# pierotofy/OpenSplat

Hardware: NVIDIA H100
Metric: fwd_bwd_mpixel_per_s (higher is better)
Workload: dtype f32

## Files before the change

include/gsplat_b200.h:

```cpp
#ifndef GSPLAT_B200_H
#define GSPLAT_B200_H

#include <stddef.h>
#include <stdint.h>

#ifdef __cplusplus
extern "C" {
#endif

#define GSB_TILE 16
#define GSB_ERR_INVALID_ARG (-1)
#define GSB_ERR_WORKSPACE (-2)
#define GSB_ERR_UNSUPPORTED (-3)
#define GSB_RASTER_CLAMP_MAX_ONE 1u
#define GSB_BIN_COUNT_VISIBLE 2

typedef void *gsb_stream_t;

int gsb_version(void);
const char *gsb_last_error(void);

int gsb_sh_forward(int n, int degree, int degrees_to_use, const float *viewdirs, const float *coeffs,
                   float *colors, gsb_stream_t stream);
int gsb_sh_backward(int n, int degree, int degrees_to_use, const float *viewdirs, const float *v_colors,
                    float *v_coeffs, gsb_stream_t stream);

int gsb_sh_forward_rgb(int n, int degree, int degrees_to_use, const float *viewdirs, const float *coeffs,
                       float bias, float *rgbs, gsb_stream_t stream);
int gsb_sh_backward_rgb(int n, int degree, int degrees_to_use, const float *viewdirs, const float *rgbs,
                        const float *v_rgbs, float *v_coeffs, gsb_stream_t stream);

int gsb_sh_forward_split(int n, int degree, int degrees_to_use, const float *means, const float *cam_pos,
                         const float *features_dc, const float *features_rest, float bias, float *rgbs,
                         gsb_stream_t stream);
int gsb_sh_backward_split(int n, int degree, int degrees_to_use, const float *means, const float *cam_pos,
                          const float *rgbs, const float *v_rgbs, float *v_features_dc, float *v_features_rest,
                          gsb_stream_t stream);
int gsb_sh_forward_rgb_cam(int n, int degree, int degrees_to_use, const float *means, const float *cam_pos,
                           const float *coeffs, float bias, float *rgbs, gsb_stream_t stream);
int gsb_sh_backward_rgb_cam(int n, int degree, int degrees_to_use, const float *means, const float *cam_pos,
                            const float *rgbs, const float *v_rgbs, float *v_coeffs, gsb_stream_t stream);
int gsb_sh_forward_rgb_cam_multiview(int n, int degree, int degrees_to_use, const float *means, int num_views,
                                     const float *cam_positions, const float *coeffs, float bias, float *rgbs,
                                     gsb_stream_t stream);

int gsb_mask_rgb_grad(int n, const float *rgbs, float *v_rgbs, gsb_stream_t stream);
int gsb_sh_backward_multiview(int n, int degree, int degrees_to_use, const float *means, int num_views,
                              const float *cam_positions, const float *const *v_rgbs_per_view, float scale,
                              float *v_coeffs, gsb_stream_t stream);
int gsb_exchange_gradients(int n, int degree, int degrees_to_use, const float *means, int num_views,
                           const float *cam_positions, const float *const *v_rgbs_per_view, float scale,
                           float *v_coeffs, int rank, int world, long long geom_floats,
                           float *const *geom_per_rank, float *geom_multicast, gsb_stream_t stream);
int gsb_sh_backward_multiview_cams(int n, int degree, int degrees_to_use, const float *means, int num_views,
                                   const float *const *cam_pos_per_view, const float *const *v_rgbs_per_view,
                                   float scale, float *v_coeffs, gsb_stream_t stream);
int gsb_exchange_gradients_cams(int n, int degree, int degrees_to_use, const float *means, int num_views,
                                const float *const *cam_pos_per_view, const float *const *v_rgbs_per_view,
                                float scale, float *v_coeffs, int rank, int world, long long geom_floats,
                                float *const *geom_per_rank, float *geom_multicast, gsb_stream_t stream);

int gsb_project_forward(int n, const float *means3d, const float *scales, float glob_scale,
                        const float *quats, const float *viewmat, const float *projmat, float fx, float fy,
                        float cx, float cy, int img_h, int img_w, int tiles_x, int tiles_y,
                        float clip_thresh, float *cov3d, float *xys, float *depths, int32_t *radii,
                        float *conics, int32_t *num_tiles_hit, gsb_stream_t stream);
int gsb_project_backward(int n, const float *means3d, const float *scales, float glob_scale,
                         const float *quats, const float *viewmat, const float *projmat, float fx, float fy,
                         float cx, float cy, int img_h, int img_w, const float *cov3d,
                         const int32_t *radii, const float *conics, const float *v_xy,
                         const float *v_depth, const float *v_conic, float *v_mean3d, float *v_scale,
                         float *v_quat, gsb_stream_t stream);
int gsb_project_forward_activated(int n, const float *means3d, const float *log_scales, float glob_scale,
                                  const float *raw_quats, const float *opacity_logits, const float *viewmat,
                                  const float *projmat, float fx, float fy, float cx, float cy, int img_h,
                                  int img_w, int tiles_x, int tiles_y, float clip_thresh, float *cov3d, float *xys,
                                  float *depths, int32_t *radii, float *conics, int32_t *num_tiles_hit,
                                  float *opacities, gsb_stream_t stream);
int gsb_project_backward_activated(int n, const float *means3d, const float *log_scales, float glob_scale,
                                   const float *raw_quats, const float *opacities, const float *viewmat,
                                   const float *projmat, float fx, float fy, int img_h, int img_w,
                                   const int32_t *radii, const float *conics, const float *v_xy,
                                   const float *v_depth, const float *v_conic, const float *v_opacity,
                                   float *v_mean3d, float *v_log_scales, float *v_raw_quats,
                                   float *v_opacity_logits, gsb_stream_t stream);
int gsb_project_backward_activated_acc(int n, const float *means3d, const float *log_scales, float glob_scale,
                                       const float *raw_quats, const float *opacities, const float *viewmat,
                                       const float *projmat, float fx, float fy, int img_h, int img_w,
                                       const int32_t *radii, const float *conics, const float *v_xy,
                                       const float *v_depth, const float *v_conic, const float *v_opacity,
                                       float *v_mean3d, float *v_log_scales, float *v_raw_quats,
                                       float *v_opacity_logits, gsb_stream_t stream);
int gsb_project_forward_activated_aa(int n, const float *means3d, const float *log_scales, float glob_scale,
                                     const float *raw_quats, const float *opacity_logits, const float *viewmat,
                                     const float *projmat, float fx, float fy, float cx, float cy, int img_h,
                                     int img_w, int tiles_x, int tiles_y, float clip_thresh, float *cov3d, float *xys,
                                     float *depths, int32_t *radii, float *conics, int32_t *num_tiles_hit,
                                     float *opacities, gsb_stream_t stream);
int gsb_project_backward_activated_aa(int n, const float *means3d, const float *log_scales, float glob_scale,
                                      const float *raw_quats, const float *opacity_logits, const float *viewmat,
                                      const float *projmat, float fx, float fy, int img_h, int img_w,
                                      const int32_t *radii, const float *conics, const float *v_xy,
                                      const float *v_depth, const float *v_conic, const float *v_opacity,
                                      float *v_mean3d, float *v_log_scales, float *v_raw_quats,
                                      float *v_opacity_logits, gsb_stream_t stream);
int gsb_project_backward_activated_aa_acc(int n, const float *means3d, const float *log_scales, float glob_scale,
                                          const float *raw_quats, const float *opacity_logits, const float *viewmat,
                                          const float *projmat, float fx, float fy, int img_h, int img_w,
                                          const int32_t *radii, const float *conics, const float *v_xy,
                                          const float *v_depth, const float *v_conic, const float *v_opacity,
                                          float *v_mean3d, float *v_log_scales, float *v_raw_quats,
                                          float *v_opacity_logits, gsb_stream_t stream);

size_t gsb_cumsum_workspace_bytes(int n);
int gsb_cumsum_tiles_hit(int n, const int32_t *num_tiles_hit, int32_t *cum_tiles_hit, void *workspace,
                         size_t workspace_bytes, gsb_stream_t stream);
int gsb_map_gaussian_to_intersects(int n, int m, const float *xys, const float *depths,
                                   const int32_t *radii, const int32_t *cum_tiles_hit, int tiles_x,
                                   int tiles_y, int64_t *isect_ids, int32_t *gaussian_ids,
                                   gsb_stream_t stream);
size_t gsb_sort_workspace_bytes(int m);
int gsb_sort_intersects(int m, int num_tiles, const int64_t *isect_ids, int64_t *isect_ids_sorted,
                        int32_t *sorted_index, void *workspace, size_t workspace_bytes,
                        gsb_stream_t stream);
int gsb_gather_bin_edges(int m, int num_tiles, const int64_t *isect_ids_sorted,
                         const int32_t *sorted_index, const int32_t *gaussian_ids,
                         int32_t *gaussian_ids_sorted, int32_t *tile_bins, gsb_stream_t stream);

int gsb_bucket_max_tile_len(void);
size_t gsb_bucket_workspace_bytes(int n, int m_capacity, int num_tiles);
int gsb_bucket_tile_ranges(int n, const float *xys, const int32_t *radii, const float *conics, const float *colors,
                           const float *opacities, int cull, int tiles_x, int tiles_y, int m_capacity,
                           int len_capacity, void *workspace, size_t workspace_bytes, int32_t *cum_tiles_hit,
                           int32_t *tile_bins, int32_t *tile_order, int32_t *stats, gsb_stream_t stream);
int gsb_bucket_sort_pack(int n, int m_capacity, int len_capacity, const float *depths, const int32_t *radii,
                         const int32_t *cum_tiles_hit, int cull, int tiles_x, int tiles_y, const int32_t *tile_bins,
                         const int32_t *stats, void *workspace, size_t workspace_bytes, void *records,
                         int32_t *sorted_index, int32_t *gaussian_ids_sorted, gsb_stream_t stream);

size_t gsb_raster_records_bytes(int m);
size_t gsb_raster_grad_rows_bytes(int m);
int gsb_pack_records(int m, const int32_t *gaussian_ids_sorted, const int32_t *sorted_index, const float *xys,
                     const float *conics, const float *colors, const float *opacities, void *records,
                     gsb_stream_t stream);
int gsb_rasterize_forward_packed(int img_h, int img_w, int tiles_x, int tiles_y, int m, const int32_t *tile_bins,
                                 const int32_t *tile_order, const int32_t *bin_stats, const float *background,
                                 void *records, float *out_img, float *final_Ts, int32_t *final_idx,
                                 unsigned flags, gsb_stream_t stream);
int gsb_rasterize_forward_count(int img_h, int img_w, int tiles_x, int tiles_y, int m, const int32_t *tile_bins,
                                const float *background, void *records, float *out_img, float *final_Ts,
                                int32_t *final_idx, unsigned long long *pair_counts, gsb_stream_t stream);
int gsb_rasterize_backward(int img_h, int img_w, int tiles_x, int tiles_y, int n, int m, const int32_t *tile_bins,
                           const int32_t *tile_order, const float *conics, const float *opacities, void *records,
                           const int32_t *cum_tiles_hit, const float *background, const float *final_Ts,
                           const int32_t *final_idx, const float *v_output, const float *v_output_alpha,
                           void *grad_rows, float *v_xy, float *v_conic, float *v_colors, float *v_opacity,
                           unsigned flags, gsb_stream_t stream);
int gsb_gather_record_depths(int m, const int32_t *gaussian_ids_sorted, const float *depths, const int32_t *bin_stats,
                             float *record_depths, gsb_stream_t stream);
int gsb_rasterize_forward_packed_depth(int img_h, int img_w, int tiles_x, int tiles_y, int m, const int32_t *tile_bins,
                                       const int32_t *tile_order, const int32_t *bin_stats, const float *background,
                                       void *records, float *out_img, float *final_Ts, int32_t *final_idx,
                                       unsigned flags, const float *record_depths, float *out_depth, float *out_alpha,
                                       gsb_stream_t stream);
int gsb_rasterize_backward_depth(int img_h, int img_w, int tiles_x, int tiles_y, int n, int m,
                                 const int32_t *tile_bins, const int32_t *tile_order, const float *conics,
                                 const float *opacities, void *records, const int32_t *cum_tiles_hit,
                                 const float *background, const float *final_Ts, const int32_t *final_idx,
                                 const float *v_output, const float *v_output_alpha, void *grad_rows, float *v_xy,
                                 float *v_conic, float *v_colors, float *v_opacity, unsigned flags,
                                 const float *record_depths, const float *v_output_depth, float *v_depths,
                                 gsb_stream_t stream);
int gsb_rasterize_backward_absgrad(int img_h, int img_w, int tiles_x, int tiles_y, int n, int m,
                                   const int32_t *tile_bins, const int32_t *tile_order, const float *conics,
                                   const float *opacities, void *records, const int32_t *cum_tiles_hit,
                                   const float *background, const float *final_Ts, const int32_t *final_idx,
                                   const float *v_output, const float *v_output_alpha, void *grad_rows, float *v_xy,
                                   float *v_conic, float *v_colors, float *v_opacity, unsigned flags,
                                   const float *record_depths, const float *v_output_depth, float *v_depths,
                                   float *v_xy_abs, gsb_stream_t stream);

int gsb_mse_loss_grad(long long n, const float *img, const float *target, float *v_img, float *loss_out,
                      float inv_count, gsb_stream_t stream);
int gsb_adam_step(long long n, float *param, const float *grad, float *exp_avg, float *exp_avg_sq, float lr,
                  float beta1, float beta2, float eps, float bias_correction1, float bias_correction2,
                  gsb_stream_t stream);
#define GSB_ADAM_MAX_SEGMENTS 8
typedef struct gsb_adam_segment {
    long long offset, count;
    int row_floats, head_floats;
    float lr_head, lr_rest;
} gsb_adam_segment;
int gsb_adam_step_segments(int num_segments, const gsb_adam_segment *segments, float *param, const float *grad,
                           float *exp_avg, float *exp_avg_sq, float beta1, float beta2, float eps,
                           float bias_correction1, float bias_correction2, gsb_stream_t stream);

int gsb_activate_forward(int n, const float *means, const float *log_scales, const float *raw_quats,
                         const float *opacity_logits, const float *cam_pos, float *scales, float *quats,
                         float *opacities, float *viewdirs, gsb_stream_t stream);
int gsb_activate_backward(int n, const float *scales, const float *raw_quats, const float *opacities,
                          const float *v_scales, const float *v_quats, const float *v_opacities,
                          float *v_log_scales, float *v_raw_quats, float *v_opacity_logits, gsb_stream_t stream);

int gsb_densify_stats_update(int n, const float *v_xy, const int32_t *radii, int img_h, int img_w,
                             float *xys_grad_norm, float *vis_counts, float *max_2d_size, gsb_stream_t stream);
int gsb_densify_stats_init(int n, const float *v_xy, const int32_t *radii, int img_h, int img_w,
                           float *xys_grad_norm, float *vis_counts, float *max_2d_size, gsb_stream_t stream);

size_t gsb_densify_workspace_bytes(int n);
int gsb_densify_classify(int n, const float *scales, const float *opacities, const float *xys_grad_norm,
                         const float *vis_counts, const float *max_2d_size, float max_dim,
                         float densify_grad_thresh, float densify_size_thresh, int check_split_screen,
                         float split_screen_size, float cull_alpha_thresh, int check_huge, float cull_scale_thresh,
                         int check_cull_screen, float cull_screen_size, float size_fac, void *workspace,
                         size_t workspace_bytes, int32_t *src_map, int32_t *split_rank, int32_t *counts,
                         gsb_stream_t stream);
int gsb_densify_means_scales(int new_n, int n_splits, const int32_t *src_map, const int32_t *split_rank,
                             const float *samples, const float *means, const float *scales, const float *quats,
                             float size_fac, float *new_means, float *new_scales, gsb_stream_t stream);
int gsb_densify_gather_rows(int new_n, int row_floats, const int32_t *src_map, const float *src, float *dst,
                            int zero_children, gsb_stream_t stream);
int gsb_reset_opacity(int n, float max_logit, float *opacities, float *exp_avg, float *exp_avg_sq,
                      gsb_stream_t stream);

#define GSB_MCMC_MAX_SEGMENTS 8
typedef struct gsb_row_segment {
    long long offset;
    int row_floats, reserved;
} gsb_row_segment;
size_t gsb_mcmc_workspace_bytes(int n);
int gsb_mcmc_plan(int n, const float *logits, float min_opacity, int mask_dead, void *workspace,
                  size_t workspace_bytes, double *cdf, int32_t *dead, int32_t *result, gsb_stream_t stream);
int gsb_mcmc_sample(int num_samples, int n, const double *cdf, unsigned key0, unsigned key1, int step, int tag,
                    int32_t *samples, int32_t *counts, gsb_stream_t stream);
int gsb_mcmc_relocate(int n, const int32_t *counts, float min_opacity, float *logits, float *log_scales,
                      int zero_moments, int num_segments, const gsb_row_segment *segments, float *exp_avg,
                      float *exp_avg_sq, gsb_stream_t stream);
int gsb_mcmc_copy_rows(int num_rows, const int32_t *dst_rows, const int32_t *src_rows, int num_segments,
                       const gsb_row_segment *segments, float *param, gsb_stream_t stream);
int gsb_mcmc_regularize(int n, const float *logits, const float *log_scales, float opacity_coef, float scale_coef,
                        float *grad_logits, float *grad_log_scales, gsb_stream_t stream);
int gsb_mcmc_add_noise(int n, const float *logits, const float *log_scales, const float *raw_quats, unsigned key0,
                       unsigned key1, int step, float noise_scale, float *means, gsb_stream_t stream);
int gsb_mcmc_draws(int count, unsigned key0, unsigned key1, int step, int tag, int32_t *words, float *normals,
                   gsb_stream_t stream);

#define GSB_BILAGRID_X 16
#define GSB_BILAGRID_Y 16
#define GSB_BILAGRID_L 8
#define GSB_BILAGRID_COEFFS 12
#define GSB_BILAGRID_FLOATS (GSB_BILAGRID_L * GSB_BILAGRID_Y * GSB_BILAGRID_X * GSB_BILAGRID_COEFFS)
int gsb_bilagrid_slice_forward(int H, int W, const float *grid, const float *rgb, float *out, gsb_stream_t stream);
size_t gsb_bilagrid_workspace_bytes(int H, int W);
int gsb_bilagrid_slice_backward(int H, int W, const float *grid, const float *rgb, const float *v_out, float scale,
                                float *v_rgb, float *v_grid, void *workspace, size_t workspace_bytes,
                                gsb_stream_t stream);
int gsb_bilagrid_tv(int num_grids, const float *grids, float weight, float *v_grids, float *tv_out,
                    gsb_stream_t stream);

#define GSB_POSE_FLOATS 9
size_t gsb_project_camera_partials_floats(int n);
int gsb_project_backward_activated_camgrad(int n, const float *means3d, const float *log_scales, float glob_scale,
                                           const float *raw_quats, const float *opacities, const float *viewmat,
                                           const float *projmat, float fx, float fy, int img_h, int img_w,
                                           const int32_t *radii, const float *conics, const float *v_xy,
                                           const float *v_depth, const float *v_conic, const float *v_opacity,
                                           float *v_mean3d, float *v_log_scales, float *v_raw_quats,
                                           float *v_opacity_logits, int accumulate, int antialiased,
                                           float *cam_partials, gsb_stream_t stream);
int gsb_project_camera_grad_reduce(int nblocks, const float *partials, float *v_viewmat, float *v_projmat,
                                   gsb_stream_t stream);
int gsb_pose_apply(const float *pose, const float *view, const float *centre, float *view_out, float *centre_out,
                   gsb_stream_t stream);
int gsb_pose_backward(const float *pose, const float *view, const float *proj, const float *v_viewmat,
                      const float *v_projmat, float scale, float *grad, gsb_stream_t stream);

int gsb_inverse_depths(int n, const float *depths, const int32_t *radii, float *inv, gsb_stream_t stream);
int gsb_inverse_depths_backward(int n, const float *depths, const int32_t *radii, const float *v_inv, float *v_z,
                                gsb_stream_t stream);
size_t gsb_inverse_depth_l1_workspace_bytes(int img_h, int img_w);
int gsb_inverse_depth_l1(int img_h, int img_w, const float *rendered, const float *prior, float scale_g,
                         float *v_rendered, float *loss_out, void *workspace, size_t workspace_bytes,
                         gsb_stream_t stream);
int gsb_depth_downscale_mean(int h, int w, int factor, const float *src, float *dst, gsb_stream_t stream);

int gsb_ply_row_floats(int sh_bases);
int gsb_pack_ply_rows(int n, int sh_bases, const float *means, const float *features_dc, int dc_stride,
                      const float *features_rest, int rest_stride, const float *opacities, const float *scales,
                      const float *quats, int keep_crs, float crs_scale, const float *crs_translation,
                      float *out_rows, gsb_stream_t stream);
int gsb_unpack_ply_rows(int n, int sh_bases, const float *rows, int keep_crs, float crs_scale,
                        const float *crs_translation, float *means, float *features_dc, int dc_stride,
                        float *features_rest, int rest_stride, float *opacities, float *scales, float *quats,
                        gsb_stream_t stream);
int gsb_splat_order_keys(int n, const float *scales, const float *opacities, int keep_crs, float crs_scale,
                         int64_t *keys, gsb_stream_t stream);
int gsb_pack_splat_rows(int n, const int32_t *order, const float *means, const float *scales,
                        const float *features_dc, int dc_stride, const float *opacities, const float *quats,
                        int keep_crs, float crs_scale, const float *crs_translation, void *out_rows,
                        gsb_stream_t stream);

size_t gsb_ssim_workspace_bytes(int img_h, int img_w);
int gsb_ssim_l1_loss(int img_h, int img_w, const float *rendered, const float *gt, float ssim_weight,
                     float *v_rendered, float *loss_out, void *workspace, size_t workspace_bytes,
                     gsb_stream_t stream);

size_t gsb_knn_workspace_bytes(int n);
int gsb_knn_mean_dist(int n, const float *xyz, float *mean_dist, void *workspace, size_t workspace_bytes,
                      gsb_stream_t stream);

#define GSB_FILTER3D_CAM_FLOATS 18
int gsb_project_forward_activated_filter3d(int n, const float *means3d, const float *log_scales, float glob_scale,
                                           const float *raw_quats, const float *opacity_logits, const float *filter3d,
                                           const float *viewmat, const float *projmat, float fx, float fy, float cx,
                                           float cy, int img_h, int img_w, int tiles_x, int tiles_y,
                                           float clip_thresh, float *cov3d, float *xys, float *depths, int32_t *radii,
                                           float *conics, int32_t *num_tiles_hit, float *opacities, int antialiased,
                                           gsb_stream_t stream);
int gsb_project_backward_activated_filter3d(int n, const float *means3d, const float *log_scales, float glob_scale,
                                            const float *raw_quats, const float *opacity_logits,
                                            const float *filter3d, const float *viewmat, const float *projmat,
                                            float fx, float fy, int img_h, int img_w, const int32_t *radii,
                                            const float *conics, const float *v_xy, const float *v_depth,
                                            const float *v_conic, const float *v_opacity, float *v_mean3d,
                                            float *v_log_scales, float *v_raw_quats, float *v_opacity_logits,
                                            int accumulate, int antialiased, int camgrad, float *cam_partials,
                                            gsb_stream_t stream);
size_t gsb_filter3d_workspace_bytes(void);
int gsb_filter3d_compute(int n, const float *means, int num_cameras, const float *cameras, float near, float margin,
                         float variance, void *workspace, size_t workspace_bytes, float *filter3d,
                         gsb_stream_t stream);
int gsb_filter3d_bake(int n, const float *log_scales, const float *opacity_logits, const float *filter3d,
                      float *out_log_scales, float *out_opacity_logits, gsb_stream_t stream);
int gsb_reset_opacity_filter3d(int n, float max_logit, float reset_value, const float *log_scales,
                               const float *filter3d, float *opacities, float *exp_avg, float *exp_avg_sq,
                               gsb_stream_t stream);

int gsb_resize_area_u8(int src_h, int src_w, const uint8_t *src, int dst_h, int dst_w, uint8_t *dst, float inv_scale,
                       gsb_stream_t stream);
int gsb_undistort_u8(int h, int w, const uint8_t *src, float fx, float fy, float cx, float cy, float k1, float k2,
                     float p1, float p2, float k3, float new_fx, float new_fy, float new_cx, float new_cy, int roi_x,
                     int roi_y, int roi_w, int roi_h, uint8_t *dst, gsb_stream_t stream);
int gsb_u8_to_f32_views(int num_views, const int64_t *views, int h, int w, float *out, gsb_stream_t stream);

#ifdef __cplusplus
}
#endif
#endif
```

opensplat_b200/capi.py:

```python
import ctypes as C
import os

import torch

_HERE = os.path.dirname(os.path.abspath(__file__))
LIB_PATH = os.environ.get("GSB_LIB") or os.path.join(_HERE, "lib", "libgsplat_b200.so")
_lib = None

_vp, _i, _f, _sz = C.c_void_p, C.c_int, C.c_float, C.c_size_t

_SIGS = {
    "gsb_version": (C.c_int, []),
    "gsb_last_error": (C.c_char_p, []),
    "gsb_sh_forward": (_i, [_i, _i, _i, _vp, _vp, _vp, _vp]),
    "gsb_sh_backward": (_i, [_i, _i, _i, _vp, _vp, _vp, _vp]),
    "gsb_sh_forward_rgb": (_i, [_i, _i, _i, _vp, _vp, _f, _vp, _vp]),
    "gsb_sh_backward_rgb": (_i, [_i, _i, _i, _vp, _vp, _vp, _vp, _vp]),
    "gsb_sh_forward_split": (_i, [_i, _i, _i, _vp, _vp, _vp, _vp, _f, _vp, _vp]),
    "gsb_sh_backward_split": (_i, [_i, _i, _i, _vp, _vp, _vp, _vp, _vp, _vp, _vp]),
    "gsb_sh_forward_rgb_cam": (_i, [_i, _i, _i, _vp, _vp, _vp, _f, _vp, _vp]),
    "gsb_sh_backward_rgb_cam": (_i, [_i, _i, _i, _vp, _vp, _vp, _vp, _vp, _vp]),
    "gsb_sh_forward_rgb_cam_multiview": (_i, [_i, _i, _i, _vp, _i, _vp, _vp, _f, _vp, _vp]),
    "gsb_mask_rgb_grad": (_i, [_i, _vp, _vp, _vp]),
    "gsb_sh_backward_multiview": (_i, [_i, _i, _i, _vp, _i, _vp, _vp, _f, _vp, _vp]),
    "gsb_exchange_gradients": (_i, [_i, _i, _i, _vp, _i, _vp, _vp, _f, _vp, _i, _i, C.c_longlong, _vp, _vp, _vp]),
    "gsb_sh_backward_multiview_cams": (_i, [_i, _i, _i, _vp, _i, _vp, _vp, _f, _vp, _vp]),
    "gsb_exchange_gradients_cams": (_i, [_i, _i, _i, _vp, _i, _vp, _vp, _f, _vp, _i, _i, C.c_longlong, _vp, _vp,
                                         _vp]),
    "gsb_project_forward": (_i, [_i, _vp, _vp, _f, _vp, _vp, _vp, _f, _f, _f, _f, _i, _i, _i, _i, _f,
                                 _vp, _vp, _vp, _vp, _vp, _vp, _vp]),
    "gsb_project_backward": (_i, [_i, _vp, _vp, _f, _vp, _vp, _vp, _f, _f, _f, _f, _i, _i,
                                  _vp, _vp, _vp, _vp, _vp, _vp, _vp, _vp, _vp, _vp]),
    "gsb_project_forward_activated": (_i, [_i, _vp, _vp, _f, _vp, _vp, _vp, _vp, _f, _f, _f, _f, _i, _i, _i, _i, _f,
                                           _vp, _vp, _vp, _vp, _vp, _vp, _vp, _vp]),
    "gsb_project_backward_activated": (_i, [_i, _vp, _vp, _f, _vp, _vp, _vp, _vp, _f, _f, _i, _i,
                                            _vp, _vp, _vp, _vp, _vp, _vp, _vp, _vp, _vp, _vp, _vp]),
    "gsb_project_backward_activated_acc": (_i, [_i, _vp, _vp, _f, _vp, _vp, _vp, _vp, _f, _f, _i, _i,
                                                _vp, _vp, _vp, _vp, _vp, _vp, _vp, _vp, _vp, _vp, _vp]),
    "gsb_project_forward_activated_aa": (_i, [_i, _vp, _vp, _f, _vp, _vp, _vp, _vp, _f, _f, _f, _f, _i, _i, _i, _i,
                                              _f, _vp, _vp, _vp, _vp, _vp, _vp, _vp, _vp]),
    "gsb_project_backward_activated_aa": (_i, [_i, _vp, _vp, _f, _vp, _vp, _vp, _vp, _f, _f, _i, _i,
                                               _vp, _vp, _vp, _vp, _vp, _vp, _vp, _vp, _vp, _vp, _vp]),
    "gsb_project_backward_activated_aa_acc": (_i, [_i, _vp, _vp, _f, _vp, _vp, _vp, _vp, _f, _f, _i, _i,
                                                   _vp, _vp, _vp, _vp, _vp, _vp, _vp, _vp, _vp, _vp, _vp]),
    "gsb_cumsum_workspace_bytes": (_sz, [_i]),
    "gsb_cumsum_tiles_hit": (_i, [_i, _vp, _vp, _vp, _sz, _vp]),
    "gsb_map_gaussian_to_intersects": (_i, [_i, _i, _vp, _vp, _vp, _vp, _i, _i, _vp, _vp, _vp]),
    "gsb_sort_workspace_bytes": (_sz, [_i]),
    "gsb_sort_intersects": (_i, [_i, _i, _vp, _vp, _vp, _vp, _sz, _vp]),
    "gsb_gather_bin_edges": (_i, [_i, _i, _vp, _vp, _vp, _vp, _vp, _vp]),
    "gsb_raster_records_bytes": (_sz, [_i]),
    "gsb_raster_grad_rows_bytes": (_sz, [_i]),
    "gsb_pack_records": (_i, [_i, _vp, _vp, _vp, _vp, _vp, _vp, _vp, _vp]),
    "gsb_rasterize_forward_packed": (_i, [_i, _i, _i, _i, _i, _vp, _vp, _vp, _vp, _vp, _vp, _vp, _vp, C.c_uint, _vp]),
    "gsb_rasterize_forward_count": (_i, [_i, _i, _i, _i, _i, _vp, _vp, _vp, _vp, _vp, _vp, _vp, _vp]),
    "gsb_rasterize_backward": (_i, [_i, _i, _i, _i, _i, _i, _vp, _vp, _vp, _vp, _vp, _vp, _vp, _vp, _vp, _vp,
                                    _vp, _vp, _vp, _vp, _vp, _vp, C.c_uint, _vp]),
    "gsb_gather_record_depths": (_i, [_i, _vp, _vp, _vp, _vp, _vp]),
    "gsb_rasterize_forward_packed_depth": (_i, [_i, _i, _i, _i, _i, _vp, _vp, _vp, _vp, _vp, _vp, _vp, _vp, C.c_uint,
                                                _vp, _vp, _vp, _vp]),
    "gsb_rasterize_backward_depth": (_i, [_i, _i, _i, _i, _i, _i, _vp, _vp, _vp, _vp, _vp, _vp, _vp, _vp, _vp, _vp,
                                          _vp, _vp, _vp, _vp, _vp, _vp, C.c_uint, _vp, _vp, _vp, _vp]),
    "gsb_rasterize_backward_absgrad": (_i, [_i, _i, _i, _i, _i, _i, _vp, _vp, _vp, _vp, _vp, _vp, _vp, _vp, _vp, _vp,
                                            _vp, _vp, _vp, _vp, _vp, _vp, C.c_uint, _vp, _vp, _vp, _vp, _vp]),
    "gsb_bucket_max_tile_len": (_i, []),
    "gsb_bucket_workspace_bytes": (_sz, [_i, _i, _i]),
    "gsb_bucket_tile_ranges": (_i, [_i, _vp, _vp, _vp, _vp, _vp, _i, _i, _i, _i, _i, _vp, _sz, _vp, _vp, _vp, _vp, _vp]),
    "gsb_bucket_sort_pack": (_i, [_i, _i, _i, _vp, _vp, _vp, _i, _i, _i, _vp, _vp, _vp, _sz, _vp, _vp, _vp, _vp]),
    "gsb_activate_forward": (_i, [_i, _vp, _vp, _vp, _vp, _vp, _vp, _vp, _vp, _vp, _vp]),
    "gsb_activate_backward": (_i, [_i, _vp, _vp, _vp, _vp, _vp, _vp, _vp, _vp, _vp, _vp]),
    "gsb_densify_stats_update": (_i, [_i, _vp, _vp, _i, _i, _vp, _vp, _vp, _vp]),
    "gsb_densify_stats_init": (_i, [_i, _vp, _vp, _i, _i, _vp, _vp, _vp, _vp]),
    "gsb_densify_workspace_bytes": (_sz, [_i]),
    "gsb_densify_classify": (_i, [_i, _vp, _vp, _vp, _vp, _vp, _f, _f, _f, _i, _f, _f, _i, _f, _i, _f, _f, _vp, _sz,
                                  _vp, _vp, _vp, _vp]),
    "gsb_densify_means_scales": (_i, [_i, _i, _vp, _vp, _vp, _vp, _vp, _vp, _f, _vp, _vp, _vp]),
    "gsb_densify_gather_rows": (_i, [_i, _i, _vp, _vp, _vp, _i, _vp]),
    "gsb_reset_opacity": (_i, [_i, _f, _vp, _vp, _vp, _vp]),
    "gsb_mcmc_workspace_bytes": (_sz, [_i]),
    "gsb_mcmc_plan": (_i, [_i, _vp, _f, _i, _vp, _sz, _vp, _vp, _vp, _vp]),
    "gsb_mcmc_sample": (_i, [_i, _i, _vp, C.c_uint, C.c_uint, _i, _i, _vp, _vp, _vp]),
    "gsb_mcmc_relocate": (_i, [_i, _vp, _f, _vp, _vp, _i, _i, _vp, _vp, _vp, _vp]),
    "gsb_mcmc_copy_rows": (_i, [_i, _vp, _vp, _i, _vp, _vp, _vp]),
    "gsb_mcmc_regularize": (_i, [_i, _vp, _vp, _f, _f, _vp, _vp, _vp]),
    "gsb_mcmc_add_noise": (_i, [_i, _vp, _vp, _vp, C.c_uint, C.c_uint, _i, _f, _vp, _vp]),
    "gsb_mcmc_draws": (_i, [_i, C.c_uint, C.c_uint, _i, _i, _vp, _vp, _vp]),
    "gsb_bilagrid_slice_forward": (_i, [_i, _i, _vp, _vp, _vp, _vp]),
    "gsb_bilagrid_workspace_bytes": (_sz, [_i, _i]),
    "gsb_bilagrid_slice_backward": (_i, [_i, _i, _vp, _vp, _vp, _f, _vp, _vp, _vp, _sz, _vp]),
    "gsb_bilagrid_tv": (_i, [_i, _vp, _f, _vp, _vp, _vp]),
    "gsb_project_camera_partials_floats": (_sz, [_i]),
    "gsb_project_backward_activated_camgrad": (_i, [_i, _vp, _vp, _f, _vp, _vp, _vp, _vp, _f, _f, _i, _i,
                                                    _vp, _vp, _vp, _vp, _vp, _vp, _vp, _vp, _vp, _vp, _i, _i, _vp,
                                                    _vp]),
    "gsb_project_camera_grad_reduce": (_i, [_i, _vp, _vp, _vp, _vp]),
    "gsb_pose_apply": (_i, [_vp, _vp, _vp, _vp, _vp, _vp]),
    "gsb_pose_backward": (_i, [_vp, _vp, _vp, _vp, _vp, _f, _vp, _vp]),
    "gsb_inverse_depths": (_i, [_i, _vp, _vp, _vp, _vp]),
    "gsb_inverse_depths_backward": (_i, [_i, _vp, _vp, _vp, _vp, _vp]),
    "gsb_inverse_depth_l1_workspace_bytes": (_sz, [_i, _i]),
    "gsb_inverse_depth_l1": (_i, [_i, _i, _vp, _vp, _f, _vp, _vp, _vp, _sz, _vp]),
    "gsb_depth_downscale_mean": (_i, [_i, _i, _i, _vp, _vp, _vp]),
    "gsb_project_forward_activated_filter3d": (_i, [_i, _vp, _vp, _f, _vp, _vp, _vp, _vp, _vp, _f, _f, _f, _f, _i, _i,
                                                    _i, _i, _f, _vp, _vp, _vp, _vp, _vp, _vp, _vp, _i, _vp]),
    "gsb_project_backward_activated_filter3d": (_i, [_i, _vp, _vp, _f, _vp, _vp, _vp, _vp, _vp, _f, _f, _i, _i,
                                                     _vp, _vp, _vp, _vp, _vp, _vp, _vp, _vp, _vp, _vp, _i, _i, _i,
                                                     _vp, _vp]),
    "gsb_filter3d_workspace_bytes": (_sz, []),
    "gsb_filter3d_compute": (_i, [_i, _vp, _i, _vp, _f, _f, _f, _vp, _sz, _vp, _vp]),
    "gsb_filter3d_bake": (_i, [_i, _vp, _vp, _vp, _vp, _vp, _vp]),
    "gsb_reset_opacity_filter3d": (_i, [_i, _f, _f, _vp, _vp, _vp, _vp, _vp, _vp]),
    "gsb_ply_row_floats": (_i, [_i]),
    "gsb_pack_ply_rows": (_i, [_i, _i, _vp, _vp, _i, _vp, _i, _vp, _vp, _vp, _i, _f, C.POINTER(C.c_float), _vp, _vp]),
    "gsb_unpack_ply_rows": (_i, [_i, _i, _vp, _i, _f, C.POINTER(C.c_float), _vp, _vp, _i, _vp, _i, _vp, _vp, _vp, _vp]),
    "gsb_splat_order_keys": (_i, [_i, _vp, _vp, _i, _f, _vp, _vp]),
    "gsb_pack_splat_rows": (_i, [_i, _vp, _vp, _vp, _vp, _i, _vp, _vp, _i, _f, C.POINTER(C.c_float), _vp, _vp]),
    "gsb_ssim_workspace_bytes": (_sz, [_i, _i]),
    "gsb_ssim_l1_loss": (_i, [_i, _i, _vp, _vp, _f, _vp, _vp, _vp, _sz, _vp]),
    "gsb_adam_step": (_i, [C.c_longlong, _vp, _vp, _vp, _vp, _f, _f, _f, _f, _f, _f, _vp]),
    "gsb_adam_step_segments": (_i, [_i, _vp, _vp, _vp, _vp, _vp, _f, _f, _f, _f, _f, _vp]),
    "gsb_mse_loss_grad": (_i, [C.c_longlong, _vp, _vp, _vp, _vp, _f, _vp]),
    "gsb_knn_workspace_bytes": (_sz, [_i]),
    "gsb_knn_mean_dist": (_i, [_i, _vp, _vp, _vp, _sz, _vp]),
    "gsb_resize_area_u8": (_i, [_i, _i, _vp, _i, _i, _vp, _f, _vp]),
    "gsb_undistort_u8": (_i, [_i, _i, _vp, _f, _f, _f, _f, _f, _f, _f, _f, _f, _f, _f, _f, _f, _i, _i, _i, _i, _vp,
                              _vp]),
    "gsb_u8_to_f32_views": (_i, [_i, _vp, _i, _i, _vp, _vp]),
}

ADAM_MAX_SEGMENTS = 8


class AdamSegment(C.Structure):
    _fields_ = [("offset", C.c_longlong), ("count", C.c_longlong), ("row_floats", C.c_int),
                ("head_floats", C.c_int), ("lr_head", C.c_float), ("lr_rest", C.c_float)]


MCMC_MAX_SEGMENTS = 8


class RowSegment(C.Structure):
    _fields_ = [("offset", C.c_longlong), ("row_floats", C.c_int), ("reserved", C.c_int)]


BILAGRID_X, BILAGRID_Y, BILAGRID_L, BILAGRID_COEFFS = 16, 16, 8, 12
BILAGRID_FLOATS = BILAGRID_L * BILAGRID_Y * BILAGRID_X * BILAGRID_COEFFS
POSE_FLOATS = 9
CAMGRAD_TERMS = 24
FILTER3D_CAM_FLOATS = 18


_OPT_SIGS = {}


class GsbError(RuntimeError):
    pass


def lib():
    global _lib
    if _lib is None:
        if not os.path.exists(LIB_PATH):
            raise GsbError(f"{LIB_PATH} not built -- run `python -m opensplat_b200.build` "
                           "(there is no CPU fallback)")
        L = C.CDLL(LIB_PATH)
        for name, (res, args) in _SIGS.items():
            fn = getattr(L, name)
            fn.restype, fn.argtypes = res, args
        for name, (res, args) in _OPT_SIGS.items():
            if hasattr(L, name):
                fn = getattr(L, name)
                fn.restype, fn.argtypes = res, args
        _lib = L
    return _lib


def exported_symbols():
    return list(_SIGS.keys())


def check(code):
    if code != 0:
        raise GsbError(lib().gsb_last_error().decode() or f"gsplat_b200 error {code}")


def ptr(t):
    if t is None:
        return None
    if not t.is_cuda:
        raise GsbError("gsplat_b200 kernels need CUDA tensors (no CPU fallback)")
    if not t.is_contiguous():
        raise GsbError("tensor must be contiguous")
    return t.data_ptr()


def stream():
    return torch.cuda.current_stream().cuda_stream


def f32(t):
    return t.contiguous() if t.dtype == torch.float32 else t.float().contiguous()
```

opensplat_b200/csrc/project.cu:

```cuda
#include "gsb_common.cuh"

namespace {

constexpr int PJ_THREADS = 256;
constexpr int CG_TERMS = 24;

__device__ __forceinline__ void camgrad_block_sum(const float (&cg)[CG_TERMS], float *__restrict__ out) {
    __shared__ float red[PJ_THREADS / 32][CG_TERMS];
    const int lane = threadIdx.x & 31, warp = threadIdx.x >> 5;
#pragma unroll
    for (int k = 0; k < CG_TERMS; ++k) {
        float v = cg[k];
#pragma unroll
        for (int o = 16; o > 0; o >>= 1) v = v + __shfl_down_sync(0xffffffffu, v, o);
        if (lane == 0) red[warp][k] = v;
    }
    __syncthreads();
    if (threadIdx.x < CG_TERMS) {
        float v = red[0][threadIdx.x];
#pragma unroll
        for (int w = 1; w < PJ_THREADS / 32; ++w) v = v + red[w][threadIdx.x];
        out[threadIdx.x] = v;
    }
}

struct Cam {
    float V[12];
    float P[16];
};

__device__ __forceinline__ void quat_to_rotmat(float qw, float qx, float qy, float qz, float R[3][3]) {
    float s = 1.0f / sqrtf(qw * qw + qx * qx + qy * qy + qz * qz);
    float w = qw * s, x = qx * s, y = qy * s, z = qz * s;
    R[0][0] = 1.f - 2.f * (y * y + z * z);
    R[0][1] = 2.f * (x * y - w * z);
    R[0][2] = 2.f * (x * z + w * y);
    R[1][0] = 2.f * (x * y + w * z);
    R[1][1] = 1.f - 2.f * (x * x + z * z);
    R[1][2] = 2.f * (y * z - w * x);
    R[2][0] = 2.f * (x * z - w * y);
    R[2][1] = 2.f * (y * z + w * x);
    R[2][2] = 1.f - 2.f * (x * x + y * y);
}

__device__ __forceinline__ void load_cam(const float *__restrict__ viewmat,
                                         const float *__restrict__ projmat, Cam &c) {
#pragma unroll
    for (int i = 0; i < 12; ++i) c.V[i] = __ldg(viewmat + i);
#pragma unroll
    for (int i = 0; i < 16; ++i) c.P[i] = __ldg(projmat + i);
}

__device__ __forceinline__ void filter3d_scales(float glob_scale, const float (&e)[3], float f, float (&sig)[3],
                                                float (&r)[3], float &c3) {
    const float ff = f * f;
#pragma unroll
    for (int k = 0; k < 3; ++k) {
        const float s = glob_scale * e[k];
        sig[k] = sqrtf(s * s + ff);
        r[k] = s / sig[k];
    }
    c3 = r[0] * r[1] * r[2];
}

template <bool ACT, bool AA = false, bool F3D = false>
__global__ void __launch_bounds__(PJ_THREADS)
project_forward_kernel(int n, const float *__restrict__ means3d, const float *__restrict__ scales,
                       float glob_scale, const float *__restrict__ quats,
                       const float *__restrict__ viewmat, const float *__restrict__ projmat, float fx,
                       float fy, float cx, float cy, float tan_fovx, float tan_fovy, int img_h, int img_w,
                       int tiles_x, int tiles_y, float clip_thresh, float *__restrict__ cov3d,
                       float2 *__restrict__ xys, float *__restrict__ depths, int *__restrict__ radii,
                       float *__restrict__ conics, int *__restrict__ num_tiles_hit,
                       const float *__restrict__ opacity_logits, float *__restrict__ opacities,
                       const float *__restrict__ filter3d = nullptr) {
    static_assert(ACT || !AA, "the anti-aliased opacity needs the activated projection");
    static_assert(ACT || !F3D, "the 3-D filter needs the activated projection");
    const int i = blockIdx.x * PJ_THREADS + threadIdx.x;
    if (i >= n) return;
    if (ACT && !AA && !F3D) opacities[i] = 1.f / (1.f + expf(-opacity_logits[i]));
    float fsig[3] = {0.f, 0.f, 0.f}, fc3 = 1.f;
    if constexpr (F3D) {
        const float e[3] = {expf(scales[3 * i]), expf(scales[3 * i + 1]), expf(scales[3 * i + 2])};
        float r[3];
        filter3d_scales(glob_scale, e, filter3d[i], fsig, r, fc3);
        if (!AA) opacities[i] = 1.f / (1.f + expf(-opacity_logits[i])) * fc3;
    }
    float comp = 0.f;
    Cam cam;
    load_cam(viewmat, projmat, cam);
    const float *V = cam.V, *P = cam.P;

    float c3[6] = {0.f, 0.f, 0.f, 0.f, 0.f, 0.f};
    float conic0 = 0.f, conic1 = 0.f, conic2 = 0.f;
    float ux = 0.f, uy = 0.f, depth = 0.f;
    int radius_i = 0, area = 0;

    const float px = means3d[3 * i], py = means3d[3 * i + 1], pz = means3d[3 * i + 2];
    const float tx = V[0] * px + V[1] * py + V[2] * pz + V[3];
    const float ty = V[4] * px + V[5] * py + V[6] * pz + V[7];
    const float tz = V[8] * px + V[9] * py + V[10] * pz + V[11];
    if (tz > clip_thresh) {
        const float4 q = reinterpret_cast<const float4 *>(quats)[i];
        float R[3][3], M[3][3];
        quat_to_rotmat(q.x, q.y, q.z, q.w, R);
        const float a0 = scales[3 * i], a1 = scales[3 * i + 1], a2 = scales[3 * i + 2];
        const float s0 = F3D ? fsig[0] : glob_scale * (ACT ? expf(a0) : a0),
                    s1 = F3D ? fsig[1] : glob_scale * (ACT ? expf(a1) : a1),
                    s2 = F3D ? fsig[2] : glob_scale * (ACT ? expf(a2) : a2);
#pragma unroll
        for (int r = 0; r < 3; ++r) {
            M[r][0] = R[r][0] * s0;
            M[r][1] = R[r][1] * s1;
            M[r][2] = R[r][2] * s2;
        }
        float C[3][3];
#pragma unroll
        for (int r = 0; r < 3; ++r)
#pragma unroll
            for (int c = 0; c < 3; ++c)
                C[r][c] = M[r][0] * M[c][0] + M[r][1] * M[c][1] + M[r][2] * M[c][2];
        c3[0] = C[0][0]; c3[1] = C[0][1]; c3[2] = C[0][2];
        c3[3] = C[1][1]; c3[4] = C[1][2]; c3[5] = C[2][2];

        const float lim_x = 1.3f * tan_fovx, lim_y = 1.3f * tan_fovy;
        const float ttx = tz * fminf(lim_x, fmaxf(-lim_x, tx / tz));
        const float tty = tz * fminf(lim_y, fmaxf(-lim_y, ty / tz));
        const float rz = 1.f / tz, rz2 = rz * rz;
        const float J00 = fx * rz, J02 = -fx * ttx * rz2, J11 = fy * rz, J12 = -fy * tty * rz2;
        float T[2][3];
#pragma unroll
        for (int c = 0; c < 3; ++c) {
            T[0][c] = J00 * V[c] + J02 * V[8 + c];
            T[1][c] = J11 * V[4 + c] + J12 * V[8 + c];
        }
        const float Cs[3][3] = {{c3[0], c3[1], c3[2]}, {c3[1], c3[3], c3[4]}, {c3[2], c3[4], c3[5]}};
        float TV[2][3];
#pragma unroll
        for (int r = 0; r < 2; ++r)
#pragma unroll
            for (int c = 0; c < 3; ++c)
                TV[r][c] = T[r][0] * Cs[0][c] + T[r][1] * Cs[1][c] + T[r][2] * Cs[2][c];
        const float cxx0 = TV[0][0] * T[0][0] + TV[0][1] * T[0][1] + TV[0][2] * T[0][2];
        const float cxy = TV[0][0] * T[1][0] + TV[0][1] * T[1][1] + TV[0][2] * T[1][2];
        const float cyy0 = TV[1][0] * T[1][0] + TV[1][1] * T[1][1] + TV[1][2] * T[1][2];
        const float cxx = cxx0 + 0.3f, cyy = cyy0 + 0.3f;

        const float det = cxx * cyy - cxy * cxy;
        if (det != 0.f) {
            const float inv_det = 1.f / det;
            conic0 = cyy * inv_det;
            conic1 = -cxy * inv_det;
            conic2 = cxx * inv_det;
            const float b = 0.5f * (cxx + cyy);
            const float sq = sqrtf(fmaxf(0.1f, b * b - det));
            const float v1 = b + sq, v2 = b - sq;
            const float radius = ceilf(3.f * sqrtf(fmaxf(v1, v2)));

            const float hx = P[0] * px + P[1] * py + P[2] * pz + P[3];
            const float hy = P[4] * px + P[5] * py + P[6] * pz + P[7];
            const float hw = P[12] * px + P[13] * py + P[14] * pz + P[15];
            const float rw = 1.f / (hw + 1e-6f);
            const float ndcx = hx * rw, ndcy = hy * rw;
            const float pxc = 0.5f * (float)img_w * ndcx + cx - 0.5f;
            const float pyc = 0.5f * (float)img_h * ndcy + cy - 0.5f;

            int x0, x1, y0, y1;
            gsb_tile_bbox(pxc, pyc, radius, tiles_x, tiles_y, x0, x1, y0, y1);
            const int a = (x1 - x0) * (y1 - y0);
            if (a > 0) {
                area = a;
                depth = tz;
                radius_i = (int)radius;
                ux = pxc;
                uy = pyc;
                if (AA && radius_i > 0) comp = sqrtf(fmaxf(0.f, (cxx0 * cyy0 - cxy * cxy) / det));
            }
        }
    }
    if constexpr (AA && F3D) opacities[i] = 1.f / (1.f + expf(-opacity_logits[i])) * fc3 * comp;
    else if (AA) opacities[i] = 1.f / (1.f + expf(-opacity_logits[i])) * comp;
    float *c3o = cov3d + 6 * (size_t)i;
#pragma unroll
    for (int k = 0; k < 6; ++k) c3o[k] = c3[k];
    xys[i] = make_float2(ux, uy);
    depths[i] = depth;
    radii[i] = radius_i;
    conics[3 * i] = conic0;
    conics[3 * i + 1] = conic1;
    conics[3 * i + 2] = conic2;
    num_tiles_hit[i] = area;
}

template <bool ACT, bool ACC, bool AA = false, bool CAMGRAD = false, bool F3D = false>
__global__ void __launch_bounds__(PJ_THREADS)
project_backward_kernel(int n, const float *__restrict__ means3d, const float *__restrict__ scales,
                        float glob_scale, const float *__restrict__ quats,
                        const float *__restrict__ viewmat, const float *__restrict__ projmat, float fx,
                        float fy, float tan_fovx, float tan_fovy, int img_h, int img_w,
                        const int *__restrict__ radii, const float *__restrict__ conics,
                        const float2 *__restrict__ v_xy, const float *__restrict__ v_depth,
                        const float *__restrict__ v_conic, float *__restrict__ v_mean3d,
                        float *__restrict__ v_scale, float4 *__restrict__ v_quat,
                        const float *__restrict__ opacities, const float *__restrict__ v_opacity,
                        float *__restrict__ v_opacity_logits, float *__restrict__ cam_partials = nullptr,
                        const float *__restrict__ filter3d = nullptr) {
    static_assert(ACT || !AA, "the anti-aliased opacity needs the activated projection");
    static_assert(ACT || !F3D, "the 3-D filter needs the activated projection");
    static_assert(ACT || !CAMGRAD, "the camera gradient is taken with the activated projection");
    const int i = blockIdx.x * PJ_THREADS + threadIdx.x;
    if (!CAMGRAD && i >= n) return;
    float cg[CG_TERMS];
#pragma unroll
    for (int k = 0; k < CG_TERMS; ++k) cg[k] = 0.f;
    if (!CAMGRAD || i < n) {
        float comp = 0.f;
        float f3 = 0.f, fr[3] = {1.f, 1.f, 1.f}, fc3 = 1.f, fsh[3] = {0.f, 0.f, 0.f};
        if constexpr (F3D) f3 = filter3d[i];
        if (ACT && !AA && !F3D) {
            const float o = opacities[i];
            if constexpr (ACC)
                v_opacity_logits[i] = v_opacity_logits[i] + (v_opacity ? v_opacity[i] * o * (1.f - o) : 0.f);
            else
                v_opacity_logits[i] = v_opacity ? v_opacity[i] * o * (1.f - o) : 0.f;
        }
        float vm[3] = {0.f, 0.f, 0.f}, vs[3] = {0.f, 0.f, 0.f};
        float4 vq = make_float4(0.f, 0.f, 0.f, 0.f);
        if (radii[i] > 0) {
            Cam cam;
            load_cam(viewmat, projmat, cam);
            const float *V = cam.V, *P = cam.P;
            const float px = means3d[3 * i], py = means3d[3 * i + 1], pz = means3d[3 * i + 2];

            const float hx = P[0] * px + P[1] * py + P[2] * pz + P[3];
            const float hy = P[4] * px + P[5] * py + P[6] * pz + P[7];
            const float hw = P[12] * px + P[13] * py + P[14] * pz + P[15];
            const float rw = 1.f / (hw + 1e-6f);
            const float2 vxy = v_xy[i];
            const float vndcx = 0.5f * (float)img_w * vxy.x, vndcy = 0.5f * (float)img_h * vxy.y;
            const float vhx = vndcx * rw, vhy = vndcy * rw;
            const float vhw = -(vndcx * hx + vndcy * hy) * rw * rw;
            vm[0] = P[0] * vhx + P[4] * vhy + P[12] * vhw;
            vm[1] = P[1] * vhx + P[5] * vhy + P[13] * vhw;
            vm[2] = P[2] * vhx + P[6] * vhy + P[14] * vhw;

            const float tx = V[0] * px + V[1] * py + V[2] * pz + V[3];
            const float ty = V[4] * px + V[5] * py + V[6] * pz + V[7];
            const float tz = V[8] * px + V[9] * py + V[10] * pz + V[11];
            float vtx = 0.f, vty = 0.f, vtz = v_depth ? v_depth[i] : 0.f;

            const float A = conics[3 * i], B = conics[3 * i + 1], Cc = conics[3 * i + 2];
            const float gA = v_conic[3 * i], gB = 0.5f * v_conic[3 * i + 1], gC = v_conic[3 * i + 2];
            const float xg00 = A * gA + B * gB, xg01 = A * gB + B * gC;
            const float xg10 = B * gA + Cc * gB, xg11 = B * gB + Cc * gC;
            float vS00 = -(xg00 * A + xg01 * B);
            float vS01 = -(xg00 * B + xg01 * Cc);
            float vS11 = -(xg10 * B + xg11 * Cc);

            const float4 q = reinterpret_cast<const float4 *>(quats)[i];
            float R[3][3], M[3][3];
            quat_to_rotmat(q.x, q.y, q.z, q.w, R);
            const float a[3] = {scales[3 * i], scales[3 * i + 1], scales[3 * i + 2]};
            const float e[3] = {ACT ? expf(a[0]) : a[0], ACT ? expf(a[1]) : a[1], ACT ? expf(a[2]) : a[2]};
            float s[3] = {glob_scale * e[0], glob_scale * e[1], glob_scale * e[2]};
            if constexpr (F3D) filter3d_scales(glob_scale, e, f3, s, fr, fc3);
#pragma unroll
            for (int r = 0; r < 3; ++r)
#pragma unroll
                for (int c = 0; c < 3; ++c) M[r][c] = R[r][c] * s[c];
            float Cs[3][3];
#pragma unroll
            for (int r = 0; r < 3; ++r)
#pragma unroll
                for (int c = 0; c < 3; ++c)
                    Cs[r][c] = M[r][0] * M[c][0] + M[r][1] * M[c][1] + M[r][2] * M[c][2];
            const float lim_x = 1.3f * tan_fovx, lim_y = 1.3f * tan_fovy;
            const float qx = tx / tz, qy = ty / tz;
            const bool clamp_x = !(qx > -lim_x && qx < lim_x), clamp_y = !(qy > -lim_y && qy < lim_y);
            const float cqx = fminf(lim_x, fmaxf(-lim_x, qx)), cqy = fminf(lim_y, fmaxf(-lim_y, qy));
            const float ttx = tz * cqx, tty = tz * cqy;
            const float rz = 1.f / tz, rz2 = rz * rz, rz3 = rz2 * rz;
            const float J00 = fx * rz, J02 = -fx * ttx * rz2, J11 = fy * rz, J12 = -fy * tty * rz2;
            float T[2][3];
#pragma unroll
            for (int c = 0; c < 3; ++c) {
                T[0][c] = J00 * V[c] + J02 * V[8 + c];
                T[1][c] = J11 * V[4 + c] + J12 * V[8 + c];
            }
            if constexpr (AA) {
                float TV[2][3];
#pragma unroll
                for (int r = 0; r < 2; ++r)
#pragma unroll
                    for (int c = 0; c < 3; ++c)
                        TV[r][c] = T[r][0] * Cs[0][c] + T[r][1] * Cs[1][c] + T[r][2] * Cs[2][c];
                const float cxx0 = TV[0][0] * T[0][0] + TV[0][1] * T[0][1] + TV[0][2] * T[0][2];
                const float cxy = TV[0][0] * T[1][0] + TV[0][1] * T[1][1] + TV[0][2] * T[1][2];
                const float cyy0 = TV[1][0] * T[1][0] + TV[1][1] * T[1][1] + TV[1][2] * T[1][2];
                const float det = (cxx0 + 0.3f) * (cyy0 + 0.3f) - cxy * cxy;
                comp = sqrtf(fmaxf(0.f, (cxx0 * cyy0 - cxy * cxy) / det));
                if (v_opacity && comp > 0.f) {
                    const float o = 1.f / (1.f + expf(-opacities[i]));
                    const float k = 0.5f * (v_opacity[i] * (F3D ? o * fc3 : o)) / comp;
                    const float id = 1.f / det;
                    const float a = cyy0 * id, b = cxy * id, c = cxx0 * id, e = 0.3f * id;
                    vS00 = vS00 + k * (0.3f * (a * a + b * b + e * a));
                    vS01 = vS01 - k * (0.3f * (b * (a + c + e)));
                    vS11 = vS11 + k * (0.3f * (c * c + b * b + e * c));
                }
            }
            float vST[2][3];
#pragma unroll
            for (int c = 0; c < 3; ++c) {
                vST[0][c] = vS00 * T[0][c] + vS01 * T[1][c];
                vST[1][c] = vS01 * T[0][c] + vS11 * T[1][c];
            }
            float vV[3][3];
#pragma unroll
            for (int r = 0; r < 3; ++r)
#pragma unroll
                for (int c = 0; c < 3; ++c) vV[r][c] = T[0][r] * vST[0][c] + T[1][r] * vST[1][c];
            float vT[2][3];
#pragma unroll
            for (int r = 0; r < 2; ++r)
#pragma unroll
                for (int c = 0; c < 3; ++c)
                    vT[r][c] = 2.f * (vST[r][0] * Cs[0][c] + vST[r][1] * Cs[1][c] + vST[r][2] * Cs[2][c]);
            const float vJ00 = vT[0][0] * V[0] + vT[0][1] * V[1] + vT[0][2] * V[2];
            const float vJ02 = vT[0][0] * V[8] + vT[0][1] * V[9] + vT[0][2] * V[10];
            const float vJ11 = vT[1][0] * V[4] + vT[1][1] * V[5] + vT[1][2] * V[6];
            const float vJ12 = vT[1][0] * V[8] + vT[1][1] * V[9] + vT[1][2] * V[10];
            const float vttx = -fx * rz2 * vJ02, vtty = -fy * rz2 * vJ12;
            vtz += -fx * rz2 * vJ00 + 2.f * fx * ttx * rz3 * vJ02 - fy * rz2 * vJ11 +
                   2.f * fy * tty * rz3 * vJ12;
            if (qx == lim_x || qx == -lim_x) { const float h = 0.5f * vttx; vtx += h; vtz += cqx * h; }
            else if (clamp_x) vtz += cqx * vttx; else vtx += vttx;
            if (qy == lim_y || qy == -lim_y) { const float h = 0.5f * vtty; vty += h; vtz += cqy * h; }
            else if (clamp_y) vtz += cqy * vtty; else vty += vtty;
            vm[0] += V[0] * vtx + V[4] * vty + V[8] * vtz;
            vm[1] += V[1] * vtx + V[5] * vty + V[9] * vtz;
            vm[2] += V[2] * vtx + V[6] * vty + V[10] * vtz;
            if constexpr (CAMGRAD) {
                const float pc[3] = {px, py, pz}, vt[3] = {vtx, vty, vtz}, vh[3] = {vhx, vhy, vhw};
#pragma unroll
                for (int r = 0; r < 3; ++r) {
#pragma unroll
                    for (int c = 0; c < 3; ++c) {
                        cg[4 * r + c] = vt[r] * pc[c];
                        cg[12 + 4 * r + c] = vh[r] * pc[c];
                    }
                    cg[4 * r + 3] = vt[r];
                    cg[12 + 4 * r + 3] = vh[r];
                }
#pragma unroll
                for (int c = 0; c < 3; ++c) {
                    cg[c] = cg[c] + J00 * vT[0][c];
                    cg[4 + c] = cg[4 + c] + J11 * vT[1][c];
                    cg[8 + c] = cg[8 + c] + (J02 * vT[0][c] + J12 * vT[1][c]);
                }
            }

            float vM[3][3];
#pragma unroll
            for (int r = 0; r < 3; ++r)
#pragma unroll
                for (int c = 0; c < 3; ++c)
                    vM[r][c] = 2.f * (vV[r][0] * M[0][c] + vV[r][1] * M[1][c] + vV[r][2] * M[2][c]);
#pragma unroll
            for (int c = 0; c < 3; ++c) {
                vs[c] = glob_scale * (R[0][c] * vM[0][c] + R[1][c] * vM[1][c] + R[2][c] * vM[2][c]);
                if (ACT) vs[c] = vs[c] * e[c];
                if (F3D) vs[c] = vs[c] * fr[c];
            }
            float vR[3][3];
#pragma unroll
            for (int r = 0; r < 3; ++r)
#pragma unroll
                for (int c = 0; c < 3; ++c) vR[r][c] = vM[r][c] * s[c];
            const float nq = sqrtf(q.x * q.x + q.y * q.y + q.z * q.z + q.w * q.w);
            const float inv = 1.0f / nq;
            const float w = q.x * inv, x = q.y * inv, y = q.z * inv, z = q.w * inv;
            const float gw = 2.f * (x * (vR[2][1] - vR[1][2]) + y * (vR[0][2] - vR[2][0]) + z * (vR[1][0] - vR[0][1]));
            const float gx = 2.f * (-2.f * x * (vR[1][1] + vR[2][2]) + y * (vR[1][0] + vR[0][1]) +
                                    z * (vR[2][0] + vR[0][2]) + w * (vR[2][1] - vR[1][2]));
            const float gy = 2.f * (x * (vR[1][0] + vR[0][1]) - 2.f * y * (vR[0][0] + vR[2][2]) +
                                    z * (vR[2][1] + vR[1][2]) + w * (vR[0][2] - vR[2][0]));
            const float gz = 2.f * (x * (vR[2][0] + vR[0][2]) + y * (vR[2][1] + vR[1][2]) -
                                    2.f * z * (vR[0][0] + vR[1][1]) + w * (vR[1][0] - vR[0][1]));
            const float dot = w * gw + x * gx + y * gy + z * gz;
            vq = make_float4((gw - w * dot) * inv, (gx - x * dot) * inv, (gy - y * dot) * inv,
                             (gz - z * dot) * inv);
            if constexpr (F3D) {
#pragma unroll
                for (int k = 0; k < 3; ++k) { const float t = f3 / s[k]; fsh[k] = t * t; }
            }
        } else if constexpr (F3D) {
            const float e[3] = {expf(scales[3 * i]), expf(scales[3 * i + 1]), expf(scales[3 * i + 2])};
            float sg[3];
            filter3d_scales(glob_scale, e, f3, sg, fr, fc3);
#pragma unroll
            for (int k = 0; k < 3; ++k) { const float t = f3 / sg[k]; fsh[k] = t * t; }
        }
        if constexpr (AA && !F3D) {
            float vol = 0.f;
            if (v_opacity) {
                const float o = 1.f / (1.f + expf(-opacities[i]));
                vol = v_opacity[i] * comp * o * (1.f - o);
            }
            v_opacity_logits[i] = ACC ? v_opacity_logits[i] + vol : vol;
        }
        if constexpr (F3D) {
            float vol = 0.f;
            if (v_opacity) {
                const float o = 1.f / (1.f + expf(-opacities[i]));
                vol = AA ? v_opacity[i] * fc3 * comp * o * (1.f - o) : v_opacity[i] * fc3 * o * (1.f - o);
                if (f3 > 0.f) {
                    const float vo = v_opacity[i] * (AA ? o * fc3 * comp : o * fc3);
#pragma unroll
                    for (int k = 0; k < 3; ++k) vs[k] = vs[k] + vo * fsh[k];
                }
            }
            v_opacity_logits[i] = ACC ? v_opacity_logits[i] + vol : vol;
        }
        if constexpr (ACC) {
            const float4 pq = v_quat[i];
            v_mean3d[3 * i] += vm[0]; v_mean3d[3 * i + 1] += vm[1]; v_mean3d[3 * i + 2] += vm[2];
            v_scale[3 * i] += vs[0]; v_scale[3 * i + 1] += vs[1]; v_scale[3 * i + 2] += vs[2];
            v_quat[i] = make_float4(pq.x + vq.x, pq.y + vq.y, pq.z + vq.z, pq.w + vq.w);
        } else {
            v_mean3d[3 * i] = vm[0]; v_mean3d[3 * i + 1] = vm[1]; v_mean3d[3 * i + 2] = vm[2];
            v_scale[3 * i] = vs[0]; v_scale[3 * i + 1] = vs[1]; v_scale[3 * i + 2] = vs[2];
            v_quat[i] = vq;
        }
    }
    if constexpr (CAMGRAD) camgrad_block_sum(cg, cam_partials + CG_TERMS * (size_t)blockIdx.x);
}

__global__ void __launch_bounds__(CG_TERMS * 32)
camgrad_reduce_kernel(int nblocks, const float *__restrict__ partials, float *__restrict__ v_viewmat,
                      float *__restrict__ v_projmat) {
    const int k = threadIdx.x >> 5, lane = threadIdx.x & 31;
    double s = 0.0;
    for (int b = lane; b < nblocks; b += 32) s += (double)partials[CG_TERMS * (size_t)b + k];
#pragma unroll
    for (int o = 16; o > 0; o >>= 1) s += __shfl_down_sync(0xffffffffu, s, o);
    if (lane == 0) {
        const float r = (float)s;
        if (k < 12) v_viewmat[k] = r;
        else v_projmat[k < 20 ? k - 12 : k - 8] = r;
    }
    if (threadIdx.x < 4) {
        v_viewmat[12 + threadIdx.x] = 0.f;
        v_projmat[8 + threadIdx.x] = 0.f;
    }
}

}

static int project_forward_impl(bool act, bool aa, int n, const float *means3d, const float *scales, float glob_scale,
                                const float *quats, const float *opacity_logits, const float *filter3d,
                                const float *viewmat,
                                const float *projmat, float fx, float fy, float cx, float cy, int img_h, int img_w,
                                int tiles_x, int tiles_y, float clip_thresh, float *cov3d, float *xys, float *depths,
                                int32_t *radii, float *conics, int32_t *num_tiles_hit, float *opacities,
                                gsb_stream_t stream) {
    GSB_CHECK_ARG(n >= 0 && img_h > 0 && img_w > 0 && tiles_x > 0 && tiles_y > 0);
    if (n == 0) return 0;
    GSB_CHECK_ARG(means3d && scales && quats && viewmat && projmat && cov3d && xys && depths && radii &&
                  conics && num_tiles_hit);
    GSB_CHECK_ARG(!act || (opacity_logits && opacities));
    GSB_CHECK_ARG(((uintptr_t)quats % 16) == 0 && ((uintptr_t)xys % 8) == 0);
    const float tan_fovx = (float)(0.5 * (double)img_w / (double)fx);
    const float tan_fovy = (float)(0.5 * (double)img_h / (double)fy);
#define GSB_PJ_F(A, AA, F3D) project_forward_kernel<A, AA, F3D><<<gsb_div_up(n, PJ_THREADS), PJ_THREADS, 0, (cudaStream_t)stream>>>( \
        n, means3d, scales, glob_scale, quats, viewmat, projmat, fx, fy, cx, cy, tan_fovx, tan_fovy, img_h, img_w,   \
        tiles_x, tiles_y, clip_thresh, cov3d, reinterpret_cast<float2 *>(xys), depths, radii, conics, num_tiles_hit, \
        opacity_logits, opacities, filter3d)
    if (filter3d) { if (aa) GSB_PJ_F(true, true, true); else GSB_PJ_F(true, false, true); }
    else if (aa) GSB_PJ_F(true, true, false); else if (act) GSB_PJ_F(true, false, false);
    else GSB_PJ_F(false, false, false);
#undef GSB_PJ_F
    GSB_LAUNCH_CHECK();
    return 0;
}

extern "C" int gsb_project_forward(int n, const float *means3d, const float *scales, float glob_scale,
                                   const float *quats, const float *viewmat, const float *projmat,
                                   float fx, float fy, float cx, float cy, int img_h, int img_w,
                                   int tiles_x, int tiles_y, float clip_thresh, float *cov3d, float *xys,
                                   float *depths, int32_t *radii, float *conics, int32_t *num_tiles_hit,
                                   gsb_stream_t stream) {
    return project_forward_impl(false, false, n, means3d, scales, glob_scale, quats, nullptr, nullptr, viewmat, projmat, fx, fy, cx,
                                cy, img_h, img_w, tiles_x, tiles_y, clip_thresh, cov3d, xys, depths, radii, conics,
                                num_tiles_hit, nullptr, stream);
}

extern "C" int gsb_project_forward_activated(int n, const float *means3d, const float *log_scales, float glob_scale,
                                             const float *raw_quats, const float *opacity_logits,
                                             const float *viewmat, const float *projmat, float fx, float fy,
                                             float cx, float cy, int img_h, int img_w, int tiles_x, int tiles_y,
                                             float clip_thresh, float *cov3d, float *xys, float *depths,
                                             int32_t *radii, float *conics, int32_t *num_tiles_hit,
                                             float *opacities, gsb_stream_t stream) {
    return project_forward_impl(true, false, n, means3d, log_scales, glob_scale, raw_quats, opacity_logits, nullptr, viewmat, projmat,
                                fx, fy, cx, cy, img_h, img_w, tiles_x, tiles_y, clip_thresh, cov3d, xys, depths, radii,
                                conics, num_tiles_hit, opacities, stream);
}

static int project_backward_impl(bool act, bool acc, bool aa, int n, const float *means3d, const float *scales, float glob_scale,
                                 const float *quats, const float *opacities, const float *viewmat,
                                 const float *projmat, float fx, float fy, int img_h, int img_w,
                                 const int32_t *radii, const float *conics, const float *v_xy, const float *v_depth,
                                 const float *v_conic, const float *v_opacity, float *v_mean3d, float *v_scale,
                                 float *v_quat, float *v_opacity_logits, float *cam_partials, gsb_stream_t stream,
                                 const float *filter3d = nullptr) {
    GSB_CHECK_ARG(n >= 0 && img_h > 0 && img_w > 0);
    if (n == 0) return 0;
    GSB_CHECK_ARG(means3d && scales && quats && viewmat && projmat && radii && conics && v_xy && v_conic &&
                  v_mean3d && v_scale && v_quat);
    GSB_CHECK_ARG(!act || (opacities && v_opacity_logits));
    GSB_CHECK_ARG(((uintptr_t)quats % 16) == 0 && ((uintptr_t)v_quat % 16) == 0 && ((uintptr_t)v_xy % 8) == 0);
    const float tan_fovx = (float)(0.5 * (double)img_w / (double)fx);
    const float tan_fovy = (float)(0.5 * (double)img_h / (double)fy);
#define GSB_PJ_B5(A, ACC, AA, CG, F3D) project_backward_kernel<A, ACC, AA, CG, F3D><<<gsb_div_up(n, PJ_THREADS), PJ_THREADS, 0, (cudaStream_t)stream>>>( \
        n, means3d, scales, glob_scale, quats, viewmat, projmat, fx, fy, tan_fovx, tan_fovy, img_h, img_w, radii,     \
        conics, reinterpret_cast<const float2 *>(v_xy), v_depth, v_conic, v_mean3d, v_scale,                          \
        reinterpret_cast<float4 *>(v_quat), opacities, v_opacity, v_opacity_logits, cam_partials, filter3d)
#define GSB_PJ_B(A, ACC, AA, CG) GSB_PJ_B5(A, ACC, AA, CG, false)
#define GSB_PJ_BF(ACC, AA, CG) GSB_PJ_B5(true, ACC, AA, CG, true)
    if (filter3d) {
        if (cam_partials) {
            if (aa) { if (acc) GSB_PJ_BF(true, true, true); else GSB_PJ_BF(false, true, true); }
            else if (acc) GSB_PJ_BF(true, false, true); else GSB_PJ_BF(false, false, true);
        } else if (aa) { if (acc) GSB_PJ_BF(true, true, false); else GSB_PJ_BF(false, true, false); }
        else if (acc) GSB_PJ_BF(true, false, false); else GSB_PJ_BF(false, false, false);
    } else if (cam_partials) {
        if (aa) { if (acc) GSB_PJ_B(true, true, true, true); else GSB_PJ_B(true, false, true, true); }
        else if (acc) GSB_PJ_B(true, true, false, true); else GSB_PJ_B(true, false, false, true);
    } else if (aa) { if (acc) GSB_PJ_B(true, true, true, false); else GSB_PJ_B(true, false, true, false); }
    else if (acc) GSB_PJ_B(true, true, false, false); else if (act) GSB_PJ_B(true, false, false, false);
    else GSB_PJ_B(false, false, false, false);
#undef GSB_PJ_BF
#undef GSB_PJ_B
#undef GSB_PJ_B5
    GSB_LAUNCH_CHECK();
    return 0;
}

extern "C" int gsb_project_backward(int n, const float *means3d, const float *scales, float glob_scale,
                                    const float *quats, const float *viewmat, const float *projmat,
                                    float fx, float fy, float cx, float cy, int img_h, int img_w,
                                    const float *cov3d, const int32_t *radii, const float *conics,
                                    const float *v_xy, const float *v_depth, const float *v_conic,
                                    float *v_mean3d, float *v_scale, float *v_quat, gsb_stream_t stream) {
    (void)cov3d; (void)cx; (void)cy;
    return project_backward_impl(false, false, false, n, means3d, scales, glob_scale, quats, nullptr, viewmat, projmat, fx,
                                 fy, img_h, img_w, radii, conics, v_xy, v_depth, v_conic, nullptr, v_mean3d, v_scale,
                                 v_quat, nullptr, nullptr, stream);
}

extern "C" int gsb_project_backward_activated(int n, const float *means3d, const float *log_scales, float glob_scale,
                                              const float *raw_quats, const float *opacities, const float *viewmat,
                                              const float *projmat, float fx, float fy, int img_h, int img_w,
                                              const int32_t *radii, const float *conics, const float *v_xy,
                                              const float *v_depth, const float *v_conic, const float *v_opacity,
                                              float *v_mean3d, float *v_log_scales, float *v_raw_quats,
                                              float *v_opacity_logits, gsb_stream_t stream) {
    return project_backward_impl(true, false, false, n, means3d, log_scales, glob_scale, raw_quats, opacities, viewmat,
                                 projmat, fx, fy, img_h, img_w, radii, conics, v_xy, v_depth, v_conic, v_opacity,
                                 v_mean3d, v_log_scales, v_raw_quats, v_opacity_logits, nullptr, stream);
}

extern "C" int gsb_project_backward_activated_acc(int n, const float *means3d, const float *log_scales,
                                                  float glob_scale, const float *raw_quats, const float *opacities,
                                                  const float *viewmat, const float *projmat, float fx, float fy,
                                                  int img_h, int img_w, const int32_t *radii, const float *conics,
                                                  const float *v_xy, const float *v_depth, const float *v_conic,
                                                  const float *v_opacity, float *v_mean3d, float *v_log_scales,
                                                  float *v_raw_quats, float *v_opacity_logits, gsb_stream_t stream) {
    return project_backward_impl(true, true, false, n, means3d, log_scales, glob_scale, raw_quats, opacities, viewmat,
                                 projmat, fx, fy, img_h, img_w, radii, conics, v_xy, v_depth, v_conic, v_opacity,
                                 v_mean3d, v_log_scales, v_raw_quats, v_opacity_logits, nullptr, stream);
}

extern "C" int gsb_project_forward_activated_aa(int n, const float *means3d, const float *log_scales,
                                                float glob_scale, const float *raw_quats, const float *opacity_logits,
                                                const float *viewmat, const float *projmat, float fx, float fy,
                                                float cx, float cy, int img_h, int img_w, int tiles_x, int tiles_y,
                                                float clip_thresh, float *cov3d, float *xys, float *depths,
                                                int32_t *radii, float *conics, int32_t *num_tiles_hit,
                                                float *opacities, gsb_stream_t stream) {
    return project_forward_impl(true, true, n, means3d, log_scales, glob_scale, raw_quats, opacity_logits, nullptr, viewmat,
                                projmat, fx, fy, cx, cy, img_h, img_w, tiles_x, tiles_y, clip_thresh, cov3d, xys,
                                depths, radii, conics, num_tiles_hit, opacities, stream);
}

extern "C" int gsb_project_backward_activated_aa(int n, const float *means3d, const float *log_scales,
                                                 float glob_scale, const float *raw_quats,
                                                 const float *opacity_logits, const float *viewmat,
                                                 const float *projmat, float fx, float fy, int img_h, int img_w,
                                                 const int32_t *radii, const float *conics, const float *v_xy,
                                                 const float *v_depth, const float *v_conic, const float *v_opacity,
                                                 float *v_mean3d, float *v_log_scales, float *v_raw_quats,
                                                 float *v_opacity_logits, gsb_stream_t stream) {
    return project_backward_impl(true, false, true, n, means3d, log_scales, glob_scale, raw_quats, opacity_logits,
                                 viewmat, projmat, fx, fy, img_h, img_w, radii, conics, v_xy, v_depth, v_conic,
                                 v_opacity, v_mean3d, v_log_scales, v_raw_quats, v_opacity_logits, nullptr, stream);
}

extern "C" int gsb_project_backward_activated_aa_acc(int n, const float *means3d, const float *log_scales,
                                                     float glob_scale, const float *raw_quats,
                                                     const float *opacity_logits, const float *viewmat,
                                                     const float *projmat, float fx, float fy, int img_h, int img_w,
                                                     const int32_t *radii, const float *conics, const float *v_xy,
                                                     const float *v_depth, const float *v_conic,
                                                     const float *v_opacity, float *v_mean3d, float *v_log_scales,
                                                     float *v_raw_quats, float *v_opacity_logits,
                                                     gsb_stream_t stream) {
    return project_backward_impl(true, true, true, n, means3d, log_scales, glob_scale, raw_quats, opacity_logits,
                                 viewmat, projmat, fx, fy, img_h, img_w, radii, conics, v_xy, v_depth, v_conic,
                                 v_opacity, v_mean3d, v_log_scales, v_raw_quats, v_opacity_logits, nullptr, stream);
}

extern "C" size_t gsb_project_camera_partials_floats(int n) {
    return n > 0 ? (size_t)CG_TERMS * gsb_div_up(n, PJ_THREADS) : 0;
}

extern "C" int gsb_project_backward_activated_camgrad(int n, const float *means3d, const float *log_scales,
                                                      float glob_scale, const float *raw_quats,
                                                      const float *opacities, const float *viewmat,
                                                      const float *projmat, float fx, float fy, int img_h, int img_w,
                                                      const int32_t *radii, const float *conics, const float *v_xy,
                                                      const float *v_depth, const float *v_conic,
                                                      const float *v_opacity, float *v_mean3d, float *v_log_scales,
                                                      float *v_raw_quats, float *v_opacity_logits, int accumulate,
                                                      int antialiased, float *cam_partials, gsb_stream_t stream) {
    GSB_CHECK_ARG((accumulate == 0 || accumulate == 1) && (antialiased == 0 || antialiased == 1));
    GSB_CHECK_ARG(n >= 0 && (n == 0 || cam_partials));
    return project_backward_impl(true, accumulate != 0, antialiased != 0, n, means3d, log_scales, glob_scale,
                                 raw_quats, opacities, viewmat, projmat, fx, fy, img_h, img_w, radii, conics, v_xy,
                                 v_depth, v_conic, v_opacity, v_mean3d, v_log_scales, v_raw_quats, v_opacity_logits,
                                 cam_partials, stream);
}

extern "C" int gsb_project_camera_grad_reduce(int nblocks, const float *partials, float *v_viewmat, float *v_projmat,
                                              gsb_stream_t stream) {
    GSB_CHECK_ARG(nblocks >= 0 && (nblocks == 0 || partials) && v_viewmat && v_projmat);
    camgrad_reduce_kernel<<<1, CG_TERMS * 32, 0, (cudaStream_t)stream>>>(nblocks, partials, v_viewmat, v_projmat);
    GSB_LAUNCH_CHECK();
    return 0;
}

extern "C" int gsb_project_forward_activated_filter3d(int n, const float *means3d, const float *log_scales,
                                                      float glob_scale, const float *raw_quats,
                                                      const float *opacity_logits, const float *filter3d,
                                                      const float *viewmat, const float *projmat, float fx, float fy,
                                                      float cx, float cy, int img_h, int img_w, int tiles_x,
                                                      int tiles_y, float clip_thresh, float *cov3d, float *xys,
                                                      float *depths, int32_t *radii, float *conics,
                                                      int32_t *num_tiles_hit, float *opacities, int antialiased,
                                                      gsb_stream_t stream) {
    GSB_CHECK_ARG(antialiased == 0 || antialiased == 1);
    GSB_CHECK_ARG(n >= 0 && (n == 0 || filter3d));
    return project_forward_impl(true, antialiased != 0, n, means3d, log_scales, glob_scale, raw_quats, opacity_logits,
                                filter3d, viewmat, projmat, fx, fy, cx, cy, img_h, img_w, tiles_x, tiles_y,
                                clip_thresh, cov3d, xys, depths, radii, conics, num_tiles_hit, opacities, stream);
}

extern "C" int gsb_project_backward_activated_filter3d(int n, const float *means3d, const float *log_scales,
                                                       float glob_scale, const float *raw_quats,
                                                       const float *opacity_logits, const float *filter3d,
                                                       const float *viewmat, const float *projmat, float fx, float fy,
                                                       int img_h, int img_w, const int32_t *radii,
                                                       const float *conics, const float *v_xy, const float *v_depth,
                                                       const float *v_conic, const float *v_opacity, float *v_mean3d,
                                                       float *v_log_scales, float *v_raw_quats,
                                                       float *v_opacity_logits, int accumulate, int antialiased,
                                                       int camgrad, float *cam_partials, gsb_stream_t stream) {
    GSB_CHECK_ARG((accumulate == 0 || accumulate == 1) && (antialiased == 0 || antialiased == 1) &&
                  (camgrad == 0 || camgrad == 1));
    GSB_CHECK_ARG(n >= 0 && (n == 0 || (filter3d && (!camgrad || cam_partials))));
    return project_backward_impl(true, accumulate != 0, antialiased != 0, n, means3d, log_scales, glob_scale,
                                 raw_quats, opacity_logits, viewmat, projmat, fx, fy, img_h, img_w, radii, conics,
                                 v_xy, v_depth, v_conic, v_opacity, v_mean3d, v_log_scales, v_raw_quats,
                                 v_opacity_logits, camgrad ? cam_partials : nullptr, stream, filter3d);
}
```

opensplat_b200/csrc/raster_bwd.cu:

```cuda
#include "raster_common.cuh"

int gsb_blend_grid(const void *kernel, int num_tiles);

namespace {

__device__ __forceinline__ float rcp_approx(float x) {
    float y;
    asm("rcp.approx.ftz.f32 %0, %1;" : "=f"(y) : "f"(x));
    return y;
}

__device__ __forceinline__ void zero_row(float *grad_rows, int k) {
    float4 *row = reinterpret_cast<float4 *>(grad_rows + (size_t)k * GSB_GRAD_ROW_FLOATS);
    const float4 z = make_float4(0.f, 0.f, 0.f, 0.f);
    row[0] = z; row[1] = z; row[2] = z;
}

constexpr int BWD_MIN_BLOCKS = 6;
constexpr int BWD_DEPTH_MIN_BLOCKS = 5;
constexpr int BWD_ABS_MIN_BLOCKS = 5;
constexpr int BWD_DEPTH_ABS_MIN_BLOCKS = 4;
template <bool SAT, bool DEPTH, bool ABS>
__global__ void __launch_bounds__(RK_THREADS, ABS ? (DEPTH ? BWD_DEPTH_ABS_MIN_BLOCKS : BWD_ABS_MIN_BLOCKS)
                                                  : (DEPTH ? BWD_DEPTH_MIN_BLOCKS : BWD_MIN_BLOCKS))
rasterize_backward_kernel(int img_h, int img_w, int tiles_x, int num_tiles,
                          const int2 *__restrict__ tile_bins, const GsbRecord *__restrict__ records,
                          const float *__restrict__ background, const float *__restrict__ final_Ts,
                          const int *__restrict__ final_idx, const float *__restrict__ v_output,
                          const float *__restrict__ v_output_alpha, float *__restrict__ grad_rows,
                          unsigned *__restrict__ tile_counter, const int *__restrict__ tile_order,
                          const float *__restrict__ record_depths, const float *__restrict__ v_output_depth) {
    __shared__ WarpRing rings[RK_WARPS];
    const int warp = threadIdx.x >> 5, lane = threadIdx.x & 31;
    WarpRing &ring = rings[warp];
    if (lane == 0) {
#pragma unroll
        for (int s = 0; s < RK_STAGES; ++s) mbar_init(&ring.full[s], 1);
        mbar_fence_init();
    }
    __syncwarp();
    const float bg0 = __ldg(background), bg1 = __ldg(background + 1), bg2 = __ldg(background + 2);
    unsigned gchunk = 0;

    while (true) {
        int tile = 0;
        if (lane == 0) tile = (int)atomicAdd(tile_counter, 1u);
        tile = __shfl_sync(0xffffffffu, tile, 0);
        if (tile >= num_tiles) break;
        if (tile_order) tile = __ldg(tile_order + tile);
        const int2 range = tile_bins[tile];
        if (range.y <= range.x) continue;

        const int tx = tile % tiles_x, ty = tile / tiles_x;
        const int X = tx * GSB_TILE + (lane & 15);
        const int Y0 = ty * GSB_TILE + (lane >> 4);
        const float px = (float)X;
        const float tile_x0 = (float)(tx * GSB_TILE), tile_y0 = (float)(ty * GSB_TILE);

        float T[RK_PIX], Bq[RK_PIX];
        const float py0 = (float)Y0;
        float vor[RK_PIX], vog[RK_PIX], vob[RK_PIX];
        float vD[RK_PIX];
        int binf[RK_PIX];
        int my_max = -1;
#pragma unroll
        for (int j = 0; j < RK_PIX; ++j) {
            const int Y = Y0 + 2 * j;
            if (X < img_w && Y < img_h) {
                const size_t p = (size_t)Y * img_w + X;
                const float Tf = final_Ts[p];
                T[j] = Tf;
                vor[j] = v_output[3 * p]; vog[j] = v_output[3 * p + 1]; vob[j] = v_output[3 * p + 2];
                binf[j] = final_idx[p];
                if (SAT) {
                    const int f = binf[j];
                    if (f & GSB_SAT_BIT0) vor[j] = 0.f;
                    if (f & (GSB_SAT_BIT0 << 1)) vog[j] = 0.f;
                    if (f & (GSB_SAT_BIT0 << 2)) vob[j] = 0.f;
                    binf[j] = f & ~GSB_SAT_MASK;
                }
                if (DEPTH) vD[j] = v_output_depth ? v_output_depth[p] : 0.f;
                const float voa = v_output_alpha ? v_output_alpha[p] : 0.f;
                Bq[j] = -(Tf * (voa - (bg0 * vor[j] + bg1 * vog[j] + bg2 * vob[j])));
            } else {
                T[j] = 1.f; vor[j] = vog[j] = vob[j] = 0.f; Bq[j] = 0.f;
                if (DEPTH) vD[j] = 0.f;
                binf[j] = -1;
            }
            my_max = max(my_max, binf[j]);
        }
        const int warp_max = __reduce_max_sync(0xffffffffu, my_max);
        const int hi = min(range.y - 1, max(warp_max, range.x - 1));

        for (int idx = hi + 1 + lane; idx < range.y; idx += 32)
            zero_row(grad_rows, __float_as_int(__ldg(&records[idx].q0.w)));
        const int L = hi - range.x + 1;
        if (L <= 0) continue;
        const int nchunks = (L + RK_CHUNK - 1) / RK_CHUNK;

        const unsigned g0 = gchunk;
        auto stage_of = [&](int c) { return (g0 + (unsigned)c) % RK_STAGES; };
        auto parity_of = [&](int c) { return ((g0 + (unsigned)c) / RK_STAGES) & 1u; };
        auto chunk_lo = [&](int c) { return max(range.x, hi + 1 - (c + 1) * RK_CHUNK); };
        auto chunk_cnt = [&](int c) { return (hi + 1 - c * RK_CHUNK) - chunk_lo(c); };
        auto issue = [&](int c) {
            if (lane == 0) {
                const unsigned s = stage_of(c);
                const uint32_t bytes = (uint32_t)chunk_cnt(c) * (uint32_t)sizeof(GsbRecord);
                mbar_arrive_expect_tx(&ring.full[s], bytes);
                tma_load_1d(&ring.rec[s][0], records + chunk_lo(c), bytes, &ring.full[s]);
            }
        };
        const int pro = min(RK_STAGES, nchunks);
        for (int c = 0; c < pro; ++c) issue(c);
        int issued = pro;

        for (int c = 0; c < nchunks; ++c) {
            const unsigned s = stage_of(c);
            float zl = 0.f;
            if (DEPTH && lane < chunk_cnt(c)) zl = __ldg(record_depths + chunk_lo(c) + lane);
            mbar_wait(&ring.full[s], parity_of(c));
            const int lo = chunk_lo(c), cnt = chunk_cnt(c);
            unsigned my_mask = 0;
            if (lane < cnt) {
                my_mask = record_slot_mask(ring.rec[s][lane], tile_x0, tile_y0);
                if (my_mask == 0u) zero_row(grad_rows, __float_as_int(ring.rec[s][lane].q0.w));
            }
            unsigned live = __ballot_sync(0xffffffffu, my_mask != 0u);
            while (live) {
                const int t = 31 - __clz(live);
                live &= ~(1u << t);
                const unsigned rm = __shfl_sync(0xffffffffu, my_mask, t);
                float z = 0.f;
                if (DEPTH) z = __shfl_sync(0xffffffffu, zl, t);
                const int idx = lo + t;
                const float4 q0 = ring.rec[s][t].q0;
                const float4 q1 = ring.rec[s][t].q1;
                const float4 q2 = ring.rec[s][t].q2;
                const float smax = fmaxf(0.f, fmaf(q0.z, GSB_LN2, GSB_SMAX_BIAS));
                const float dx = q0.x - px;
                const float adx2 = q1.x * dx * dx;
                const float bdx = q1.y * dx;
                const float dy0 = q0.y - py0;
                float s0 = 0.f, s1 = 0.f, s2 = 0.f;
                float a_r = 0.f, a_g = 0.f, a_b = 0.f;
                float a_z = 0.f;
                float g_x = 0.f, g_y = 0.f;
                float adx = 0.f, c2 = 0.f;
                if (ABS) { adx = (2.f * q1.x) * dx; c2 = 2.f * q1.z; }
                bool any = false;
                const int jlo = __ffs(rm) - 1, jhi = 31 - __clz(rm);
#define GSB_BWD_SLOT(j)                                                                                   \
    {                                                                                                     \
        const float dy = dy0 - (float)(2 * j);                                                                      \
        const float sigma = fmaf(dy, fmaf(q1.z, dy, bdx), adx2);                                          \
        if (__float_as_uint(sigma) <= __float_as_uint(smax)) {                    \
            const float au = ex2_approx(fmaf(sigma, -GSB_LOG2E, q0.z));           \
            const float alpha = fminf(0.99f, au);                                                         \
            if (idx <= binf[j] && alpha >= (1.f / 255.f)) {                                               \
                any = true;                                                                               \
                const float ra = rcp_approx(1.f - alpha);                                                 \
                T[j] *= ra;                                                                               \
                const float fac = alpha * T[j];                                                           \
                a_r = fmaf(fac, vor[j], a_r);                                                             \
                a_g = fmaf(fac, vog[j], a_g);                                                             \
                a_b = fmaf(fac, vob[j], a_b);                                                             \
                if (DEPTH) a_z = fmaf(fac, vD[j], a_z);                                                   \
                float d = fmaf(q2.z, vob[j], fmaf(q2.y, vog[j], q2.x * vor[j]));         \
                if (DEPTH) d = fmaf(z, vD[j], d);                                        \
                const float v_alpha = fmaf(d, T[j], -(ra * Bq[j]));                                       \
                Bq[j] = fmaf(d, fac, Bq[j]);                                                              \
                 \
                const float w = au * v_alpha;                                                             \
                const float wdy = w * dy;                                                                 \
                s0 += w;                                                                                  \
                s1 += wdy;                                                                                \
                s2 = fmaf(wdy, dy, s2);                                                                   \
                if (ABS) {                                                                                \
                    g_x = fmaf(fabsf(w), fabsf(fmaf(q1.y, dy, adx)), g_x);                                \
                    g_y = fmaf(fabsf(w), fabsf(fmaf(c2, dy, bdx)), g_y);                                  \
                }                                                                                         \
            }                                                                                             \
        }                                                                                                 \
        if (jhi == j) break;                                                                              \
    }
                switch (jlo) {
                    case 0: GSB_BWD_SLOT(0)
                    case 1: GSB_BWD_SLOT(1)
                    case 2: GSB_BWD_SLOT(2)
                    case 3: GSB_BWD_SLOT(3)
                    case 4: GSB_BWD_SLOT(4)
                    case 5: GSB_BWD_SLOT(5)
                    case 6: GSB_BWD_SLOT(6)
                    default: GSB_BWD_SLOT(7)
                }
#undef GSB_BWD_SLOT
                const int k = __float_as_int(q0.w);
                float *row = grad_rows + (size_t)k * GSB_GRAD_ROW_FLOATS;
                if (!__any_sync(0xffffffffu, any)) {
                    if (lane < (ABS ? 12 : DEPTH ? 10 : 9)) row[lane] = 0.f;
                    continue;
                }
                const float sx = dx * s0;
                float v0 = s0, v1 = sx, v2 = s1, v3 = dx * sx, v4 = dx * s1, v5 = s2, v6 = a_r, v7 = a_g;
                float v8 = a_b;
                {
                    const bool up = lane & 16;
                    const float t0 = up ? v0 : v4, t1 = up ? v1 : v5, t2 = up ? v2 : v6, t3 = up ? v3 : v7;
                    const float k0 = up ? v4 : v0, k1 = up ? v5 : v1, k2 = up ? v6 : v2, k3 = up ? v7 : v3;
                    v0 = k0 + __shfl_xor_sync(0xffffffffu, t0, 16);
                    v1 = k1 + __shfl_xor_sync(0xffffffffu, t1, 16);
                    v2 = k2 + __shfl_xor_sync(0xffffffffu, t2, 16);
                    v3 = k3 + __shfl_xor_sync(0xffffffffu, t3, 16);
                }
                {
                    const bool up = lane & 8;
                    const float t0 = up ? v0 : v2, t1 = up ? v1 : v3;
                    const float k0 = up ? v2 : v0, k1 = up ? v3 : v1;
                    v0 = k0 + __shfl_xor_sync(0xffffffffu, t0, 8);
                    v1 = k1 + __shfl_xor_sync(0xffffffffu, t1, 8);
                }
                {
                    const bool up = lane & 4;
                    const float t0 = up ? v0 : v1;
                    const float k0 = up ? v1 : v0;
                    v0 = k0 + __shfl_xor_sync(0xffffffffu, t0, 4);
                }
                v0 += __shfl_xor_sync(0xffffffffu, v0, 2);
                v0 += __shfl_xor_sync(0xffffffffu, v0, 1);
                if (ABS) {
                    const bool up = lane & 16;
                    const float t8 = up ? v8 : a_z, k8 = up ? a_z : v8;
                    const float tg = up ? g_x : g_y, kg = up ? g_y : g_x;
                    v8 = k8 + __shfl_xor_sync(0xffffffffu, t8, 16);
                    const float e = kg + __shfl_xor_sync(0xffffffffu, tg, 16);
                    const bool up8 = lane & 8;
                    const float t = up8 ? v8 : e, kk = up8 ? e : v8;
                    v8 = kk + __shfl_xor_sync(0xffffffffu, t, 8);
#pragma unroll
                    for (int o = 4; o > 0; o >>= 1) v8 += __shfl_xor_sync(0xffffffffu, v8, o);
                    const bool wx = (lane & 7) == 1 && (DEPTH || lane != 17);
                    if (((lane & 3) == 0) || wx) row[wx ? 8 + ((lane >> 3) & 1) * 2 + (lane >> 4) : (lane >> 2)] =
                        wx ? v8 : v0;
                } else if (DEPTH) {
                    const bool up = lane & 16;
                    const float t8 = up ? v8 : a_z, k8 = up ? a_z : v8;
                    v8 = k8 + __shfl_xor_sync(0xffffffffu, t8, 16);
#pragma unroll
                    for (int o = 8; o > 0; o >>= 1) v8 += __shfl_xor_sync(0xffffffffu, v8, o);
                    const bool w8 = (lane == 1), w9 = (lane == 17);
                    if (((lane & 3) == 0) || w8 || w9) row[w8 ? 8 : w9 ? 9 : (lane >> 2)] = (w8 || w9) ? v8 : v0;
                } else {
#pragma unroll
                    for (int o = 16; o > 0; o >>= 1) v8 += __shfl_xor_sync(0xffffffffu, v8, o);
                    const bool w8 = (lane == 1);
                    if (((lane & 3) == 0) || w8) row[w8 ? 8 : (lane >> 2)] = w8 ? v8 : v0;
                }
            }
            __syncwarp();
            if (issued < nchunks) { issue(issued); ++issued; }
        }
        gchunk = g0 + (unsigned)issued;
        __syncwarp();
    }
}

template <bool DEPTH, bool ABS>
__global__ void __launch_bounds__(256)
reduce_grad_rows_kernel(int n, const int *__restrict__ cum_tiles_hit, const float *__restrict__ grad_rows,
                        const float *__restrict__ conics, const float *__restrict__ opacities,
                        float2 *__restrict__ v_xy, float *__restrict__ v_conic,
                        float *__restrict__ v_colors, float *__restrict__ v_opacity, float *__restrict__ v_depths,
                        float2 *__restrict__ v_xy_abs) {
    const int g = blockIdx.x * blockDim.x + threadIdx.x;
    if (g >= n) return;
    const int k0 = g ? cum_tiles_hit[g - 1] : 0, k1 = cum_tiles_hit[g];
    float a[9] = {0.f, 0.f, 0.f, 0.f, 0.f, 0.f, 0.f, 0.f, 0.f};
    float az = 0.f;
    float ax = 0.f, ay = 0.f;
    for (int k = k0; k < k1; ++k) {
        const float4 *row = reinterpret_cast<const float4 *>(grad_rows + (size_t)k * GSB_GRAD_ROW_FLOATS);
        const float4 r0 = row[0], r1 = row[1];
        a[0] += r0.x; a[1] += r0.y; a[2] += r0.z; a[3] += r0.w;
        a[4] += r1.x; a[5] += r1.y; a[6] += r1.z; a[7] += r1.w;
        if (ABS) {
            const float4 r2 = row[2];
            a[8] += r2.x;
            if (DEPTH) az += r2.y;
            ax += r2.z; ay += r2.w;
        } else {
            a[8] += reinterpret_cast<const float *>(row)[8];
            if (DEPTH) az += reinterpret_cast<const float *>(row)[9];
        }
    }
    const float S0 = a[0], Sx = a[1], Sy = a[2], Sxx = a[3], Sxy = a[4], Syy = a[5];
    const float ca = conics[3 * g], cb = conics[3 * g + 1], cc = conics[3 * g + 2];
    const float op = opacities[g];
    v_xy[g] = make_float2(-(ca * Sx + cb * Sy), -(cb * Sx + cc * Sy));
    v_conic[3 * g] = -0.5f * Sxx; v_conic[3 * g + 1] = -0.5f * Sxy; v_conic[3 * g + 2] = -0.5f * Syy;
    v_colors[3 * g] = a[6]; v_colors[3 * g + 1] = a[7]; v_colors[3 * g + 2] = a[8];
    v_opacity[g] = (op > 0.f) ? S0 / op : 0.f;
    if (DEPTH) v_depths[g] = az;
    if (ABS) v_xy_abs[g] = make_float2(ax, ay);
}

}

extern "C" size_t gsb_raster_grad_rows_bytes(int m) {
    return gsb_align_up((size_t)(m > 0 ? m : 0) * GSB_GRAD_ROW_FLOATS * 4 + 256, 256);
}

static int backward(int img_h, int img_w, int tiles_x, int tiles_y, int n, int m, const int32_t *tile_bins,
                    const int32_t *tile_order, const float *conics, const float *opacities, void *records,
                    const int32_t *cum_tiles_hit, const float *background, const float *final_Ts,
                    const int32_t *final_idx, const float *v_output, const float *v_output_alpha, void *grad_rows,
                    float *v_xy, float *v_conic, float *v_colors, float *v_opacity, unsigned flags, bool depth,
                    const float *record_depths, const float *v_output_depth, float *v_depths, float *v_xy_abs,
                    gsb_stream_t stream) {
    GSB_CHECK_ARG(img_h > 0 && img_w > 0 && n >= 0 && m >= 0);
    GSB_CHECK_ARG((flags & ~(unsigned)GSB_RASTER_CLAMP_MAX_ONE) == 0);
    const bool sat = (flags & GSB_RASTER_CLAMP_MAX_ONE) != 0;
    GSB_CHECK_ARG(tiles_x == gsb_div_up(img_w, GSB_TILE) && tiles_y == gsb_div_up(img_h, GSB_TILE));
    if (n == 0) return 0;
    GSB_CHECK_ARG(tile_bins && conics && opacities && cum_tiles_hit && background && final_Ts && final_idx &&
                  v_output && v_xy && v_conic && v_colors && v_opacity);
    GSB_CHECK_ARG(!depth || (v_depths && (record_depths || m == 0)));
    GSB_CHECK_ARG(((uintptr_t)v_xy % 8) == 0 && ((uintptr_t)v_xy_abs % 8) == 0);
    const bool abs = v_xy_abs != nullptr;
    cudaStream_t s = (cudaStream_t)stream;
    if (m > 0) {
        GSB_CHECK_ARG(records && grad_rows && ((uintptr_t)records % 16) == 0 && ((uintptr_t)grad_rows % 16) == 0);
        unsigned *counters = reinterpret_cast<unsigned *>(
            reinterpret_cast<char *>(records) + gsb_raster_records_bytes(m) - 256);
        GSB_CUDA(cudaMemsetAsync(counters, 0, 256, s));
        const int num_tiles = tiles_x * tiles_y;
#define GSB_BWD_LAUNCH(S, D, A)                                                                                 \
    rasterize_backward_kernel<S, D, A><<<gsb_blend_grid((const void *)rasterize_backward_kernel<S, D, A>,       \
                                                        num_tiles), RK_THREADS, 0, s>>>(                        \
        img_h, img_w, tiles_x, num_tiles, reinterpret_cast<const int2 *>(tile_bins),                            \
        reinterpret_cast<const GsbRecord *>(records), background, final_Ts, final_idx, v_output, v_output_alpha, \
        reinterpret_cast<float *>(grad_rows), counters, tile_order, record_depths, v_output_depth)
        if (abs) {
            if (depth) {
                if (sat) GSB_BWD_LAUNCH(true, true, true); else GSB_BWD_LAUNCH(false, true, true);
            } else {
                if (sat) GSB_BWD_LAUNCH(true, false, true); else GSB_BWD_LAUNCH(false, false, true);
            }
        } else if (depth) {
            if (sat) GSB_BWD_LAUNCH(true, true, false); else GSB_BWD_LAUNCH(false, true, false);
        } else {
            if (sat) GSB_BWD_LAUNCH(true, false, false); else GSB_BWD_LAUNCH(false, false, false);
        }
#undef GSB_BWD_LAUNCH
    }
#define GSB_REDUCE_LAUNCH(D, A)                                                                                 \
    reduce_grad_rows_kernel<D, A><<<gsb_div_up(n, 256), 256, 0, s>>>(                                           \
        n, cum_tiles_hit, reinterpret_cast<const float *>(grad_rows), conics, opacities,                        \
        reinterpret_cast<float2 *>(v_xy), v_conic, v_colors, v_opacity, v_depths,                               \
        reinterpret_cast<float2 *>(v_xy_abs))
    if (abs) {
        if (depth) GSB_REDUCE_LAUNCH(true, true); else GSB_REDUCE_LAUNCH(false, true);
    } else if (depth) {
        GSB_REDUCE_LAUNCH(true, false);
    } else {
        GSB_REDUCE_LAUNCH(false, false);
    }
#undef GSB_REDUCE_LAUNCH
    GSB_LAUNCH_CHECK();
    return 0;
}

extern "C" int gsb_rasterize_backward(int img_h, int img_w, int tiles_x, int tiles_y, int n, int m,
                                      const int32_t *tile_bins, const int32_t *tile_order, const float *conics,
                                      const float *opacities, void *records, const int32_t *cum_tiles_hit,
                                      const float *background, const float *final_Ts, const int32_t *final_idx,
                                      const float *v_output, const float *v_output_alpha, void *grad_rows,
                                      float *v_xy, float *v_conic, float *v_colors, float *v_opacity, unsigned flags,
                                      gsb_stream_t stream) {
    return backward(img_h, img_w, tiles_x, tiles_y, n, m, tile_bins, tile_order, conics, opacities, records,
                    cum_tiles_hit, background, final_Ts, final_idx, v_output, v_output_alpha, grad_rows, v_xy, v_conic,
                    v_colors, v_opacity, flags, false, nullptr, nullptr, nullptr, nullptr, stream);
}

extern "C" int gsb_rasterize_backward_depth(int img_h, int img_w, int tiles_x, int tiles_y, int n, int m,
                                            const int32_t *tile_bins, const int32_t *tile_order, const float *conics,
                                            const float *opacities, void *records, const int32_t *cum_tiles_hit,
                                            const float *background, const float *final_Ts, const int32_t *final_idx,
                                            const float *v_output, const float *v_output_alpha, void *grad_rows,
                                            float *v_xy, float *v_conic, float *v_colors, float *v_opacity,
                                            unsigned flags, const float *record_depths, const float *v_output_depth,
                                            float *v_depths, gsb_stream_t stream) {
    return backward(img_h, img_w, tiles_x, tiles_y, n, m, tile_bins, tile_order, conics, opacities, records,
                    cum_tiles_hit, background, final_Ts, final_idx, v_output, v_output_alpha, grad_rows, v_xy, v_conic,
                    v_colors, v_opacity, flags, true, record_depths, v_output_depth, v_depths, nullptr, stream);
}

extern "C" int gsb_rasterize_backward_absgrad(int img_h, int img_w, int tiles_x, int tiles_y, int n, int m,
                                              const int32_t *tile_bins, const int32_t *tile_order,
                                              const float *conics, const float *opacities, void *records,
                                              const int32_t *cum_tiles_hit, const float *background,
                                              const float *final_Ts, const int32_t *final_idx, const float *v_output,
                                              const float *v_output_alpha, void *grad_rows, float *v_xy,
                                              float *v_conic, float *v_colors, float *v_opacity, unsigned flags,
                                              const float *record_depths, const float *v_output_depth,
                                              float *v_depths, float *v_xy_abs, gsb_stream_t stream) {
    GSB_CHECK_ARG(v_xy_abs != nullptr);
    GSB_CHECK_ARG(v_depths || (!record_depths && !v_output_depth));
    return backward(img_h, img_w, tiles_x, tiles_y, n, m, tile_bins, tile_order, conics, opacities, records,
                    cum_tiles_hit, background, final_Ts, final_idx, v_output, v_output_alpha, grad_rows, v_xy, v_conic,
                    v_colors, v_opacity, flags, v_depths != nullptr, record_depths, v_output_depth, v_depths, v_xy_abs,
                    stream);
}
```

opensplat_b200/csrc/sh.cu:

```cuda
#include <type_traits>

#include "gsb_common.cuh"

int gsb_sm_count();

namespace {

constexpr int SH_THREADS = 128;

__host__ __device__ constexpr int sh_row_stride(int K) {
    int q = (3 * K + 3) / 4;
    return 4 * ((q & 1) ? q : q + 1);
}

template <bool ROUNDED_PRODUCTS = false>
__device__ __forceinline__ void sh_basis(int nb, float vx, float vy, float vz, float *Y) {
    Y[0] = 0.28209479177387814f;
    if (nb <= 1) return;
    float norm = sqrtf(vx * vx + vy * vy + vz * vz);
    float x = vx / norm, y = vy / norm, z = vz / norm;
    float xx, xy, xz, yy, yz, zz;
    if constexpr (ROUNDED_PRODUCTS) {
        xx = __fmul_rn(x, x); xy = __fmul_rn(x, y); xz = __fmul_rn(x, z);
        yy = __fmul_rn(y, y); yz = __fmul_rn(y, z); zz = __fmul_rn(z, z);
    } else {
        xx = x * x; xy = x * y; xz = x * z; yy = y * y; yz = y * z; zz = z * z;
    }
    Y[1] = -0.4886025119029199f * y;
    Y[2] = 0.4886025119029199f * z;
    Y[3] = -0.4886025119029199f * x;
    if (nb <= 4) return;
    Y[4] = 1.0925484305920792f * xy;
    Y[5] = -1.0925484305920792f * yz;
    Y[6] = 0.31539156525252005f * (2.f * zz - xx - yy);
    Y[7] = -1.0925484305920792f * xz;
    Y[8] = 0.5462742152960396f * (xx - yy);
    if (nb <= 9) return;
    Y[9] = -0.5900435899266435f * y * (3.f * xx - yy);
    Y[10] = 2.890611442640554f * xy * z;
    Y[11] = -0.4570457994644658f * y * (4.f * zz - xx - yy);
    Y[12] = 0.3731763325901154f * z * (2.f * zz - 3.f * xx - 3.f * yy);
    Y[13] = -0.4570457994644658f * x * (4.f * zz - xx - yy);
    Y[14] = 1.445305721320277f * z * (xx - yy);
    Y[15] = -0.5900435899266435f * x * (xx - 3.f * yy);
    if (nb <= 16) return;
    Y[16] = 2.5033429417967046f * xy * (xx - yy);
    Y[17] = -1.7701307697799304f * yz * (3.f * xx - yy);
    Y[18] = 0.9461746957575601f * xy * (7.f * zz - 1.f);
    Y[19] = -0.6690465435572892f * yz * (7.f * zz - 3.f);
    Y[20] = 0.10578554691520431f * (zz * (35.f * zz - 30.f) + 3.f);
    Y[21] = -0.6690465435572892f * xz * (7.f * zz - 3.f);
    Y[22] = 0.47308734787878004f * (xx - yy) * (7.f * zz - 1.f);
    Y[23] = -1.7701307697799304f * xz * (xx - 3.f * yy);
    Y[24] = 0.6258357354491761f * (xx * (xx - 3.f * yy) - yy * (3.f * xx - yy));
}

__device__ __forceinline__ int nb_of(int degrees_to_use) {
    return (degrees_to_use + 1) * (degrees_to_use + 1);
}

__device__ __forceinline__ float clamp_rgb(float s) { return s > 0.f ? s : (s == 0.f ? -0.f : 0.f); }
__device__ __forceinline__ bool rgb_grad_passes(float rgb) { return rgb > 0.f || (rgb == 0.f && signbit(rgb)); }

template <int K>
__global__ void __launch_bounds__(SH_THREADS)
sh_forward_kernel(int n, int degrees_to_use, const float *__restrict__ viewdirs,
                  const float *__restrict__ coeffs, float *__restrict__ colors, int vec_ok, int fuse_rgb,
                  float bias,
                  int split, const float *__restrict__ rest, const float *__restrict__ cam_pos) {
    constexpr int C = 3 * K;
    constexpr int S = sh_row_stride(K);
    __shared__ __align__(16) float tile[SH_THREADS * S];
    const int g0 = blockIdx.x * SH_THREADS;
    const int ng = min(SH_THREADS, n - g0);
    const int nb = min(nb_of(degrees_to_use), K);
    const float *src = coeffs + (size_t)g0 * C;
    const int total = ng * C;
    if (split) {
        const float *dc = coeffs + (size_t)g0 * 3, *rs = rest + (size_t)g0 * (C - 3);
        for (int e = threadIdx.x; e < ng * 3; e += SH_THREADS) tile[(e / 3) * S + (e % 3)] = __ldg(dc + e);
        if (C > 3)
            for (int e = threadIdx.x; e < ng * (C - 3); e += SH_THREADS) {
                const int g = e / (C - 3), j = e - g * (C - 3);
                tile[g * S + 3 + j] = __ldg(rs + e);
            }
    } else if (vec_ok && (C % 4 == 0)) {
        const float4 *src4 = reinterpret_cast<const float4 *>(src);
        for (int f = threadIdx.x; f < total / 4; f += SH_THREADS) {
            float4 v = ldg_stream4(src4 + f);
            int e = 4 * f, g = e / C, j = e - g * C;
            *reinterpret_cast<float4 *>(&tile[g * S + j]) = v;
        }
    } else {
        for (int e = threadIdx.x; e < total; e += SH_THREADS) {
            int g = e / C, j = e - g * C;
            tile[g * S + j] = __ldg(src + e);
        }
    }
    __syncthreads();
    const int t = threadIdx.x;
    if (t >= ng) return;
    const int g = g0 + t;
    float Y[K];
    {
        float vx = viewdirs[3 * g], vy = viewdirs[3 * g + 1], vz = viewdirs[3 * g + 2];
        if (cam_pos) { vx -= __ldg(cam_pos); vy -= __ldg(cam_pos + 1); vz -= __ldg(cam_pos + 2); }
        sh_basis(nb, vx, vy, vz, Y);
    }
    float row[S];
#pragma unroll
    for (int j = 0; j < S; j += 4) {
        float4 v = *reinterpret_cast<const float4 *>(&tile[t * S + j]);
        row[j] = v.x; row[j + 1] = v.y; row[j + 2] = v.z; row[j + 3] = v.w;
    }
    float c0 = 0.f, c1 = 0.f, c2 = 0.f;
#pragma unroll
    for (int b = 0; b < K; ++b) {
        if (b < nb) {
            c0 += Y[b] * row[3 * b];
            c1 += Y[b] * row[3 * b + 1];
            c2 += Y[b] * row[3 * b + 2];
        }
    }
    if (fuse_rgb) {
        c0 = clamp_rgb(c0 + bias);
        c1 = clamp_rgb(c1 + bias);
        c2 = clamp_rgb(c2 + bias);
    }
    colors[3 * g] = c0;
    colors[3 * g + 1] = c1;
    colors[3 * g + 2] = c2;
}

template <int K>
__global__ void __launch_bounds__(SH_THREADS)
sh_forward_multiview_kernel(int n, int degrees_to_use, const float *__restrict__ means, int num_views,
                            const float *__restrict__ cam_pos, const float *__restrict__ coeffs, float bias,
                            float *__restrict__ rgbs, int vec_ok) {
    constexpr int C = 3 * K;
    constexpr int S = sh_row_stride(K);
    __shared__ __align__(16) float tile[SH_THREADS * S];
    const int g0 = blockIdx.x * SH_THREADS;
    const int ng = min(SH_THREADS, n - g0);
    const int nb = min(nb_of(degrees_to_use), K);
    const float *src = coeffs + (size_t)g0 * C;
    const int total = ng * C;
    if (vec_ok && (C % 4 == 0)) {
        const float4 *src4 = reinterpret_cast<const float4 *>(src);
        for (int f = threadIdx.x; f < total / 4; f += SH_THREADS) {
            float4 v = ldg_stream4(src4 + f);
            int e = 4 * f, g = e / C, j = e - g * C;
            *reinterpret_cast<float4 *>(&tile[g * S + j]) = v;
        }
    } else {
        for (int e = threadIdx.x; e < total; e += SH_THREADS) {
            int g = e / C, j = e - g * C;
            tile[g * S + j] = __ldg(src + e);
        }
    }
    __syncthreads();
    const int t = threadIdx.x;
    if (t >= ng) return;
    const int g = g0 + t;
    const float mx = means[3 * g], my = means[3 * g + 1], mz = means[3 * g + 2];
    float row[S];
#pragma unroll
    for (int j = 0; j < S; j += 4) {
        float4 v = *reinterpret_cast<const float4 *>(&tile[t * S + j]);
        row[j] = v.x; row[j + 1] = v.y; row[j + 2] = v.z; row[j + 3] = v.w;
    }
    for (int view = 0; view < num_views; ++view) {
        float Y[K];
        {
            float vx = mx, vy = my, vz = mz;
            vx -= __ldg(cam_pos + 3 * view); vy -= __ldg(cam_pos + 3 * view + 1); vz -= __ldg(cam_pos + 3 * view + 2);
            sh_basis<(K >= 16)>(nb, vx, vy, vz, Y);
        }
        float c0 = 0.f, c1 = 0.f, c2 = 0.f;
#pragma unroll
        for (int b = 0; b < K; ++b) {
            if (b < nb) {
                c0 += Y[b] * row[3 * b];
                c1 += Y[b] * row[3 * b + 1];
                c2 += Y[b] * row[3 * b + 2];
            }
        }
        c0 = clamp_rgb(c0 + bias);
        c1 = clamp_rgb(c1 + bias);
        c2 = clamp_rgb(c2 + bias);
        float *out = rgbs + (size_t)view * 3 * n;
        out[3 * g] = c0;
        out[3 * g + 1] = c1;
        out[3 * g + 2] = c2;
    }
}

template <int K>
__global__ void __launch_bounds__(SH_THREADS)
sh_backward_kernel(int n, int degrees_to_use, const float *__restrict__ viewdirs,
                   const float *__restrict__ v_colors, float *__restrict__ v_coeffs, int vec_ok,
                   const float *__restrict__ rgb_mask,
                   int split, float *__restrict__ v_rest, const float *__restrict__ cam_pos) {
    constexpr int C = 3 * K;
    constexpr int S = sh_row_stride(K);
    __shared__ __align__(16) float tile[SH_THREADS * S];
    const int g0 = blockIdx.x * SH_THREADS;
    const int ng = min(SH_THREADS, n - g0);
    const int nb = min(nb_of(degrees_to_use), K);
    const int t = threadIdx.x;
    if (t < ng) {
        const int g = g0 + t;
        float Y[K];
        {
            float vx = viewdirs[3 * g], vy = viewdirs[3 * g + 1], vz = viewdirs[3 * g + 2];
            if (cam_pos) { vx -= __ldg(cam_pos); vy -= __ldg(cam_pos + 1); vz -= __ldg(cam_pos + 2); }
            sh_basis(nb, vx, vy, vz, Y);
        }
        float v0 = v_colors[3 * g], v1 = v_colors[3 * g + 1], v2 = v_colors[3 * g + 2];
        if (rgb_mask) {
            v0 = rgb_grad_passes(rgb_mask[3 * g]) ? v0 : 0.f;
            v1 = rgb_grad_passes(rgb_mask[3 * g + 1]) ? v1 : 0.f;
            v2 = rgb_grad_passes(rgb_mask[3 * g + 2]) ? v2 : 0.f;
        }
        float row[S];
#pragma unroll
        for (int b = 0; b < K; ++b) {
            float yb = (b < nb) ? Y[b] : 0.f;
            row[3 * b] = yb * v0;
            row[3 * b + 1] = yb * v1;
            row[3 * b + 2] = yb * v2;
        }
#pragma unroll
        for (int j = C; j < S; ++j) row[j] = 0.f;
#pragma unroll
        for (int j = 0; j < S; j += 4)
            *reinterpret_cast<float4 *>(&tile[t * S + j]) = make_float4(row[j], row[j + 1], row[j + 2], row[j + 3]);
    }
    __syncthreads();
    float *dst = v_coeffs + (size_t)g0 * C;
    const int total = ng * C;
    if (split) {
        float *dc = v_coeffs + (size_t)g0 * 3, *rs = v_rest + (size_t)g0 * (C - 3);
        for (int e = threadIdx.x; e < ng * 3; e += SH_THREADS) dc[e] = tile[(e / 3) * S + (e % 3)];
        if (C > 3)
            for (int e = threadIdx.x; e < ng * (C - 3); e += SH_THREADS) {
                const int g = e / (C - 3), j = e - g * (C - 3);
                rs[e] = tile[g * S + 3 + j];
            }
    } else if (vec_ok && (C % 4 == 0)) {
        float4 *dst4 = reinterpret_cast<float4 *>(dst);
        for (int f = threadIdx.x; f < total / 4; f += SH_THREADS) {
            int e = 4 * f, g = e / C, j = e - g * C;
            stg_stream4(dst4 + f, *reinterpret_cast<const float4 *>(&tile[g * S + j]));
        }
    } else {
        for (int e = threadIdx.x; e < total; e += SH_THREADS) {
            int g = e / C, j = e - g * C;
            dst[e] = tile[g * S + j];
        }
    }
}

template <bool PEER_CAMS>
using MvCamPos = typename std::conditional<PEER_CAMS, const float *const *, const float *>::type;

__device__ __forceinline__ float4 multimem_ld_reduce_add(const float *mc_ptr) {
    float4 v;
    asm volatile("multimem.ld_reduce.relaxed.sys.global.add.v4.f32 {%0,%1,%2,%3}, [%4];"
                 : "=f"(v.x), "=f"(v.y), "=f"(v.z), "=f"(v.w) : "l"(mc_ptr) : "memory");
    return v;
}
__device__ __forceinline__ void multimem_st(float *mc_ptr, float4 v) {
    asm volatile("multimem.st.relaxed.sys.global.v4.f32 [%0], {%1,%2,%3,%4};"
                 :: "l"(mc_ptr), "f"(v.x), "f"(v.y), "f"(v.z), "f"(v.w) : "memory");
}

constexpr int MV_MAX_RANKS = 16;

template <int K, bool PEER_CAMS>
__global__ void __launch_bounds__(SH_THREADS)
sh_backward_multiview_kernel(int n, int degrees_to_use, const float *__restrict__ means, int num_views,
                             MvCamPos<PEER_CAMS> __restrict__ cam_pos, const float *const *__restrict__ v_rgb_views,
                             float scale, float *__restrict__ v_coeffs, int vec_ok,
                             int geom_blocks, int rank, int world, long long geom_vec4,
                             float *const *__restrict__ geom_ranks, float *geom_mc) {
    constexpr int C = 3 * K;
    constexpr int S = sh_row_stride(K);
    constexpr int VB = (K > 16) ? 4 : 8;
    if ((int)blockIdx.x < geom_blocks) {
        const long long chunk = (geom_vec4 + world - 1) / world;
        const long long lo = chunk * rank, hi = min(geom_vec4, lo + chunk);
        const long long stride = (long long)geom_blocks * SH_THREADS;
        if (geom_mc != nullptr) {
            constexpr int GU = 4;
            for (long long i0 = lo + (long long)blockIdx.x * SH_THREADS + threadIdx.x; i0 < hi; i0 += GU * stride) {
                float4 v[GU];
#pragma unroll
                for (int u = 0; u < GU; ++u)
                    if (i0 + u * stride < hi) v[u] = multimem_ld_reduce_add(geom_mc + 4 * (i0 + u * stride));
#pragma unroll
                for (int u = 0; u < GU; ++u)
                    if (i0 + u * stride < hi) {
                        v[u].x *= scale; v[u].y *= scale; v[u].z *= scale; v[u].w *= scale;
                        multimem_st(geom_mc + 4 * (i0 + u * stride), v[u]);
                    }
            }
        } else {
            for (long long i = lo + (long long)blockIdx.x * SH_THREADS + threadIdx.x; i < hi; i += stride) {
                float4 acc = make_float4(0.f, 0.f, 0.f, 0.f);
                float4 part[MV_MAX_RANKS];
#pragma unroll
                for (int r = 0; r < MV_MAX_RANKS; ++r)
                    if (r < world) part[r] = *(reinterpret_cast<const float4 *>(geom_ranks[r]) + i);
#pragma unroll
                for (int r = 0; r < MV_MAX_RANKS; ++r)
                    if (r < world) { acc.x += part[r].x; acc.y += part[r].y; acc.z += part[r].z; acc.w += part[r].w; }
                acc.x *= scale; acc.y *= scale; acc.z *= scale; acc.w *= scale;
#pragma unroll
                for (int r = 0; r < MV_MAX_RANKS; ++r)
                    if (r < world) *(reinterpret_cast<float4 *>(geom_ranks[r]) + i) = acc;
            }
        }
        return;
    }
    __shared__ __align__(16) float tile[SH_THREADS * S];
    __shared__ float stage[VB][3 * SH_THREADS];
    __shared__ float cam_stage[3 * VB];
    const int blk = (int)blockIdx.x - geom_blocks;
    const int g0 = blk * SH_THREADS;
    const int ng = min(SH_THREADS, n - g0);
    const int nb = min(nb_of(degrees_to_use), K);
    const int t = threadIdx.x;
    const int g = g0 + t;
    float mx = 0.f, my = 0.f, mz = 0.f;
    if (t < ng) { mx = means[3 * g]; my = means[3 * g + 1]; mz = means[3 * g + 2]; }
    float row[S];
#pragma unroll
    for (int j = 0; j < S; ++j) row[j] = 0.f;
    const int span = 3 * ng;
    for (int r0 = 0; r0 < num_views; r0 += VB) {
        float pull[VB][3];
#pragma unroll
        for (int u = 0; u < VB; ++u) {
            pull[u][0] = pull[u][1] = pull[u][2] = 0.f;
            if (r0 + u < num_views) {
                const float *vr = v_rgb_views[r0 + u] + (size_t)3 * g0;
#pragma unroll
                for (int q = 0; q < 3; ++q)
                    if (t + q * SH_THREADS < span) pull[u][q] = vr[t + q * SH_THREADS];
            }
        }
        float cam_pull = 0.f;
        if constexpr (PEER_CAMS) {
            if (t < 3 * VB && r0 + t / 3 < num_views) cam_pull = cam_pos[r0 + t / 3][t % 3];
        }
        __syncthreads();
#pragma unroll
        for (int u = 0; u < VB; ++u)
#pragma unroll
            for (int q = 0; q < 3; ++q) stage[u][t + q * SH_THREADS] = pull[u][q];
        if constexpr (PEER_CAMS) {
            if (t < 3 * VB) cam_stage[t] = cam_pull;
        }
        __syncthreads();
        float cam_x[VB], cam_y[VB], cam_z[VB];
        if constexpr (PEER_CAMS) {
#pragma unroll
            for (int u = 0; u < VB; ++u) {
                cam_x[u] = cam_stage[3 * u]; cam_y[u] = cam_stage[3 * u + 1]; cam_z[u] = cam_stage[3 * u + 2];
            }
        }
        if (t < ng) {
#pragma unroll
            for (int u = 0; u < VB; ++u) {
                if (r0 + u >= num_views) break;
                const float v0 = stage[u][3 * t], v1 = stage[u][3 * t + 1], v2 = stage[u][3 * t + 2];
                if (v0 == 0.f && v1 == 0.f && v2 == 0.f) continue;
                const int r = r0 + u;
                float Y[K];
                if constexpr (PEER_CAMS)
                    sh_basis(nb, mx - cam_x[u], my - cam_y[u], mz - cam_z[u], Y);
                else
                    sh_basis(nb, mx - __ldg(cam_pos + 3 * r), my - __ldg(cam_pos + 3 * r + 1),
                             mz - __ldg(cam_pos + 3 * r + 2), Y);
#pragma unroll
                for (int b = 0; b < K; ++b) {
                    if (b < nb) {
                        row[3 * b] = fmaf(Y[b], v0, row[3 * b]);
                        row[3 * b + 1] = fmaf(Y[b], v1, row[3 * b + 1]);
                        row[3 * b + 2] = fmaf(Y[b], v2, row[3 * b + 2]);
                    }
                }
            }
        }
    }
    if (t < ng) {
#pragma unroll
        for (int j = 0; j < S; j += 4)
            *reinterpret_cast<float4 *>(&tile[t * S + j]) =
                make_float4(scale * row[j], scale * row[j + 1], scale * row[j + 2], scale * row[j + 3]);
    }
    __syncthreads();
    float *dst = v_coeffs + (size_t)g0 * C;
    const int total = ng * C;
    if (vec_ok && (C % 4 == 0)) {
        float4 *dst4 = reinterpret_cast<float4 *>(dst);
        for (int f = threadIdx.x; f < total / 4; f += SH_THREADS) {
            int e = 4 * f, gg = e / C, j = e - gg * C;
            stg_stream4(dst4 + f, *reinterpret_cast<const float4 *>(&tile[gg * S + j]));
        }
    } else {
        for (int e = threadIdx.x; e < total; e += SH_THREADS) {
            int gg = e / C, j = e - gg * C;
            dst[e] = tile[gg * S + j];
        }
    }
}

__global__ void __launch_bounds__(256)
mask_rgb_grad_kernel(long long n3, const float *__restrict__ rgbs, float *__restrict__ v_rgbs) {
    const long long i = (long long)blockIdx.x * blockDim.x + threadIdx.x;
    if (i < n3 && !rgb_grad_passes(rgbs[i])) v_rgbs[i] = 0.f;
}

int bases_of_degree(int degree) {
    switch (degree) {
        case 0: return 1;
        case 1: return 4;
        case 2: return 9;
        case 3: return 16;
        case 4: return 25;
        default: return -1;
    }
}

}

static int launch_sh_forward(int n, int degree, int degrees_to_use, const float *viewdirs, const float *coeffs,
                             float *colors, int fuse_rgb, float bias, gsb_stream_t stream, int split = 0,
                             const float *rest = nullptr, const float *cam_pos = nullptr) {
    GSB_CHECK_ARG(n >= 0 && bases_of_degree(degree) > 0 && degrees_to_use >= 0 && degrees_to_use <= degree);
    if (n == 0) return 0;
    GSB_CHECK_ARG(viewdirs && coeffs && colors);
    cudaStream_t s = (cudaStream_t)stream;
    int grid = gsb_div_up(n, SH_THREADS);
    int vec_ok = ((uintptr_t)coeffs % 16) == 0;
#define GSB_SH_F(K) sh_forward_kernel<K><<<grid, SH_THREADS, 0, s>>>(n, degrees_to_use, viewdirs, coeffs, colors, vec_ok, fuse_rgb, bias, split, rest, cam_pos)
    switch (degree) {
        case 0: GSB_SH_F(1); break;
        case 1: GSB_SH_F(4); break;
        case 2: GSB_SH_F(9); break;
        case 3: GSB_SH_F(16); break;
        default: GSB_SH_F(25); break;
    }
#undef GSB_SH_F
    GSB_LAUNCH_CHECK();
    return 0;
}

static int launch_sh_backward(int n, int degree, int degrees_to_use, const float *viewdirs, const float *v_colors,
                              float *v_coeffs, const float *rgb_mask, gsb_stream_t stream, int split = 0,
                              float *v_rest = nullptr, const float *cam_pos = nullptr) {
    GSB_CHECK_ARG(n >= 0 && bases_of_degree(degree) > 0 && degrees_to_use >= 0 && degrees_to_use <= degree);
    if (n == 0) return 0;
    GSB_CHECK_ARG(viewdirs && v_colors && v_coeffs);
    cudaStream_t s = (cudaStream_t)stream;
    int grid = gsb_div_up(n, SH_THREADS);
    int vec_ok = ((uintptr_t)v_coeffs % 16) == 0;
#define GSB_SH_B(K) sh_backward_kernel<K><<<grid, SH_THREADS, 0, s>>>(n, degrees_to_use, viewdirs, v_colors, v_coeffs, vec_ok, rgb_mask, split, v_rest, cam_pos)
    switch (degree) {
        case 0: GSB_SH_B(1); break;
        case 1: GSB_SH_B(4); break;
        case 2: GSB_SH_B(9); break;
        case 3: GSB_SH_B(16); break;
        default: GSB_SH_B(25); break;
    }
#undef GSB_SH_B
    GSB_LAUNCH_CHECK();
    return 0;
}

extern "C" int gsb_sh_forward(int n, int degree, int degrees_to_use, const float *viewdirs,
                              const float *coeffs, float *colors, gsb_stream_t stream) {
    return launch_sh_forward(n, degree, degrees_to_use, viewdirs, coeffs, colors, 0, 0.f, stream);
}

extern "C" int gsb_sh_backward(int n, int degree, int degrees_to_use, const float *viewdirs,
                               const float *v_colors, float *v_coeffs, gsb_stream_t stream) {
    return launch_sh_backward(n, degree, degrees_to_use, viewdirs, v_colors, v_coeffs, nullptr, stream);
}

extern "C" int gsb_sh_forward_rgb(int n, int degree, int degrees_to_use, const float *viewdirs,
                                  const float *coeffs, float bias, float *rgbs, gsb_stream_t stream) {
    return launch_sh_forward(n, degree, degrees_to_use, viewdirs, coeffs, rgbs, 1, bias, stream);
}

extern "C" int gsb_sh_backward_rgb(int n, int degree, int degrees_to_use, const float *viewdirs,
                                   const float *rgbs, const float *v_rgbs, float *v_coeffs,
                                   gsb_stream_t stream) {
    GSB_CHECK_ARG(n == 0 || rgbs);
    return launch_sh_backward(n, degree, degrees_to_use, viewdirs, v_rgbs, v_coeffs, rgbs, stream);
}

extern "C" int gsb_sh_forward_split(int n, int degree, int degrees_to_use, const float *means, const float *cam_pos,
                                    const float *features_dc, const float *features_rest, float bias, float *rgbs,
                                    gsb_stream_t stream) {
    GSB_CHECK_ARG(n == 0 || (cam_pos && features_dc && (degree == 0 || features_rest)));
    return launch_sh_forward(n, degree, degrees_to_use, means, features_dc, rgbs, 1, bias, stream, 1, features_rest,
                             cam_pos);
}

extern "C" int gsb_sh_backward_split(int n, int degree, int degrees_to_use, const float *means, const float *cam_pos,
                                     const float *rgbs, const float *v_rgbs, float *v_features_dc,
                                     float *v_features_rest, gsb_stream_t stream) {
    GSB_CHECK_ARG(n == 0 || (cam_pos && rgbs && v_features_dc && (degree == 0 || v_features_rest)));
    return launch_sh_backward(n, degree, degrees_to_use, means, v_rgbs, v_features_dc, rgbs, stream, 1,
                              v_features_rest, cam_pos);
}

extern "C" int gsb_sh_forward_rgb_cam(int n, int degree, int degrees_to_use, const float *means, const float *cam_pos,
                                      const float *coeffs, float bias, float *rgbs, gsb_stream_t stream) {
    GSB_CHECK_ARG(n == 0 || cam_pos);
    return launch_sh_forward(n, degree, degrees_to_use, means, coeffs, rgbs, 1, bias, stream, 0, nullptr, cam_pos);
}

extern "C" int gsb_sh_backward_rgb_cam(int n, int degree, int degrees_to_use, const float *means,
                                       const float *cam_pos, const float *rgbs, const float *v_rgbs, float *v_coeffs,
                                       gsb_stream_t stream) {
    GSB_CHECK_ARG(n == 0 || (cam_pos && rgbs));
    return launch_sh_backward(n, degree, degrees_to_use, means, v_rgbs, v_coeffs, rgbs, stream, 0, nullptr, cam_pos);
}

extern "C" int gsb_sh_forward_rgb_cam_multiview(int n, int degree, int degrees_to_use, const float *means,
                                                int num_views, const float *cam_positions, const float *coeffs,
                                                float bias, float *rgbs, gsb_stream_t stream) {
    GSB_CHECK_ARG(n >= 0 && num_views >= 1 && bases_of_degree(degree) > 0 && degrees_to_use >= 0 &&
                  degrees_to_use <= degree);
    if (n == 0) return 0;
    GSB_CHECK_ARG(means && cam_positions && coeffs && rgbs);
    cudaStream_t s = (cudaStream_t)stream;
    int grid = gsb_div_up(n, SH_THREADS);
    int vec_ok = ((uintptr_t)coeffs % 16) == 0;
#define GSB_SH_FM(K) sh_forward_multiview_kernel<K><<<grid, SH_THREADS, 0, s>>>(n, degrees_to_use, means, num_views, cam_positions, coeffs, bias, rgbs, vec_ok)
    switch (degree) {
        case 0: GSB_SH_FM(1); break;
        case 1: GSB_SH_FM(4); break;
        case 2: GSB_SH_FM(9); break;
        case 3: GSB_SH_FM(16); break;
        default: GSB_SH_FM(25); break;
    }
#undef GSB_SH_FM
    GSB_LAUNCH_CHECK();
    return 0;
}

extern "C" int gsb_mask_rgb_grad(int n, const float *rgbs, float *v_rgbs, gsb_stream_t stream) {
    GSB_CHECK_ARG(n >= 0);
    if (n == 0) return 0;
    GSB_CHECK_ARG(rgbs && v_rgbs);
    const long long n3 = 3ll * n;
    mask_rgb_grad_kernel<<<(unsigned)((n3 + 255) / 256), 256, 0, (cudaStream_t)stream>>>(n3, rgbs, v_rgbs);
    GSB_LAUNCH_CHECK();
    return 0;
}

template <bool PEER_CAMS>
static int launch_multiview(int n, int degree, int degrees_to_use, const float *means, int num_views,
                            MvCamPos<PEER_CAMS> cam_positions, const float *const *v_rgbs_per_view, float scale,
                            float *v_coeffs, int rank, int world, long long geom_floats, float *const *geom_per_rank,
                            float *geom_multicast, gsb_stream_t stream) {
    GSB_CHECK_ARG(n >= 0 && bases_of_degree(degree) > 0 && degrees_to_use >= 0 && degrees_to_use <= degree);
    GSB_CHECK_ARG(num_views >= 1 && geom_floats >= 0);
    int geom_blocks = 0;
    if (geom_floats > 0) {
        GSB_CHECK_ARG(world >= 1 && rank >= 0 && rank < world && (geom_floats % 4) == 0);
        GSB_CHECK_ARG(geom_multicast || (geom_per_rank && world <= MV_MAX_RANKS));
        GSB_CHECK_ARG(((uintptr_t)geom_multicast % 16) == 0);
        const int sms = gsb_sm_count();
        const long long slice = (geom_floats / 4 + world - 1) / world;
        const long long want = (slice + 2 * 4 * SH_THREADS - 1) / (2 * 4 * SH_THREADS);
        geom_blocks = (int)(want < sms ? sms : (want > 8LL * sms ? 8LL * sms : want));
    }
    if (n == 0 && geom_blocks == 0) return 0;
    GSB_CHECK_ARG(n == 0 || (means && cam_positions && v_rgbs_per_view && v_coeffs));
    cudaStream_t s = (cudaStream_t)stream;
    int grid = geom_blocks + gsb_div_up(n, SH_THREADS);
    int vec_ok = ((uintptr_t)v_coeffs % 16) == 0;
#define GSB_SH_M(K) sh_backward_multiview_kernel<K, PEER_CAMS><<<grid, SH_THREADS, 0, s>>>(n, degrees_to_use, means, num_views, cam_positions, v_rgbs_per_view, scale, v_coeffs, vec_ok, geom_blocks, rank, world, geom_floats / 4, geom_per_rank, geom_multicast)
    switch (degree) {
        case 0: GSB_SH_M(1); break;
        case 1: GSB_SH_M(4); break;
        case 2: GSB_SH_M(9); break;
        case 3: GSB_SH_M(16); break;
        default: GSB_SH_M(25); break;
    }
#undef GSB_SH_M
    GSB_LAUNCH_CHECK();
    return 0;
}

extern "C" int gsb_sh_backward_multiview(int n, int degree, int degrees_to_use, const float *means,
                                         int num_views, const float *cam_positions,
                                         const float *const *v_rgbs_per_view, float scale, float *v_coeffs,
                                         gsb_stream_t stream) {
    return launch_multiview<false>(n, degree, degrees_to_use, means, num_views, cam_positions, v_rgbs_per_view,
                                   scale, v_coeffs, 0, 1, 0, nullptr, nullptr, stream);
}

extern "C" int gsb_exchange_gradients(int n, int degree, int degrees_to_use, const float *means, int num_views,
                                      const float *cam_positions, const float *const *v_rgbs_per_view, float scale,
                                      float *v_coeffs, int rank, int world, long long geom_floats,
                                      float *const *geom_per_rank, float *geom_multicast, gsb_stream_t stream) {
    return launch_multiview<false>(n, degree, degrees_to_use, means, num_views, cam_positions, v_rgbs_per_view,
                                   scale, v_coeffs, rank, world, geom_floats, geom_per_rank, geom_multicast, stream);
}

extern "C" int gsb_sh_backward_multiview_cams(int n, int degree, int degrees_to_use, const float *means,
                                              int num_views, const float *const *cam_pos_per_view,
                                              const float *const *v_rgbs_per_view, float scale, float *v_coeffs,
                                              gsb_stream_t stream) {
    return launch_multiview<true>(n, degree, degrees_to_use, means, num_views, cam_pos_per_view, v_rgbs_per_view,
                                  scale, v_coeffs, 0, 1, 0, nullptr, nullptr, stream);
}

extern "C" int gsb_exchange_gradients_cams(int n, int degree, int degrees_to_use, const float *means, int num_views,
                                           const float *const *cam_pos_per_view,
                                           const float *const *v_rgbs_per_view, float scale, float *v_coeffs,
                                           int rank, int world, long long geom_floats, float *const *geom_per_rank,
                                           float *geom_multicast, gsb_stream_t stream) {
    return launch_multiview<true>(n, degree, degrees_to_use, means, num_views, cam_pos_per_view, v_rgbs_per_view,
                                  scale, v_coeffs, rank, world, geom_floats, geom_per_rank, geom_multicast, stream);
}
```

opensplat_b200/pipeline.py:

```python
import os

import torch

from . import capi
from .ops import tile_bounds, num_sh_bases, BinFrame, BinPlan
from .parallel import flat_layout


class SplatPipeline(BinFrame):

    def __init__(self, n, W, H, sh_degree=3, device="cuda:0", m_capacity=None, stage_timing=False):
        super().__init__(BinPlan(), device)
        self.n, self.deg = int(n), int(sh_degree)
        self.K = num_sh_bases(sh_degree)
        d, f32 = self.dev, torch.float32
        self._alloc_gaussians(self.n)
        self._alloc_pixels(W, H)
        self.background = torch.zeros(3, dtype=f32, device=d)
        self.loss = torch.zeros(1, dtype=f32, device=d)
        self.viewmat = torch.eye(4, dtype=f32, device=d)
        self.projmat = torch.eye(4, dtype=f32, device=d)
        self.intr = (1.0, 1.0, 0.0, 0.0)
        if m_capacity:
            self.plan.grow(int(m_capacity), 0)
        self.nvtx = os.environ.get("GSB_NVTX", "0") == "1"
        self._nvtx_open = False
        self.exchange = None
        self.stage_timing = stage_timing
        self.stage_ms = {}
        self._steps_ev = []

    def _alloc_gaussians(self, n):
        self.n = n = int(n)
        d, f32, i32 = self.dev, torch.float32, torch.int32
        self.offs, self.numel = flat_layout(n, self.K)
        self.sizes = [(name, shp) for name, (o, c, shp) in self.offs.items()]
        self.geom_numel = self.offs["coeffs"][0]
        self.param_flat = torch.zeros(self.numel, dtype=f32, device=d)
        self.grad_flat = self._alloc_grad_flat(self.numel)
        self.p, self.g = {}, {}
        for name, (o, c, shp) in self.offs.items():
            self.p[name] = self.param_flat[o:o + c].view(shp)
            self.g[name] = self.grad_flat[o:o + c].view(shp)
        self.adam_m = self.adam_v = None
        self.adam_t = 0
        self.viewdirs = torch.zeros((n, 3), dtype=f32, device=d)
        self.colors = torch.empty((n, 3), dtype=f32, device=d)
        self.rgbs = torch.empty((n, 3), dtype=f32, device=d)
        self.cov3d = torch.empty((n, 6), dtype=f32, device=d)
        self.xys = torch.empty((n, 2), dtype=f32, device=d)
        self.depths = torch.empty((n,), dtype=f32, device=d)
        self.radii = torch.empty((n,), dtype=i32, device=d)
        self.conics = torch.empty((n, 3), dtype=f32, device=d)
        self.nth = torch.empty((n,), dtype=i32, device=d)
        self.v_xy = torch.empty((n, 2), dtype=f32, device=d)
        self.v_conic = torch.empty((n, 3), dtype=f32, device=d)
        self.v_rgbs = torch.empty((n, 3), dtype=f32, device=d)
        self.max_len = 0
        self.m_cap = -1

    def _alloc_pixels(self, W, H):
        self.W, self.H = int(W), int(H)
        self.tb = tile_bounds(self.W, self.H)
        self.T = self.tb[0] * self.tb[1]
        d, f32, i32 = self.dev, torch.float32, torch.int32
        H, W = self.H, self.W
        self.out_img = torch.empty((H, W, 3), dtype=f32, device=d)
        self.final_Ts = torch.empty((H, W), dtype=f32, device=d)
        self.final_idx = torch.empty((H, W), dtype=i32, device=d)
        self.v_img = torch.empty((H, W, 3), dtype=f32, device=d)
        self.target = torch.zeros((H, W, 3), dtype=f32, device=d)
        self.m_cap = -1

    def _alloc_grad_flat(self, numel):
        return torch.zeros(numel, dtype=torch.float32, device=self.dev)

    def rebind_grad_flat(self, flat):
        assert flat.numel() == self.numel and flat.dtype == torch.float32
        self.grad_flat = flat
        for name, (o, c, shp) in self.offs.items():
            self.g[name] = self.grad_flat[o:o + c].view(shp)

    def _grow(self, m_cap, n, T):
        super()._grow(m_cap, n, T)
        self.grad_rows = torch.empty(self.L.gsb_raster_grad_rows_bytes(m_cap), dtype=torch.uint8, device=self.dev)

    def load_scene(self, sc):
        for k in ("means", "scales", "quats", "opacities", "coeffs"):
            self.p[k].copy_(torch.from_numpy(sc[k]).to(self.dev))
        self.viewdirs.copy_(torch.from_numpy(sc["viewdirs"]).to(self.dev))
        self.set_camera(sc)

    def set_camera(self, cam):
        self.viewmat.copy_(torch.as_tensor(cam["viewmat"]).to(self.dev))
        self.projmat.copy_(torch.as_tensor(cam["projmat"]).to(self.dev))
        self.intr = (float(cam["fx"]), float(cam["fy"]), float(cam["cx"]), float(cam["cy"]))

    def _stage(self, name):
        if self.nvtx:
            if self._nvtx_open:
                torch.cuda.nvtx.range_pop()
            self._nvtx_open = not name.startswith("end_")
            if self._nvtx_open:
                torch.cuda.nvtx.range_push("gsb:" + name)
        if self.stage_timing:
            e = torch.cuda.Event(enable_timing=True)
            e.record()
            self._ev.append((name, e))

    def _collect(self):
        if self.stage_timing and len(self._ev) >= 2:
            self._steps_ev.append(self._ev)
        self._ev = []

    def resolve_stage_times(self):
        torch.cuda.synchronize()
        for ev in self._steps_ev:
            for (n0, e0), (_, e1) in zip(ev[:-1], ev[1:]):
                self.stage_ms.setdefault(n0, []).append(e0.elapsed_time(e1))
        self._steps_ev = []
        return {k: sum(v) / len(v) for k, v in self.stage_ms.items() if not k.startswith("end_")}

    def forward(self):
        L, P, s = self.L, capi.ptr, capi.stream()
        n, W, H = self.n, self.W, self.H
        fx, fy, cx, cy = self.intr
        p = self.p
        self._stage("sh_fwd")
        capi.check(L.gsb_sh_forward_rgb(n, self.deg, self.deg, P(self.viewdirs), P(p["coeffs"]), 0.5, P(self.rgbs), s))
        self._stage("project_fwd")
        capi.check(L.gsb_project_forward(n, P(p["means"]), P(p["scales"]), 1.0, P(p["quats"]), P(self.viewmat),
                                         P(self.projmat), fx, fy, cx, cy, H, W, self.tb[0], self.tb[1], 0.01,
                                         P(self.cov3d), P(self.xys), P(self.depths), P(self.radii), P(self.conics),
                                         P(self.nth), s))
        return self._bin_blend(p["opacities"], 0)

    def _bin_blend(self, opacities, flags, count_visible=False, rgbs=None, out_img=None, out_depth=None,
                   out_alpha=None, depth_values=None):
        return self.bin_blend(self.xys, self.radii, self.conics, self.depths, self.nth,
                              self.rgbs if rgbs is None else rgbs, opacities, self.background,
                              self.out_img if out_img is None else out_img, self.final_Ts, self.final_idx, flags,
                              count_visible, out_depth=out_depth, out_alpha=out_alpha, depth_values=depth_values)

    def _raster_backward(self, opacities, v_opacities, v_rgbs, flags, v_xy_abs=None):
        P = capi.ptr
        if v_xy_abs is not None:
            capi.check(self.L.gsb_rasterize_backward_absgrad(
                self.H, self.W, self.tb[0], self.tb[1], self.n, self.m_raster, P(self.tile_bins),
                P(self.tile_order) if self._ordered else None, P(self.conics), P(opacities), P(self.records),
                P(self.cum), P(self.background), P(self.final_Ts), P(self.final_idx), P(self.v_img), None,
                P(self.grad_rows), P(self.v_xy), P(self.v_conic), P(v_rgbs), P(v_opacities), flags, None, None, None,
                P(v_xy_abs), capi.stream()))
            return
        capi.check(self.L.gsb_rasterize_backward(
            self.H, self.W, self.tb[0], self.tb[1], self.n, self.m_raster, P(self.tile_bins),
            P(self.tile_order) if self._ordered else None, P(self.conics), P(opacities), P(self.records), P(self.cum),
            P(self.background), P(self.final_Ts), P(self.final_idx), P(self.v_img), None, P(self.grad_rows),
            P(self.v_xy), P(self.v_conic), P(v_rgbs), P(v_opacities), flags, capi.stream()))

    def _raster_backward_depth(self, opacities, v_opacities, v_rgbs, flags, v_output_depth, v_depths, v_xy_abs=None):
        P = capi.ptr
        args = (self.H, self.W, self.tb[0], self.tb[1], self.n, self.m_raster, P(self.tile_bins),
                P(self.tile_order) if self._ordered else None, P(self.conics), P(opacities), P(self.records),
                P(self.cum), P(self.background), P(self.final_Ts), P(self.final_idx), P(self.v_img), None,
                P(self.grad_rows), P(self.v_xy), P(self.v_conic), P(v_rgbs), P(v_opacities), flags,
                P(self.record_depths), P(v_output_depth), P(v_depths))
        if v_xy_abs is not None:
            capi.check(self.L.gsb_rasterize_backward_absgrad(*args, P(v_xy_abs), capi.stream()))
        else:
            capi.check(self.L.gsb_rasterize_backward_depth(*args, capi.stream()))

    def backward(self):
        L, P, s = self.L, capi.ptr, capi.stream()
        n, W, H = self.n, self.W, self.H
        fx, fy, cx, cy = self.intr
        p, g = self.p, self.g
        cnt = H * W * 3
        self._stage("loss")
        capi.check(L.gsb_mse_loss_grad(cnt, P(self.out_img), P(self.target), P(self.v_img), P(self.loss), 1.0 / cnt, s))
        v_rgbs = self.exchange.v_rgbs_buffer() if self.exchange is not None else self.v_rgbs
        self._stage("raster_bwd")
        self._raster_backward(p["opacities"], g["opacities"], v_rgbs, 0)
        if self.exchange is not None and self.exchange.overlap:
            self.exchange.start_colour(average=True)
        self._stage("project_bwd")
        capi.check(L.gsb_project_backward(n, P(p["means"]), P(p["scales"]), 1.0, P(p["quats"]), P(self.viewmat),
                                          P(self.projmat), fx, fy, cx, cy, H, W, None, P(self.radii), P(self.conics),
                                          P(self.v_xy), None, P(self.v_conic), P(g["means"]), P(g["scales"]),
                                          P(g["quats"]), s))
        self._stage("sh_bwd")
        if self.exchange is not None:
            if self.exchange.overlap:
                self.exchange.finish()
            else:
                self.exchange.exchange(average=True)
        else:
            capi.check(L.gsb_sh_backward_rgb(n, self.deg, self.deg, P(self.viewdirs), P(self.rgbs), P(self.v_rgbs),
                                             P(g["coeffs"]), s))
        self._stage("end_bwd")
        return self.loss

    def forward_backward(self):
        self.forward()
        loss = self.backward()
        self._collect()
        return loss

    def adam_step(self, lr=1e-3, b1=0.9, b2=0.999, eps=1e-8):
        if self.adam_m is None:
            self.adam_m = torch.zeros_like(self.param_flat)
            self.adam_v = torch.zeros_like(self.param_flat)
        self.adam_t += 1
        t = self.adam_t
        capi.check(self.L.gsb_adam_step(self.numel, capi.ptr(self.param_flat), capi.ptr(self.grad_flat),
                                        capi.ptr(self.adam_m), capi.ptr(self.adam_v), lr, b1, b2, eps,
                                        1.0 - b1 ** t, 1.0 - b2 ** t, capi.stream()))

    def train_step(self, world_size=1, lr=1e-3):
        self.forward()
        loss = self.backward()
        if world_size > 1 and self.exchange is None:
            import torch.distributed as dist
            dist.all_reduce(self.grad_flat, op=dist.ReduceOp.SUM)
            self.grad_flat.mul_(1.0 / world_size)
        self.adam_step(lr=lr)
        self._collect()
        return loss

    def resize_gaussians(self, params, adam_m=None, adam_v=None):
        t = self.adam_t
        self._alloc_gaussians(params["means"].shape[0])
        self.adam_t = t
        for k in self.p:
            self.p[k].copy_(params[k].view(self.p[k].shape))
        if adam_m is not None and adam_v is not None:
            self.adam_m = torch.zeros_like(self.param_flat)
            self.adam_v = torch.zeros_like(self.param_flat)
            for name, (o, c, shp) in self.offs.items():
                self.adam_m[o:o + c].copy_(adam_m[name].reshape(-1))
                self.adam_v[o:o + c].copy_(adam_v[name].reshape(-1))
        if self.exchange is not None:
            self.exchange.resize(self)

    def tile_occupancy(self, nbins=16):
        tb = self.tile_bins.cpu().numpy()
        lens = (tb[:, 1] - tb[:, 0]).astype("int64")
        import numpy as np
        mx = int(lens.max()) if lens.size else 0
        edges = np.linspace(0, max(mx, 1), nbins + 1)
        hist, _ = np.histogram(lens, bins=edges)
        q = np.percentile(lens, [50, 90, 99]) if lens.size else [0, 0, 0]
        return {"tiles": int(lens.size), "empty_tiles": int((lens == 0).sum()), "mean": float(lens.mean()),
                "p50": float(q[0]), "p90": float(q[1]), "p99": float(q[2]), "max": mx,
                "hist_edges": [round(float(e), 1) for e in edges], "hist": [int(h) for h in hist]}

    def algorithmic_bytes(self):
        n, m, P, T, K = self.n, self.m, self.W * self.H, self.T, self.K
        tile_bits = max(1, (T - 1).bit_length())
        passes = (32 + tile_bits + 7) // 8
        stages = {
            "sh_fwd": n * (12 + 12 * K + 12),
            "project_fwd": 96 * n,
            "scan": 8 * n,
            "emit": 20 * n + 12 * m,
            "sort": 8 * m + passes * 24 * m,
            "bins": 8 * m + 8 * T,
            "raster_fwd": 40 * m + 20 * P,
            "raster_bwd": 40 * m + 20 * P + 36 * n,
            "project_bwd": 144 * n,
            "sh_bwd": n * (12 + 12 * K + 12),
        }
        return stages, passes
```

Baseline: 1091.

## Fuse grad-row reduction, projection VJP and SH backward into one per-Gaussian kernel

Raster backward now only writes per-intersection gradient rows. A new per-Gaussian tail kernel sums each Gaussian's rows, computes the blend gradients, runs the projection VJP and writes SH coefficient gradients in a single launch. This drops the intermediate v_xy/v_conic/v_rgb round trips through global memory and two kernel launches. In exchange the fused kernel carries more registers and may lose occupancy. Per-Gaussian row summation can also be imbalanced when some Gaussians hit many tiles.

```diff
diff --git a/include/gsplat_b200.h b/include/gsplat_b200.h
--- a/include/gsplat_b200.h
+++ b/include/gsplat_b200.h
@@ -156,6 +156,16 @@
                            const int32_t *final_idx, const float *v_output, const float *v_output_alpha,
                            void *grad_rows, float *v_xy, float *v_conic, float *v_colors, float *v_opacity,
                            unsigned flags, gsb_stream_t stream);
+int gsb_rasterize_backward_rows(int img_h, int img_w, int tiles_x, int tiles_y, int n, int m, const int32_t *tile_bins,
+                                const int32_t *tile_order, void *records, const float *background,
+                                const float *final_Ts, const int32_t *final_idx, const float *v_output,
+                                const float *v_output_alpha, void *grad_rows, unsigned flags, gsb_stream_t stream);
+int gsb_grad_tail(int n, int degree, int degrees_to_use, const int32_t *cum_tiles_hit, const void *grad_rows,
+                  const float *means3d, const float *scales, float glob_scale, const float *quats,
+                  const float *opacities, const float *viewmat, const float *projmat, float fx, float fy, int img_h,
+                  int img_w, const int32_t *radii, const float *conics, const float *viewdirs, const float *rgbs,
+                  float *v_opacity, float *v_mean3d, float *v_scale, float *v_quat, float *v_coeffs,
+                  gsb_stream_t stream);
 int gsb_gather_record_depths(int m, const int32_t *gaussian_ids_sorted, const float *depths, const int32_t *bin_stats,
                              float *record_depths, gsb_stream_t stream);
 int gsb_rasterize_forward_packed_depth(int img_h, int img_w, int tiles_x, int tiles_y, int m, const int32_t *tile_bins,
diff --git a/opensplat_b200/capi.py b/opensplat_b200/capi.py
--- a/opensplat_b200/capi.py
+++ b/opensplat_b200/capi.py
@@ -56,6 +56,10 @@
     "gsb_rasterize_forward_count": (_i, [_i, _i, _i, _i, _i, _vp, _vp, _vp, _vp, _vp, _vp, _vp, _vp]),
     "gsb_rasterize_backward": (_i, [_i, _i, _i, _i, _i, _i, _vp, _vp, _vp, _vp, _vp, _vp, _vp, _vp, _vp, _vp,
                                     _vp, _vp, _vp, _vp, _vp, _vp, C.c_uint, _vp]),
+    "gsb_rasterize_backward_rows": (_i, [_i, _i, _i, _i, _i, _i, _vp, _vp, _vp, _vp, _vp, _vp, _vp, _vp, _vp,
+                                         C.c_uint, _vp]),
+    "gsb_grad_tail": (_i, [_i, _i, _i, _vp, _vp, _vp, _vp, _f, _vp, _vp, _vp, _vp, _f, _f, _i, _i, _vp, _vp, _vp,
+                           _vp, _vp, _vp, _vp, _vp, _vp, _vp]),
     "gsb_gather_record_depths": (_i, [_i, _vp, _vp, _vp, _vp, _vp]),
     "gsb_rasterize_forward_packed_depth": (_i, [_i, _i, _i, _i, _i, _vp, _vp, _vp, _vp, _vp, _vp, _vp, _vp, C.c_uint,
                                                 _vp, _vp, _vp, _vp]),
diff --git a/opensplat_b200/csrc/per_gaussian.cuh b/opensplat_b200/csrc/per_gaussian.cuh
--- /dev/null
+++ b/opensplat_b200/csrc/per_gaussian.cuh
@@ -0,0 +1,284 @@
+#pragma once
+#include "raster_common.cuh"
+
+namespace gsb {
+
+__device__ __forceinline__ float mul(float a, float b) { return __fmul_rn(a, b); }
+__device__ __forceinline__ float add(float a, float b) { return __fadd_rn(a, b); }
+__device__ __forceinline__ float sub(float a, float b) { return __fsub_rn(a, b); }
+__device__ __forceinline__ float twice(float x) { return add(x, x); }
+__device__ __forceinline__ float dot2(float a0, float b0, float a1, float b1) { return add(mul(a0, b0), mul(a1, b1)); }
+__device__ __forceinline__ float dot3(float a0, float b0, float a1, float b1, float a2, float b2) {
+    return add(dot2(a0, b0, a1, b1), mul(a2, b2));
+}
+__device__ __forceinline__ float dot4(float a0, float b0, float a1, float b1, float a2, float b2, float a3, float b3) {
+    return add(dot3(a0, b0, a1, b1, a2, b2), mul(a3, b3));
+}
+
+struct GradRowSums {
+    float a[9];
+    float az, ax, ay;
+};
+
+template <bool DEPTH, bool ABS>
+__device__ __forceinline__ GradRowSums sum_grad_rows(const float *__restrict__ grad_rows, int k0, int k1) {
+    GradRowSums s = {{0.f, 0.f, 0.f, 0.f, 0.f, 0.f, 0.f, 0.f, 0.f}, 0.f, 0.f, 0.f};
+    for (int k = k0; k < k1; ++k) {
+        const float4 *row = reinterpret_cast<const float4 *>(grad_rows + (size_t)k * GSB_GRAD_ROW_FLOATS);
+        const float4 r0 = row[0], r1 = row[1];
+        s.a[0] += r0.x; s.a[1] += r0.y; s.a[2] += r0.z; s.a[3] += r0.w;
+        s.a[4] += r1.x; s.a[5] += r1.y; s.a[6] += r1.z; s.a[7] += r1.w;
+        if (ABS) {
+            const float4 r2 = row[2];
+            s.a[8] += r2.x;
+            if (DEPTH) s.az += r2.y;
+            s.ax += r2.z; s.ay += r2.w;
+        } else {
+            s.a[8] += reinterpret_cast<const float *>(row)[8];
+            if (DEPTH) s.az += reinterpret_cast<const float *>(row)[9];
+        }
+    }
+    return s;
+}
+
+struct BlendGrads {
+    float2 v_xy;
+    float v_conic[3], v_rgb[3], v_opacity;
+};
+
+__device__ __forceinline__ BlendGrads blend_grads(const GradRowSums &s, float ca, float cb, float cc, float op) {
+    BlendGrads g;
+    const float S0 = s.a[0], Sx = s.a[1], Sy = s.a[2];
+    g.v_xy = make_float2(-__fmaf_rn(ca, Sx, mul(cb, Sy)), -__fmaf_rn(cb, Sx, mul(cc, Sy)));
+    g.v_conic[0] = mul(-0.5f, s.a[3]); g.v_conic[1] = mul(-0.5f, s.a[4]); g.v_conic[2] = mul(-0.5f, s.a[5]);
+    g.v_rgb[0] = s.a[6]; g.v_rgb[1] = s.a[7]; g.v_rgb[2] = s.a[8];
+    g.v_opacity = (op > 0.f) ? S0 / op : 0.f;
+    return g;
+}
+
+constexpr int CG_TERMS = 24;
+
+struct Cam {
+    float V[12];
+    float P[16];
+};
+
+__device__ __forceinline__ void load_cam(const float *__restrict__ viewmat, const float *__restrict__ projmat, Cam &c) {
+#pragma unroll
+    for (int i = 0; i < 12; ++i) c.V[i] = __ldg(viewmat + i);
+#pragma unroll
+    for (int i = 0; i < 16; ++i) c.P[i] = __ldg(projmat + i);
+}
+
+__device__ __forceinline__ void quat_to_rotmat(float qw, float qx, float qy, float qz, float R[3][3]) {
+    float s = 1.0f / sqrtf(dot4(qw, qw, qx, qx, qy, qy, qz, qz));
+    float w = mul(qw, s), x = mul(qx, s), y = mul(qy, s), z = mul(qz, s);
+    R[0][0] = sub(1.f, twice(dot2(y, y, z, z)));
+    R[0][1] = twice(sub(mul(x, y), mul(w, z)));
+    R[0][2] = twice(dot2(x, z, w, y));
+    R[1][0] = twice(dot2(x, y, w, z));
+    R[1][1] = sub(1.f, twice(dot2(x, x, z, z)));
+    R[1][2] = twice(sub(mul(y, z), mul(w, x)));
+    R[2][0] = twice(sub(mul(x, z), mul(w, y)));
+    R[2][1] = twice(dot2(y, z, w, x));
+    R[2][2] = sub(1.f, twice(dot2(x, x, y, y)));
+}
+
+__device__ __forceinline__ void filter3d_scales(float glob_scale, const float (&e)[3], float f, float (&sig)[3],
+                                                float (&r)[3], float &c3) {
+    const float ff = mul(f, f);
+#pragma unroll
+    for (int k = 0; k < 3; ++k) {
+        const float s = mul(glob_scale, e[k]);
+        sig[k] = sqrtf(add(mul(s, s), ff));
+        r[k] = s / sig[k];
+    }
+    c3 = mul(mul(r[0], r[1]), r[2]);
+}
+
+struct ProjVjpIn {
+    float px, py, pz;
+    float4 q;
+    float a[3];
+    float A, B, Cc;
+    float2 v_xy;
+    float v_depth;
+    float v_conic[3];
+    float opacity, v_opacity, f3;
+    bool has_v_opacity;
+};
+
+template <bool ACT, bool AA, bool CAMGRAD, bool F3D>
+__device__ __forceinline__ void project_vjp(const Cam &cam, const ProjVjpIn &in, float glob_scale, float fx, float fy,
+                                            float tan_fovx, float tan_fovy, int img_h, int img_w, float (&vm)[3],
+                                            float (&vs)[3], float4 &vq, float &comp, float (&fr)[3], float &fc3,
+                                            float (&fsh)[3], float (&cg)[CG_TERMS]) {
+    const float *V = cam.V, *P = cam.P;
+    const float px = in.px, py = in.py, pz = in.pz;
+
+    const float hx = add(dot3(P[0], px, P[1], py, P[2], pz), P[3]);
+    const float hy = add(dot3(P[4], px, P[5], py, P[6], pz), P[7]);
+    const float hw = add(dot3(P[12], px, P[13], py, P[14], pz), P[15]);
+    const float rw = 1.f / add(hw, 1e-6f);
+    const float2 vxy = in.v_xy;
+    const float vndcx = mul(mul(0.5f, (float)img_w), vxy.x), vndcy = mul(mul(0.5f, (float)img_h), vxy.y);
+    const float vhx = mul(vndcx, rw), vhy = mul(vndcy, rw);
+    const float vhw = mul(mul(-dot2(vndcx, hx, vndcy, hy), rw), rw);
+    vm[0] = dot3(P[0], vhx, P[4], vhy, P[12], vhw);
+    vm[1] = dot3(P[1], vhx, P[5], vhy, P[13], vhw);
+    vm[2] = dot3(P[2], vhx, P[6], vhy, P[14], vhw);
+
+    const float tx = add(dot3(V[0], px, V[1], py, V[2], pz), V[3]);
+    const float ty = add(dot3(V[4], px, V[5], py, V[6], pz), V[7]);
+    const float tz = add(dot3(V[8], px, V[9], py, V[10], pz), V[11]);
+    float vtx = 0.f, vty = 0.f, vtz = in.v_depth;
+
+    const float A = in.A, B = in.B, Cc = in.Cc;
+    const float gA = in.v_conic[0], gB = mul(0.5f, in.v_conic[1]), gC = in.v_conic[2];
+    const float xg00 = dot2(A, gA, B, gB), xg01 = dot2(A, gB, B, gC);
+    const float xg10 = dot2(B, gA, Cc, gB), xg11 = dot2(B, gB, Cc, gC);
+    float vS00 = -dot2(xg00, A, xg01, B);
+    float vS01 = -dot2(xg00, B, xg01, Cc);
+    float vS11 = -dot2(xg10, B, xg11, Cc);
+
+    const float4 q = in.q;
+    float R[3][3], M[3][3];
+    quat_to_rotmat(q.x, q.y, q.z, q.w, R);
+    const float e[3] = {ACT ? expf(in.a[0]) : in.a[0], ACT ? expf(in.a[1]) : in.a[1], ACT ? expf(in.a[2]) : in.a[2]};
+    float s[3] = {mul(glob_scale, e[0]), mul(glob_scale, e[1]), mul(glob_scale, e[2])};
+    if constexpr (F3D) filter3d_scales(glob_scale, e, in.f3, s, fr, fc3);
+#pragma unroll
+    for (int r = 0; r < 3; ++r)
+#pragma unroll
+        for (int c = 0; c < 3; ++c) M[r][c] = mul(R[r][c], s[c]);
+    float Cs[3][3];
+#pragma unroll
+    for (int r = 0; r < 3; ++r)
+#pragma unroll
+        for (int c = 0; c < 3; ++c) Cs[r][c] = dot3(M[r][0], M[c][0], M[r][1], M[c][1], M[r][2], M[c][2]);
+    const float lim_x = mul(1.3f, tan_fovx), lim_y = mul(1.3f, tan_fovy);
+    const float qx = tx / tz, qy = ty / tz;
+    const bool clamp_x = !(qx > -lim_x && qx < lim_x), clamp_y = !(qy > -lim_y && qy < lim_y);
+    const float cqx = fminf(lim_x, fmaxf(-lim_x, qx)), cqy = fminf(lim_y, fmaxf(-lim_y, qy));
+    const float ttx = mul(tz, cqx), tty = mul(tz, cqy);
+    const float rz = 1.f / tz, rz2 = mul(rz, rz), rz3 = mul(rz2, rz);
+    const float J00 = mul(fx, rz), J02 = mul(mul(-fx, ttx), rz2), J11 = mul(fy, rz), J12 = mul(mul(-fy, tty), rz2);
+    float T[2][3];
+#pragma unroll
+    for (int c = 0; c < 3; ++c) {
+        T[0][c] = dot2(J00, V[c], J02, V[8 + c]);
+        T[1][c] = dot2(J11, V[4 + c], J12, V[8 + c]);
+    }
+    if constexpr (AA) {
+        float TV[2][3];
+#pragma unroll
+        for (int r = 0; r < 2; ++r)
+#pragma unroll
+            for (int c = 0; c < 3; ++c) TV[r][c] = dot3(T[r][0], Cs[0][c], T[r][1], Cs[1][c], T[r][2], Cs[2][c]);
+        const float cxx0 = dot3(TV[0][0], T[0][0], TV[0][1], T[0][1], TV[0][2], T[0][2]);
+        const float cxy = dot3(TV[0][0], T[1][0], TV[0][1], T[1][1], TV[0][2], T[1][2]);
+        const float cyy0 = dot3(TV[1][0], T[1][0], TV[1][1], T[1][1], TV[1][2], T[1][2]);
+        const float det = sub(mul(add(cxx0, 0.3f), add(cyy0, 0.3f)), mul(cxy, cxy));
+        comp = sqrtf(fmaxf(0.f, sub(mul(cxx0, cyy0), mul(cxy, cxy)) / det));
+        if (in.has_v_opacity && comp > 0.f) {
+            const float o = 1.f / add(1.f, expf(-in.opacity));
+            const float k = mul(0.5f, mul(in.v_opacity, F3D ? mul(o, fc3) : o)) / comp;
+            const float id = 1.f / det;
+            const float a = mul(cyy0, id), b = mul(cxy, id), c = mul(cxx0, id), ee = mul(0.3f, id);
+            vS00 = add(vS00, mul(k, mul(0.3f, dot3(a, a, b, b, ee, a))));
+            vS01 = sub(vS01, mul(k, mul(0.3f, mul(b, add(add(a, c), ee)))));
+            vS11 = add(vS11, mul(k, mul(0.3f, dot3(c, c, b, b, ee, c))));
+        }
+    }
+    float vST[2][3];
+#pragma unroll
+    for (int c = 0; c < 3; ++c) {
+        vST[0][c] = dot2(vS00, T[0][c], vS01, T[1][c]);
+        vST[1][c] = dot2(vS01, T[0][c], vS11, T[1][c]);
+    }
+    float vV[3][3];
+#pragma unroll
+    for (int r = 0; r < 3; ++r)
+#pragma unroll
+        for (int c = 0; c < 3; ++c) vV[r][c] = dot2(T[0][r], vST[0][c], T[1][r], vST[1][c]);
+    float vT[2][3];
+#pragma unroll
+    for (int r = 0; r < 2; ++r)
+#pragma unroll
+        for (int c = 0; c < 3; ++c)
+            vT[r][c] = twice(dot3(vST[r][0], Cs[0][c], vST[r][1], Cs[1][c], vST[r][2], Cs[2][c]));
+    const float vJ00 = dot3(vT[0][0], V[0], vT[0][1], V[1], vT[0][2], V[2]);
+    const float vJ02 = dot3(vT[0][0], V[8], vT[0][1], V[9], vT[0][2], V[10]);
+    const float vJ11 = dot3(vT[1][0], V[4], vT[1][1], V[5], vT[1][2], V[6]);
+    const float vJ12 = dot3(vT[1][0], V[8], vT[1][1], V[9], vT[1][2], V[10]);
+    const float vttx = mul(mul(-fx, rz2), vJ02), vtty = mul(mul(-fy, rz2), vJ12);
+    vtz = add(vtz, add(sub(add(mul(mul(-fx, rz2), vJ00), mul(mul(mul(twice(fx), ttx), rz3), vJ02)),
+                           mul(mul(fy, rz2), vJ11)),
+                       mul(mul(mul(twice(fy), tty), rz3), vJ12)));
+    if (qx == lim_x || qx == -lim_x) { const float h = mul(0.5f, vttx); vtx = add(vtx, h); vtz = add(vtz, mul(cqx, h)); }
+    else if (clamp_x) vtz = add(vtz, mul(cqx, vttx)); else vtx = add(vtx, vttx);
+    if (qy == lim_y || qy == -lim_y) { const float h = mul(0.5f, vtty); vty = add(vty, h); vtz = add(vtz, mul(cqy, h)); }
+    else if (clamp_y) vtz = add(vtz, mul(cqy, vtty)); else vty = add(vty, vtty);
+    vm[0] = add(vm[0], dot3(V[0], vtx, V[4], vty, V[8], vtz));
+    vm[1] = add(vm[1], dot3(V[1], vtx, V[5], vty, V[9], vtz));
+    vm[2] = add(vm[2], dot3(V[2], vtx, V[6], vty, V[10], vtz));
+    if constexpr (CAMGRAD) {
+        const float pc[3] = {px, py, pz}, vt[3] = {vtx, vty, vtz}, vh[3] = {vhx, vhy, vhw};
+#pragma unroll
+        for (int r = 0; r < 3; ++r) {
+#pragma unroll
+            for (int c = 0; c < 3; ++c) {
+                cg[4 * r + c] = mul(vt[r], pc[c]);
+                cg[12 + 4 * r + c] = mul(vh[r], pc[c]);
+            }
+            cg[4 * r + 3] = vt[r];
+            cg[12 + 4 * r + 3] = vh[r];
+        }
+#pragma unroll
+        for (int c = 0; c < 3; ++c) {
+            cg[c] = add(cg[c], mul(J00, vT[0][c]));
+            cg[4 + c] = add(cg[4 + c], mul(J11, vT[1][c]));
+            cg[8 + c] = add(cg[8 + c], dot2(J02, vT[0][c], J12, vT[1][c]));
+        }
+    }
+
+    float vM[3][3];
+#pragma unroll
+    for (int r = 0; r < 3; ++r)
+#pragma unroll
+        for (int c = 0; c < 3; ++c) vM[r][c] = twice(dot3(vV[r][0], M[0][c], vV[r][1], M[1][c], vV[r][2], M[2][c]));
+#pragma unroll
+    for (int c = 0; c < 3; ++c) {
+        vs[c] = mul(glob_scale, dot3(R[0][c], vM[0][c], R[1][c], vM[1][c], R[2][c], vM[2][c]));
+        if (ACT) vs[c] = mul(vs[c], e[c]);
+        if (F3D) vs[c] = mul(vs[c], fr[c]);
+    }
+    float vR[3][3];
+#pragma unroll
+    for (int r = 0; r < 3; ++r)
+#pragma unroll
+        for (int c = 0; c < 3; ++c) vR[r][c] = mul(vM[r][c], s[c]);
+    const float nq = sqrtf(dot4(q.x, q.x, q.y, q.y, q.z, q.z, q.w, q.w));
+    const float inv = 1.0f / nq;
+    const float w = mul(q.x, inv), x = mul(q.y, inv), y = mul(q.z, inv), z = mul(q.w, inv);
+    const float gw = twice(add(add(mul(x, sub(vR[2][1], vR[1][2])), mul(y, sub(vR[0][2], vR[2][0]))),
+                                  mul(z, sub(vR[1][0], vR[0][1]))));
+    const float gx = twice(add(add(add(mul(-twice(x), add(vR[1][1], vR[2][2])), mul(y, add(vR[1][0], vR[0][1]))),
+                                      mul(z, add(vR[2][0], vR[0][2]))),
+                                  mul(w, sub(vR[2][1], vR[1][2]))));
+    const float gy = twice(add(add(sub(mul(x, add(vR[1][0], vR[0][1])), mul(twice(y), add(vR[0][0], vR[2][2]))),
+                                      mul(z, add(vR[2][1], vR[1][2]))),
+                                  mul(w, sub(vR[0][2], vR[2][0]))));
+    const float gz = twice(add(sub(add(mul(x, add(vR[2][0], vR[0][2])), mul(y, add(vR[2][1], vR[1][2]))),
+                                      mul(twice(z), add(vR[0][0], vR[1][1]))),
+                                  mul(w, sub(vR[1][0], vR[0][1]))));
+    const float dot = dot4(w, gw, x, gx, y, gy, z, gz);
+    vq = make_float4(mul(sub(gw, mul(w, dot)), inv), mul(sub(gx, mul(x, dot)), inv), mul(sub(gy, mul(y, dot)), inv),
+                     mul(sub(gz, mul(z, dot)), inv));
+    if constexpr (F3D) {
+#pragma unroll
+        for (int k = 0; k < 3; ++k) { const float t = in.f3 / s[k]; fsh[k] = mul(t, t); }
+    }
+}
+
+}
diff --git a/opensplat_b200/csrc/project.cu b/opensplat_b200/csrc/project.cu
--- a/opensplat_b200/csrc/project.cu
+++ b/opensplat_b200/csrc/project.cu
@@ -1,9 +1,14 @@
-#include "gsb_common.cuh"
+#include "per_gaussian.cuh"
 
 namespace {
 
+using gsb::CG_TERMS;
+using gsb::Cam;
+using gsb::filter3d_scales;
+using gsb::load_cam;
+using gsb::quat_to_rotmat;
+
 constexpr int PJ_THREADS = 256;
-constexpr int CG_TERMS = 24;
 
 __device__ __forceinline__ void camgrad_block_sum(const float (&cg)[CG_TERMS], float *__restrict__ out) {
     __shared__ float red[PJ_THREADS / 32][CG_TERMS];
@@ -22,45 +27,6 @@
         for (int w = 1; w < PJ_THREADS / 32; ++w) v = v + red[w][threadIdx.x];
         out[threadIdx.x] = v;
     }
-}
-
-struct Cam {
-    float V[12];
-    float P[16];
-};
-
-__device__ __forceinline__ void quat_to_rotmat(float qw, float qx, float qy, float qz, float R[3][3]) {
-    float s = 1.0f / sqrtf(qw * qw + qx * qx + qy * qy + qz * qz);
-    float w = qw * s, x = qx * s, y = qy * s, z = qz * s;
-    R[0][0] = 1.f - 2.f * (y * y + z * z);
-    R[0][1] = 2.f * (x * y - w * z);
-    R[0][2] = 2.f * (x * z + w * y);
-    R[1][0] = 2.f * (x * y + w * z);
-    R[1][1] = 1.f - 2.f * (x * x + z * z);
-    R[1][2] = 2.f * (y * z - w * x);
-    R[2][0] = 2.f * (x * z - w * y);
-    R[2][1] = 2.f * (y * z + w * x);
-    R[2][2] = 1.f - 2.f * (x * x + y * y);
-}
-
-__device__ __forceinline__ void load_cam(const float *__restrict__ viewmat,
-                                         const float *__restrict__ projmat, Cam &c) {
-#pragma unroll
-    for (int i = 0; i < 12; ++i) c.V[i] = __ldg(viewmat + i);
-#pragma unroll
-    for (int i = 0; i < 16; ++i) c.P[i] = __ldg(projmat + i);
-}
-
-__device__ __forceinline__ void filter3d_scales(float glob_scale, const float (&e)[3], float f, float (&sig)[3],
-                                                float (&r)[3], float &c3) {
-    const float ff = f * f;
-#pragma unroll
-    for (int k = 0; k < 3; ++k) {
-        const float s = glob_scale * e[k];
-        sig[k] = sqrtf(s * s + ff);
-        r[k] = s / sig[k];
-    }
-    c3 = r[0] * r[1] * r[2];
 }
 
 template <bool ACT, bool AA = false, bool F3D = false>
@@ -229,171 +195,20 @@
         if (radii[i] > 0) {
             Cam cam;
             load_cam(viewmat, projmat, cam);
-            const float *V = cam.V, *P = cam.P;
-            const float px = means3d[3 * i], py = means3d[3 * i + 1], pz = means3d[3 * i + 2];
-
-            const float hx = P[0] * px + P[1] * py + P[2] * pz + P[3];
-            const float hy = P[4] * px + P[5] * py + P[6] * pz + P[7];
-            const float hw = P[12] * px + P[13] * py + P[14] * pz + P[15];
-            const float rw = 1.f / (hw + 1e-6f);
-            const float2 vxy = v_xy[i];
-            const float vndcx = 0.5f * (float)img_w * vxy.x, vndcy = 0.5f * (float)img_h * vxy.y;
-            const float vhx = vndcx * rw, vhy = vndcy * rw;
-            const float vhw = -(vndcx * hx + vndcy * hy) * rw * rw;
-            vm[0] = P[0] * vhx + P[4] * vhy + P[12] * vhw;
-            vm[1] = P[1] * vhx + P[5] * vhy + P[13] * vhw;
-            vm[2] = P[2] * vhx + P[6] * vhy + P[14] * vhw;
-
-            const float tx = V[0] * px + V[1] * py + V[2] * pz + V[3];
-            const float ty = V[4] * px + V[5] * py + V[6] * pz + V[7];
-            const float tz = V[8] * px + V[9] * py + V[10] * pz + V[11];
-            float vtx = 0.f, vty = 0.f, vtz = v_depth ? v_depth[i] : 0.f;
-
-            const float A = conics[3 * i], B = conics[3 * i + 1], Cc = conics[3 * i + 2];
-            const float gA = v_conic[3 * i], gB = 0.5f * v_conic[3 * i + 1], gC = v_conic[3 * i + 2];
-            const float xg00 = A * gA + B * gB, xg01 = A * gB + B * gC;
-            const float xg10 = B * gA + Cc * gB, xg11 = B * gB + Cc * gC;
-            float vS00 = -(xg00 * A + xg01 * B);
-            float vS01 = -(xg00 * B + xg01 * Cc);
-            float vS11 = -(xg10 * B + xg11 * Cc);
-
-            const float4 q = reinterpret_cast<const float4 *>(quats)[i];
-            float R[3][3], M[3][3];
-            quat_to_rotmat(q.x, q.y, q.z, q.w, R);
-            const float a[3] = {scales[3 * i], scales[3 * i + 1], scales[3 * i + 2]};
-            const float e[3] = {ACT ? expf(a[0]) : a[0], ACT ? expf(a[1]) : a[1], ACT ? expf(a[2]) : a[2]};
-            float s[3] = {glob_scale * e[0], glob_scale * e[1], glob_scale * e[2]};
-            if constexpr (F3D) filter3d_scales(glob_scale, e, f3, s, fr, fc3);
-#pragma unroll
-            for (int r = 0; r < 3; ++r)
-#pragma unroll
-                for (int c = 0; c < 3; ++c) M[r][c] = R[r][c] * s[c];
-            float Cs[3][3];
-#pragma unroll
-            for (int r = 0; r < 3; ++r)
-#pragma unroll
-                for (int c = 0; c < 3; ++c)
-                    Cs[r][c] = M[r][0] * M[c][0] + M[r][1] * M[c][1] + M[r][2] * M[c][2];
-            const float lim_x = 1.3f * tan_fovx, lim_y = 1.3f * tan_fovy;
-            const float qx = tx / tz, qy = ty / tz;
-            const bool clamp_x = !(qx > -lim_x && qx < lim_x), clamp_y = !(qy > -lim_y && qy < lim_y);
-            const float cqx = fminf(lim_x, fmaxf(-lim_x, qx)), cqy = fminf(lim_y, fmaxf(-lim_y, qy));
-            const float ttx = tz * cqx, tty = tz * cqy;
-            const float rz = 1.f / tz, rz2 = rz * rz, rz3 = rz2 * rz;
-            const float J00 = fx * rz, J02 = -fx * ttx * rz2, J11 = fy * rz, J12 = -fy * tty * rz2;
-            float T[2][3];
-#pragma unroll
-            for (int c = 0; c < 3; ++c) {
-                T[0][c] = J00 * V[c] + J02 * V[8 + c];
-                T[1][c] = J11 * V[4 + c] + J12 * V[8 + c];
-            }
-            if constexpr (AA) {
-                float TV[2][3];
-#pragma unroll
-                for (int r = 0; r < 2; ++r)
-#pragma unroll
-                    for (int c = 0; c < 3; ++c)
-                        TV[r][c] = T[r][0] * Cs[0][c] + T[r][1] * Cs[1][c] + T[r][2] * Cs[2][c];
-                const float cxx0 = TV[0][0] * T[0][0] + TV[0][1] * T[0][1] + TV[0][2] * T[0][2];
-                const float cxy = TV[0][0] * T[1][0] + TV[0][1] * T[1][1] + TV[0][2] * T[1][2];
-                const float cyy0 = TV[1][0] * T[1][0] + TV[1][1] * T[1][1] + TV[1][2] * T[1][2];
-                const float det = (cxx0 + 0.3f) * (cyy0 + 0.3f) - cxy * cxy;
-                comp = sqrtf(fmaxf(0.f, (cxx0 * cyy0 - cxy * cxy) / det));
-                if (v_opacity && comp > 0.f) {
-                    const float o = 1.f / (1.f + expf(-opacities[i]));
-                    const float k = 0.5f * (v_opacity[i] * (F3D ? o * fc3 : o)) / comp;
-                    const float id = 1.f / det;
-                    const float a = cyy0 * id, b = cxy * id, c = cxx0 * id, e = 0.3f * id;
-                    vS00 = vS00 + k * (0.3f * (a * a + b * b + e * a));
-                    vS01 = vS01 - k * (0.3f * (b * (a + c + e)));
-                    vS11 = vS11 + k * (0.3f * (c * c + b * b + e * c));
-                }
-            }
-            float vST[2][3];
-#pragma unroll
-            for (int c = 0; c < 3; ++c) {
-                vST[0][c] = vS00 * T[0][c] + vS01 * T[1][c];
-                vST[1][c] = vS01 * T[0][c] + vS11 * T[1][c];
-            }
-            float vV[3][3];
-#pragma unroll
-            for (int r = 0; r < 3; ++r)
-#pragma unroll
-                for (int c = 0; c < 3; ++c) vV[r][c] = T[0][r] * vST[0][c] + T[1][r] * vST[1][c];
-            float vT[2][3];
-#pragma unroll
-            for (int r = 0; r < 2; ++r)
-#pragma unroll
-                for (int c = 0; c < 3; ++c)
-                    vT[r][c] = 2.f * (vST[r][0] * Cs[0][c] + vST[r][1] * Cs[1][c] + vST[r][2] * Cs[2][c]);
-            const float vJ00 = vT[0][0] * V[0] + vT[0][1] * V[1] + vT[0][2] * V[2];
-            const float vJ02 = vT[0][0] * V[8] + vT[0][1] * V[9] + vT[0][2] * V[10];
-            const float vJ11 = vT[1][0] * V[4] + vT[1][1] * V[5] + vT[1][2] * V[6];
-            const float vJ12 = vT[1][0] * V[8] + vT[1][1] * V[9] + vT[1][2] * V[10];
-            const float vttx = -fx * rz2 * vJ02, vtty = -fy * rz2 * vJ12;
-            vtz += -fx * rz2 * vJ00 + 2.f * fx * ttx * rz3 * vJ02 - fy * rz2 * vJ11 +
-                   2.f * fy * tty * rz3 * vJ12;
-            if (qx == lim_x || qx == -lim_x) { const float h = 0.5f * vttx; vtx += h; vtz += cqx * h; }
-            else if (clamp_x) vtz += cqx * vttx; else vtx += vttx;
-            if (qy == lim_y || qy == -lim_y) { const float h = 0.5f * vtty; vty += h; vtz += cqy * h; }
-            else if (clamp_y) vtz += cqy * vtty; else vty += vtty;
-            vm[0] += V[0] * vtx + V[4] * vty + V[8] * vtz;
-            vm[1] += V[1] * vtx + V[5] * vty + V[9] * vtz;
-            vm[2] += V[2] * vtx + V[6] * vty + V[10] * vtz;
-            if constexpr (CAMGRAD) {
-                const float pc[3] = {px, py, pz}, vt[3] = {vtx, vty, vtz}, vh[3] = {vhx, vhy, vhw};
-#pragma unroll
-                for (int r = 0; r < 3; ++r) {
-#pragma unroll
-                    for (int c = 0; c < 3; ++c) {
-                        cg[4 * r + c] = vt[r] * pc[c];
-                        cg[12 + 4 * r + c] = vh[r] * pc[c];
-                    }
-                    cg[4 * r + 3] = vt[r];
-                    cg[12 + 4 * r + 3] = vh[r];
-                }
-#pragma unroll
-                for (int c = 0; c < 3; ++c) {
-                    cg[c] = cg[c] + J00 * vT[0][c];
-                    cg[4 + c] = cg[4 + c] + J11 * vT[1][c];
-                    cg[8 + c] = cg[8 + c] + (J02 * vT[0][c] + J12 * vT[1][c]);
-                }
-            }
-
-            float vM[3][3];
-#pragma unroll
-            for (int r = 0; r < 3; ++r)
-#pragma unroll
-                for (int c = 0; c < 3; ++c)
-                    vM[r][c] = 2.f * (vV[r][0] * M[0][c] + vV[r][1] * M[1][c] + vV[r][2] * M[2][c]);
-#pragma unroll
-            for (int c = 0; c < 3; ++c) {
-                vs[c] = glob_scale * (R[0][c] * vM[0][c] + R[1][c] * vM[1][c] + R[2][c] * vM[2][c]);
-                if (ACT) vs[c] = vs[c] * e[c];
-                if (F3D) vs[c] = vs[c] * fr[c];
-            }
-            float vR[3][3];
-#pragma unroll
-            for (int r = 0; r < 3; ++r)
-#pragma unroll
-                for (int c = 0; c < 3; ++c) vR[r][c] = vM[r][c] * s[c];
-            const float nq = sqrtf(q.x * q.x + q.y * q.y + q.z * q.z + q.w * q.w);
-            const float inv = 1.0f / nq;
-            const float w = q.x * inv, x = q.y * inv, y = q.z * inv, z = q.w * inv;
-            const float gw = 2.f * (x * (vR[2][1] - vR[1][2]) + y * (vR[0][2] - vR[2][0]) + z * (vR[1][0] - vR[0][1]));
-            const float gx = 2.f * (-2.f * x * (vR[1][1] + vR[2][2]) + y * (vR[1][0] + vR[0][1]) +
-                                    z * (vR[2][0] + vR[0][2]) + w * (vR[2][1] - vR[1][2]));
-            const float gy = 2.f * (x * (vR[1][0] + vR[0][1]) - 2.f * y * (vR[0][0] + vR[2][2]) +
-                                    z * (vR[2][1] + vR[1][2]) + w * (vR[0][2] - vR[2][0]));
-            const float gz = 2.f * (x * (vR[2][0] + vR[0][2]) + y * (vR[2][1] + vR[1][2]) -
-                                    2.f * z * (vR[0][0] + vR[1][1]) + w * (vR[1][0] - vR[0][1]));
-            const float dot = w * gw + x * gx + y * gy + z * gz;
-            vq = make_float4((gw - w * dot) * inv, (gx - x * dot) * inv, (gy - y * dot) * inv,
-                             (gz - z * dot) * inv);
-            if constexpr (F3D) {
-#pragma unroll
-                for (int k = 0; k < 3; ++k) { const float t = f3 / s[k]; fsh[k] = t * t; }
-            }
+            gsb::ProjVjpIn in;
+            in.px = means3d[3 * i]; in.py = means3d[3 * i + 1]; in.pz = means3d[3 * i + 2];
+            in.v_xy = v_xy[i];
+            in.v_depth = v_depth ? v_depth[i] : 0.f;
+            in.A = conics[3 * i]; in.B = conics[3 * i + 1]; in.Cc = conics[3 * i + 2];
+            in.v_conic[0] = v_conic[3 * i]; in.v_conic[1] = v_conic[3 * i + 1]; in.v_conic[2] = v_conic[3 * i + 2];
+            in.q = reinterpret_cast<const float4 *>(quats)[i];
+            in.a[0] = scales[3 * i]; in.a[1] = scales[3 * i + 1]; in.a[2] = scales[3 * i + 2];
+            in.has_v_opacity = v_opacity != nullptr;
+            in.opacity = AA ? opacities[i] : 0.f;
+            in.v_opacity = AA && v_opacity ? v_opacity[i] : 0.f;
+            in.f3 = f3;
+            gsb::project_vjp<ACT, AA, CAMGRAD, F3D>(cam, in, glob_scale, fx, fy, tan_fovx, tan_fovy, img_h, img_w, vm, vs,
+                                                    vq, comp, fr, fc3, fsh, cg);
         } else if constexpr (F3D) {
             const float e[3] = {expf(scales[3 * i]), expf(scales[3 * i + 1]), expf(scales[3 * i + 2])};
             float sg[3];
diff --git a/opensplat_b200/csrc/raster_bwd.cu b/opensplat_b200/csrc/raster_bwd.cu
--- a/opensplat_b200/csrc/raster_bwd.cu
+++ b/opensplat_b200/csrc/raster_bwd.cu
@@ -1,4 +1,4 @@
-#include "raster_common.cuh"
+#include "per_gaussian.cuh"
 
 int gsb_blend_grid(const void *kernel, int num_tiles);
 
@@ -275,31 +275,13 @@
     const int g = blockIdx.x * blockDim.x + threadIdx.x;
     if (g >= n) return;
     const int k0 = g ? cum_tiles_hit[g - 1] : 0, k1 = cum_tiles_hit[g];
-    float a[9] = {0.f, 0.f, 0.f, 0.f, 0.f, 0.f, 0.f, 0.f, 0.f};
-    float az = 0.f;
-    float ax = 0.f, ay = 0.f;
-    for (int k = k0; k < k1; ++k) {
-        const float4 *row = reinterpret_cast<const float4 *>(grad_rows + (size_t)k * GSB_GRAD_ROW_FLOATS);
-        const float4 r0 = row[0], r1 = row[1];
-        a[0] += r0.x; a[1] += r0.y; a[2] += r0.z; a[3] += r0.w;
-        a[4] += r1.x; a[5] += r1.y; a[6] += r1.z; a[7] += r1.w;
-        if (ABS) {
-            const float4 r2 = row[2];
-            a[8] += r2.x;
-            if (DEPTH) az += r2.y;
-            ax += r2.z; ay += r2.w;
-        } else {
-            a[8] += reinterpret_cast<const float *>(row)[8];
-            if (DEPTH) az += reinterpret_cast<const float *>(row)[9];
-        }
-    }
-    const float S0 = a[0], Sx = a[1], Sy = a[2], Sxx = a[3], Sxy = a[4], Syy = a[5];
-    const float ca = conics[3 * g], cb = conics[3 * g + 1], cc = conics[3 * g + 2];
-    const float op = opacities[g];
-    v_xy[g] = make_float2(-(ca * Sx + cb * Sy), -(cb * Sx + cc * Sy));
-    v_conic[3 * g] = -0.5f * Sxx; v_conic[3 * g + 1] = -0.5f * Sxy; v_conic[3 * g + 2] = -0.5f * Syy;
-    v_colors[3 * g] = a[6]; v_colors[3 * g + 1] = a[7]; v_colors[3 * g + 2] = a[8];
-    v_opacity[g] = (op > 0.f) ? S0 / op : 0.f;
+    const gsb::GradRowSums sums = gsb::sum_grad_rows<DEPTH, ABS>(grad_rows, k0, k1);
+    const gsb::BlendGrads v = gsb::blend_grads(sums, conics[3 * g], conics[3 * g + 1], conics[3 * g + 2], opacities[g]);
+    v_xy[g] = v.v_xy;
+    v_conic[3 * g] = v.v_conic[0]; v_conic[3 * g + 1] = v.v_conic[1]; v_conic[3 * g + 2] = v.v_conic[2];
+    v_colors[3 * g] = v.v_rgb[0]; v_colors[3 * g + 1] = v.v_rgb[1]; v_colors[3 * g + 2] = v.v_rgb[2];
+    v_opacity[g] = v.v_opacity;
+    const float az = sums.az, ax = sums.ax, ay = sums.ay;
     if (DEPTH) v_depths[g] = az;
     if (ABS) v_xy_abs[g] = make_float2(ax, ay);
 }
@@ -316,14 +298,14 @@
                     const int32_t *final_idx, const float *v_output, const float *v_output_alpha, void *grad_rows,
                     float *v_xy, float *v_conic, float *v_colors, float *v_opacity, unsigned flags, bool depth,
                     const float *record_depths, const float *v_output_depth, float *v_depths, float *v_xy_abs,
-                    gsb_stream_t stream) {
+                    gsb_stream_t stream, bool reduce = true) {
     GSB_CHECK_ARG(img_h > 0 && img_w > 0 && n >= 0 && m >= 0);
     GSB_CHECK_ARG((flags & ~(unsigned)GSB_RASTER_CLAMP_MAX_ONE) == 0);
     const bool sat = (flags & GSB_RASTER_CLAMP_MAX_ONE) != 0;
     GSB_CHECK_ARG(tiles_x == gsb_div_up(img_w, GSB_TILE) && tiles_y == gsb_div_up(img_h, GSB_TILE));
     if (n == 0) return 0;
-    GSB_CHECK_ARG(tile_bins && conics && opacities && cum_tiles_hit && background && final_Ts && final_idx &&
-                  v_output && v_xy && v_conic && v_colors && v_opacity);
+    GSB_CHECK_ARG(tile_bins && background && final_Ts && final_idx && v_output);
+    GSB_CHECK_ARG(!reduce || (conics && opacities && cum_tiles_hit && v_xy && v_conic && v_colors && v_opacity));
     GSB_CHECK_ARG(!depth || (v_depths && (record_depths || m == 0)));
     GSB_CHECK_ARG(((uintptr_t)v_xy % 8) == 0 && ((uintptr_t)v_xy_abs % 8) == 0);
     const bool abs = v_xy_abs != nullptr;
@@ -353,6 +335,10 @@
         }
 #undef GSB_BWD_LAUNCH
     }
+    if (!reduce) {
+        GSB_LAUNCH_CHECK();
+        return 0;
+    }
 #define GSB_REDUCE_LAUNCH(D, A)                                                                                 \
     reduce_grad_rows_kernel<D, A><<<gsb_div_up(n, 256), 256, 0, s>>>(                                           \
         n, cum_tiles_hit, reinterpret_cast<const float *>(grad_rows), conics, opacities,                        \
@@ -411,3 +397,13 @@
                     v_colors, v_opacity, flags, v_depths != nullptr, record_depths, v_output_depth, v_depths, v_xy_abs,
                     stream);
 }
+
+extern "C" int gsb_rasterize_backward_rows(int img_h, int img_w, int tiles_x, int tiles_y, int n, int m,
+                                           const int32_t *tile_bins, const int32_t *tile_order, void *records,
+                                           const float *background, const float *final_Ts, const int32_t *final_idx,
+                                           const float *v_output, const float *v_output_alpha, void *grad_rows,
+                                           unsigned flags, gsb_stream_t stream) {
+    return backward(img_h, img_w, tiles_x, tiles_y, n, m, tile_bins, tile_order, nullptr, nullptr, records, nullptr,
+                    background, final_Ts, final_idx, v_output, v_output_alpha, grad_rows, nullptr, nullptr, nullptr,
+                    nullptr, flags, false, nullptr, nullptr, nullptr, nullptr, stream, false);
+}
diff --git a/opensplat_b200/csrc/sh.cu b/opensplat_b200/csrc/sh.cu
--- a/opensplat_b200/csrc/sh.cu
+++ b/opensplat_b200/csrc/sh.cu
@@ -1,6 +1,6 @@
 #include <type_traits>
 
-#include "gsb_common.cuh"
+#include "per_gaussian.cuh"
 
 int gsb_sm_count();
 
@@ -196,6 +196,48 @@
 }
 
 template <int K>
+__device__ __forceinline__ void sh_vjp_row(int nb, float vx, float vy, float vz, float v0, float v1, float v2,
+                                           float *__restrict__ tile_row) {
+    constexpr int C = 3 * K;
+    constexpr int S = sh_row_stride(K);
+    float Y[K];
+    sh_basis(nb, vx, vy, vz, Y);
+    float row[S];
+#pragma unroll
+    for (int b = 0; b < K; ++b) {
+        float yb = (b < nb) ? Y[b] : 0.f;
+        row[3 * b] = yb * v0;
+        row[3 * b + 1] = yb * v1;
+        row[3 * b + 2] = yb * v2;
+    }
+#pragma unroll
+    for (int j = C; j < S; ++j) row[j] = 0.f;
+#pragma unroll
+    for (int j = 0; j < S; j += 4)
+        *reinterpret_cast<float4 *>(&tile_row[j]) = make_float4(row[j], row[j + 1], row[j + 2], row[j + 3]);
+}
+
+template <int K>
+__device__ __forceinline__ void store_coeff_span(const float *__restrict__ tile, int ng, float *__restrict__ dst,
+                                                 int vec_ok) {
+    constexpr int C = 3 * K;
+    constexpr int S = sh_row_stride(K);
+    const int total = ng * C;
+    if (vec_ok && (C % 4 == 0)) {
+        float4 *dst4 = reinterpret_cast<float4 *>(dst);
+        for (int f = threadIdx.x; f < total / 4; f += SH_THREADS) {
+            int e = 4 * f, g = e / C, j = e - g * C;
+            stg_stream4(dst4 + f, *reinterpret_cast<const float4 *>(&tile[g * S + j]));
+        }
+    } else {
+        for (int e = threadIdx.x; e < total; e += SH_THREADS) {
+            int g = e / C, j = e - g * C;
+            dst[e] = tile[g * S + j];
+        }
+    }
+}
+
+template <int K>
 __global__ void __launch_bounds__(SH_THREADS)
 sh_backward_kernel(int n, int degrees_to_use, const float *__restrict__ viewdirs,
                    const float *__restrict__ v_colors, float *__restrict__ v_coeffs, int vec_ok,
@@ -210,35 +252,17 @@
     const int t = threadIdx.x;
     if (t < ng) {
         const int g = g0 + t;
-        float Y[K];
-        {
-            float vx = viewdirs[3 * g], vy = viewdirs[3 * g + 1], vz = viewdirs[3 * g + 2];
-            if (cam_pos) { vx -= __ldg(cam_pos); vy -= __ldg(cam_pos + 1); vz -= __ldg(cam_pos + 2); }
-            sh_basis(nb, vx, vy, vz, Y);
-        }
+        float vx = viewdirs[3 * g], vy = viewdirs[3 * g + 1], vz = viewdirs[3 * g + 2];
+        if (cam_pos) { vx -= __ldg(cam_pos); vy -= __ldg(cam_pos + 1); vz -= __ldg(cam_pos + 2); }
         float v0 = v_colors[3 * g], v1 = v_colors[3 * g + 1], v2 = v_colors[3 * g + 2];
         if (rgb_mask) {
             v0 = rgb_grad_passes(rgb_mask[3 * g]) ? v0 : 0.f;
             v1 = rgb_grad_passes(rgb_mask[3 * g + 1]) ? v1 : 0.f;
             v2 = rgb_grad_passes(rgb_mask[3 * g + 2]) ? v2 : 0.f;
         }
-        float row[S];
-#pragma unroll
-        for (int b = 0; b < K; ++b) {
-            float yb = (b < nb) ? Y[b] : 0.f;
-            row[3 * b] = yb * v0;
-            row[3 * b + 1] = yb * v1;
-            row[3 * b + 2] = yb * v2;
-        }
-#pragma unroll
-        for (int j = C; j < S; ++j) row[j] = 0.f;
-#pragma unroll
-        for (int j = 0; j < S; j += 4)
-            *reinterpret_cast<float4 *>(&tile[t * S + j]) = make_float4(row[j], row[j + 1], row[j + 2], row[j + 3]);
+        sh_vjp_row<K>(nb, vx, vy, vz, v0, v1, v2, &tile[t * S]);
     }
     __syncthreads();
-    float *dst = v_coeffs + (size_t)g0 * C;
-    const int total = ng * C;
     if (split) {
         float *dc = v_coeffs + (size_t)g0 * 3, *rs = v_rest + (size_t)g0 * (C - 3);
         for (int e = threadIdx.x; e < ng * 3; e += SH_THREADS) dc[e] = tile[(e / 3) * S + (e % 3)];
@@ -247,18 +271,63 @@
                 const int g = e / (C - 3), j = e - g * (C - 3);
                 rs[e] = tile[g * S + 3 + j];
             }
-    } else if (vec_ok && (C % 4 == 0)) {
-        float4 *dst4 = reinterpret_cast<float4 *>(dst);
-        for (int f = threadIdx.x; f < total / 4; f += SH_THREADS) {
-            int e = 4 * f, g = e / C, j = e - g * C;
-            stg_stream4(dst4 + f, *reinterpret_cast<const float4 *>(&tile[g * S + j]));
-        }
     } else {
-        for (int e = threadIdx.x; e < total; e += SH_THREADS) {
-            int g = e / C, j = e - g * C;
-            dst[e] = tile[g * S + j];
-        }
-    }
+        store_coeff_span<K>(tile, ng, v_coeffs + (size_t)g0 * C, vec_ok);
+    }
+}
+
+template <int K>
+__global__ void __launch_bounds__(SH_THREADS)
+grad_tail_kernel(int n, int degrees_to_use, const int *__restrict__ cum_tiles_hit, const float *__restrict__ grad_rows,
+                 const float *__restrict__ means3d, const float *__restrict__ scales, float glob_scale,
+                 const float *__restrict__ quats, const float *__restrict__ opacities,
+                 const float *__restrict__ viewmat, const float *__restrict__ projmat, float fx, float fy,
+                 float tan_fovx, float tan_fovy, int img_h, int img_w, const int *__restrict__ radii,
+                 const float *__restrict__ conics, const float *__restrict__ viewdirs, const float *__restrict__ rgbs,
+                 float *__restrict__ v_opacity, float *__restrict__ v_mean3d, float *__restrict__ v_scale,
+                 float4 *__restrict__ v_quat, float *__restrict__ v_coeffs, int vec_ok) {
+    constexpr int C = 3 * K;
+    constexpr int S = sh_row_stride(K);
+    __shared__ __align__(16) float tile[SH_THREADS * S];
+    const int g0 = blockIdx.x * SH_THREADS;
+    const int ng = min(SH_THREADS, n - g0);
+    const int nb = min(nb_of(degrees_to_use), K);
+    const int t = threadIdx.x;
+    if (t < ng) {
+        const int g = g0 + t;
+        const int k0 = g ? cum_tiles_hit[g - 1] : 0, k1 = cum_tiles_hit[g];
+        const float ca = conics[3 * g], cb = conics[3 * g + 1], cc = conics[3 * g + 2];
+        const gsb::BlendGrads v = gsb::blend_grads(gsb::sum_grad_rows<false, false>(grad_rows, k0, k1), ca, cb, cc,
+                                                   opacities[g]);
+        v_opacity[g] = v.v_opacity;
+        float vm[3] = {0.f, 0.f, 0.f}, vs[3] = {0.f, 0.f, 0.f};
+        float4 vq = make_float4(0.f, 0.f, 0.f, 0.f);
+        if (radii[g] > 0) {
+            gsb::Cam cam;
+            gsb::load_cam(viewmat, projmat, cam);
+            gsb::ProjVjpIn in;
+            in.px = means3d[3 * g]; in.py = means3d[3 * g + 1]; in.pz = means3d[3 * g + 2];
+            in.v_xy = v.v_xy;
+            in.v_depth = 0.f;
+            in.A = ca; in.B = cb; in.Cc = cc;
+            in.v_conic[0] = v.v_conic[0]; in.v_conic[1] = v.v_conic[1]; in.v_conic[2] = v.v_conic[2];
+            in.q = reinterpret_cast<const float4 *>(quats)[g];
+            in.a[0] = scales[3 * g]; in.a[1] = scales[3 * g + 1]; in.a[2] = scales[3 * g + 2];
+            in.opacity = 0.f; in.v_opacity = 0.f; in.f3 = 0.f; in.has_v_opacity = false;
+            float comp = 0.f, fr[3], fc3 = 1.f, fsh[3], cg[gsb::CG_TERMS];
+            gsb::project_vjp<false, false, false, false>(cam, in, glob_scale, fx, fy, tan_fovx, tan_fovy, img_h, img_w,
+                                                         vm, vs, vq, comp, fr, fc3, fsh, cg);
+        }
+        v_mean3d[3 * g] = vm[0]; v_mean3d[3 * g + 1] = vm[1]; v_mean3d[3 * g + 2] = vm[2];
+        v_scale[3 * g] = vs[0]; v_scale[3 * g + 1] = vs[1]; v_scale[3 * g + 2] = vs[2];
+        v_quat[g] = vq;
+        const float v0 = rgb_grad_passes(rgbs[3 * g]) ? v.v_rgb[0] : 0.f;
+        const float v1 = rgb_grad_passes(rgbs[3 * g + 1]) ? v.v_rgb[1] : 0.f;
+        const float v2 = rgb_grad_passes(rgbs[3 * g + 2]) ? v.v_rgb[2] : 0.f;
+        sh_vjp_row<K>(nb, viewdirs[3 * g], viewdirs[3 * g + 1], viewdirs[3 * g + 2], v0, v1, v2, &tile[t * S]);
+    }
+    __syncthreads();
+    store_coeff_span<K>(tile, ng, v_coeffs + (size_t)g0 * C, vec_ok);
 }
 
 template <bool PEER_CAMS>
@@ -502,6 +571,39 @@
     return launch_sh_backward(n, degree, degrees_to_use, viewdirs, v_rgbs, v_coeffs, rgbs, stream);
 }
 
+extern "C" int gsb_grad_tail(int n, int degree, int degrees_to_use, const int32_t *cum_tiles_hit,
+                             const void *grad_rows, const float *means3d, const float *scales, float glob_scale,
+                             const float *quats, const float *opacities, const float *viewmat, const float *projmat,
+                             float fx, float fy, int img_h, int img_w, const int32_t *radii, const float *conics,
+                             const float *viewdirs, const float *rgbs, float *v_opacity, float *v_mean3d,
+                             float *v_scale, float *v_quat, float *v_coeffs, gsb_stream_t stream) {
+    GSB_CHECK_ARG(n >= 0 && bases_of_degree(degree) > 0 && degrees_to_use >= 0 && degrees_to_use <= degree);
+    GSB_CHECK_ARG(img_h > 0 && img_w > 0);
+    if (n == 0) return 0;
+    GSB_CHECK_ARG(cum_tiles_hit && grad_rows && means3d && scales && quats && opacities && viewmat && projmat && radii &&
+                  conics && viewdirs && rgbs && v_opacity && v_mean3d && v_scale && v_quat && v_coeffs);
+    GSB_CHECK_ARG(((uintptr_t)grad_rows % 16) == 0 && ((uintptr_t)quats % 16) == 0 && ((uintptr_t)v_quat % 16) == 0);
+    const float tan_fovx = (float)(0.5 * (double)img_w / (double)fx);
+    const float tan_fovy = (float)(0.5 * (double)img_h / (double)fy);
+    cudaStream_t s = (cudaStream_t)stream;
+    const int grid = gsb_div_up(n, SH_THREADS);
+    const int vec_ok = ((uintptr_t)v_coeffs % 16) == 0;
+#define GSB_TAIL(K) grad_tail_kernel<K><<<grid, SH_THREADS, 0, s>>>(                                                  \
+        n, degrees_to_use, cum_tiles_hit, reinterpret_cast<const float *>(grad_rows), means3d, scales, glob_scale,     \
+        quats, opacities, viewmat, projmat, fx, fy, tan_fovx, tan_fovy, img_h, img_w, radii, conics, viewdirs, rgbs,   \
+        v_opacity, v_mean3d, v_scale, reinterpret_cast<float4 *>(v_quat), v_coeffs, vec_ok)
+    switch (degree) {
+        case 0: GSB_TAIL(1); break;
+        case 1: GSB_TAIL(4); break;
+        case 2: GSB_TAIL(9); break;
+        case 3: GSB_TAIL(16); break;
+        default: GSB_TAIL(25); break;
+    }
+#undef GSB_TAIL
+    GSB_LAUNCH_CHECK();
+    return 0;
+}
+
 extern "C" int gsb_sh_forward_split(int n, int degree, int degrees_to_use, const float *means, const float *cam_pos,
                                     const float *features_dc, const float *features_rest, float bias, float *rgbs,
                                     gsb_stream_t stream) {
diff --git a/opensplat_b200/pipeline.py b/opensplat_b200/pipeline.py
--- a/opensplat_b200/pipeline.py
+++ b/opensplat_b200/pipeline.py
@@ -178,10 +178,24 @@
         cnt = H * W * 3
         self._stage("loss")
         capi.check(L.gsb_mse_loss_grad(cnt, P(self.out_img), P(self.target), P(self.v_img), P(self.loss), 1.0 / cnt, s))
-        v_rgbs = self.exchange.v_rgbs_buffer() if self.exchange is not None else self.v_rgbs
+        if self.exchange is None:
+            self._stage("raster_bwd")
+            capi.check(L.gsb_rasterize_backward_rows(
+                H, W, self.tb[0], self.tb[1], n, self.m_raster, P(self.tile_bins),
+                P(self.tile_order) if self._ordered else None, P(self.records), P(self.background), P(self.final_Ts),
+                P(self.final_idx), P(self.v_img), None, P(self.grad_rows), 0, s))
+            self._stage("grad_tail")
+            capi.check(L.gsb_grad_tail(n, self.deg, self.deg, P(self.cum), P(self.grad_rows), P(p["means"]),
+                                       P(p["scales"]), 1.0, P(p["quats"]), P(p["opacities"]), P(self.viewmat),
+                                       P(self.projmat), fx, fy, H, W, P(self.radii), P(self.conics), P(self.viewdirs),
+                                       P(self.rgbs), P(g["opacities"]), P(g["means"]), P(g["scales"]), P(g["quats"]),
+                                       P(g["coeffs"]), s))
+            self._stage("end_bwd")
+            return self.loss
+        v_rgbs = self.exchange.v_rgbs_buffer()
         self._stage("raster_bwd")
         self._raster_backward(p["opacities"], g["opacities"], v_rgbs, 0)
-        if self.exchange is not None and self.exchange.overlap:
+        if self.exchange.overlap:
             self.exchange.start_colour(average=True)
         self._stage("project_bwd")
         capi.check(L.gsb_project_backward(n, P(p["means"]), P(p["scales"]), 1.0, P(p["quats"]), P(self.viewmat),
@@ -189,14 +203,10 @@
                                           P(self.v_xy), None, P(self.v_conic), P(g["means"]), P(g["scales"]),
                                           P(g["quats"]), s))
         self._stage("sh_bwd")
-        if self.exchange is not None:
-            if self.exchange.overlap:
-                self.exchange.finish()
-            else:
-                self.exchange.exchange(average=True)
+        if self.exchange.overlap:
+            self.exchange.finish()
         else:
-            capi.check(L.gsb_sh_backward_rgb(n, self.deg, self.deg, P(self.viewdirs), P(self.rgbs), P(self.v_rgbs),
-                                             P(g["coeffs"]), s))
+            self.exchange.exchange(average=True)
         self._stage("end_bwd")
         return self.loss
 
@@ -266,8 +276,7 @@
             "sort": 8 * m + passes * 24 * m,
             "bins": 8 * m + 8 * T,
             "raster_fwd": 40 * m + 20 * P,
-            "raster_bwd": 40 * m + 20 * P + 36 * n,
-            "project_bwd": 144 * n,
-            "sh_bwd": n * (12 + 12 * K + 12),
+            "raster_bwd": 40 * m + 20 * P,
+            "grad_tail": n * (88 + 44 + 12 * K),
         }
         return stages, passes
```

New measurement: 1111 (median of 6 runs). 1.8% higher.
